# timweiland/DiffEqGMRFs.jl

Hardware: AMD Instinct MI355X
Metric: GMRF posterior solves/sec (mean+samples), 256^2 Darcy (higher is better)
Workload: dtype f64; 1 GPU; darcy256: n=65536, 64 blocks x 1024, nnz=1624084; 256 independent posterior(s) per GPU and step (4 stream(s) x batch 64), each factor + mean + 64 samples; mode=problems, samples_per_problem_per_rank=64, l_blocks_kept=False

## Files before the change

### diffeqgmrfs.jl_amd/api.py

```python
from __future__ import annotations

import ctypes as C
from typing import List, Optional, Sequence, Tuple

import numpy as np
import scipy.sparse as sp

from . import _cabi
from ._cabi import GmrfError, NotPositiveDefinite


def _is_torch(x) -> bool:
    return hasattr(x, "data_ptr") and hasattr(x, "device")


def _colmajor(b, n: int):
    if _is_torch(b):
        import torch
        if b.dtype != torch.float64:
            raise TypeError("float64 required")
        if b.dim() == 1:
            if b.shape[0] != n:
                raise ValueError("dimension mismatch")
            return b.contiguous(), 1, n, True
# ... 453 lines not shown
        return {f: (list(getattr(s, f)) if hasattr(getattr(s, f), "__len__") else getattr(s, f)) for f, _ in s._fields_}

    def select_problem(self, p: int):
        _cabi.check(self._lib.gmrf_bt_select_problem(self._h, int(p)))

    def solve_batch(self, b, mode: int = _cabi.SOLVE_FULL):
        B, k, n = b.shape
        if B != self.batch or n != self.N:
            raise ValueError("expected shape (batch, k, n)")
        if _is_torch(b):
            import torch
            b = b.contiguous()
            out = torch.empty_like(b)
        else:
            b = np.ascontiguousarray(b, dtype=np.float64)
            out = np.empty_like(b)
        _cabi.check(self._lib.gmrf_bt_solve(self._h, _cabi.ptr(b), _cabi.ptr(out), k, n, n, mode))
        return out

    def sample_batch(self, k: int, mean=None, seed: int = 0x5EED, first_id: int = 0, like=None):
        B, n = self.batch, self.N
        ref = like if like is not None else mean
        if _is_torch(ref):
            import torch
            out = torch.empty((B, k, n), dtype=torch.float64, device=ref.device)
            if mean is not None:
                mean = mean.contiguous()
        else:
            out = np.empty((B, k, n), dtype=np.float64)
            if mean is not None:
                mean = np.ascontiguousarray(mean, dtype=np.float64)
        _cabi.check(self._lib.gmrf_bt_sample(self._h, seed, first_id, k, _cabi.ptr(mean), None, _cabi.ptr(out), n))
        return out

    def factor(self, A, N_blocks: int, values=None):
        A = sp.csc_matrix(A)
        if A.shape[0] != A.shape[1]:
            raise ValueError("matrix must be square")
        if not A.has_sorted_indices:
            A = A.copy()
            A.sort_indices()
        n = A.shape[0]
        colptr = A.indptr.astype(np.int64)
        rowval = A.indices.astype(np.int64)
        nz = np.ascontiguousarray(A.data if values is None else values, dtype=np.float64)
        if nz.size != self.batch * A.nnz:
            raise ValueError("values must hold batch * nnz entries")
        info = C.c_int32(0)
        st = self._lib.gmrf_bt_factor_csc(self._h, n, int(N_blocks), _cabi.ptr(colptr), _cabi.ptr(rowval),
                                          _cabi.ptr(nz), 0, C.byref(info))
        _cabi.check(st, info.value)
        self._set_shape(n, int(N_blocks))
        self._pattern = (colptr, rowval)
        return self

    def factor_blocks(self, diag_blocks, off_diag_blocks):
        nb = len(diag_blocks)
        bs = diag_blocks[0].shape[0]
        keep = []

        def mk(blocks):
            arr = (_cabi.SparseBlock * max(len(blocks), 1))()
            for i, b in enumerate(blocks):
                b = sp.csc_matrix(b)
                b.sort_indices()
                p = b.indptr.astype(np.int64); ix = b.indices.astype(np.int64); v = b.data.astype(np.float64)
                keep.extend([p, ix, v])
                arr[i].nnz = b.nnz
                arr[i].ptr = p.ctypes.data; arr[i].idx = ix.ctypes.data; arr[i].val = v.ctypes.data
            return arr

        d = mk(diag_blocks)
        lo = mk(off_diag_blocks)
        info = C.c_int32(0)
        st = self._lib.gmrf_bt_factor_blocks(self._h, nb * bs, nb, C.cast(d, C.c_void_p), C.cast(lo, C.c_void_p),
                                             0, 1, C.byref(info))
        _cabi.check(st, info.value)
        self._set_shape(nb * bs, nb)
        return self

    def refactor(self, nzval):
        info = C.c_int32(0)
        if not _is_torch(nzval):
            nzval = np.ascontiguousarray(nzval, dtype=np.float64)
        st = self._lib.gmrf_bt_refactor_values(self._h, _cabi.ptr(nzval), C.byref(info))
        _cabi.check(st, info.value)
        return self

    def _set_shape(self, n, nb):
        self.N = n
        self.n_blocks = nb
        self.block_size = n // nb
        self.chos = _LazyBlocks(self, _cabi.BLOCK_L, nb)
        self.Cs = _LazyBlocks(self, _cabi.BLOCK_C, nb - 1)
        self.inverses = _LazyBlocks(self, _cabi.BLOCK_LINV, nb)

    def _solve(self, b, mode: int, out=None):
        xa, k, ld, one_d = _colmajor(b, self.N)
        if out is None:
            store, view = _alloc_like(xa, self.N, k, one_d)
        else:
            store, view = out, out
        _cabi.check(self._lib.gmrf_bt_solve(self._h, _cabi.ptr(xa), _cabi.ptr(store), k, ld, self.N, mode))
        return view

    def get_block(self, kind: int, i: int) -> np.ndarray:
        bs = self.block_size
        out = np.empty((bs, bs), dtype=np.float64, order="F")
        _cabi.check(self._lib.gmrf_bt_get_block(self._h, kind, i, _cabi.ptr(out), bs))
        return out

    def logdet(self) -> float:
        v = C.c_double(0.0)
        _cabi.check(self._lib.gmrf_bt_logdet(self._h, C.byref(v)))
        return v.value

    def normals(self, k: int, seed: int = 0x5EED, first_id: int = 0, like=None):
        if self.batch != 1:
            raise ValueError("a batched handle draws (batch, k, n) normals: normals_batch")
        store, view = _alloc_like(like if like is not None else np.empty(0), self.N, k, False)
        _cabi.check(self._lib.gmrf_bt_normals(self._h, seed, first_id, k, _cabi.ptr(store), self.N))
        return view

    def normals_batch(self, k: int, seed: int = 0x5EED, first_id: int = 0):
        out = np.empty((self.batch, k, self.N), dtype=np.float64)
        _cabi.check(self._lib.gmrf_bt_normals(self._h, seed, first_id, k, _cabi.ptr(out), self.N))
        return out

    def sample(self, k: int, mean=None, z=None, seed: int = 0x5EED, first_id: int = 0, like=None):
        ref = like if like is not None else (z if z is not None else (mean if mean is not None else np.empty(0)))
        za = None
        if z is not None:
            za, kz, _, _ = _colmajor(z, self.N)
            k = kz
        if mean is not None and not _is_torch(mean):
            mean = np.ascontiguousarray(mean, dtype=np.float64)
        store, view = _alloc_like(ref if _is_torch(ref) else np.empty(0), self.N, k, False)
        _cabi.check(self._lib.gmrf_bt_sample(self._h, seed, first_id, k, _cabi.ptr(mean), _cabi.ptr(za),
                                             _cabi.ptr(store), self.N))
        return view

    def posterior(self, b, k: int, seed: int = 0x5EED, first_id: int = 0):
        if self.batch != 1:
            raise ValueError("posterior(): one problem per handle (use solve_batch / sample_batch for batches)")
        xa, kb, ld, one_d = _colmajor(b, self.N)
        if kb != 1:
            raise ValueError("posterior(): one right-hand side")
        mstore, mview = _alloc_like(xa, self.N, 1, True)
        sstore, sview = _alloc_like(xa, self.N, k, False)
        _cabi.check(self._lib.gmrf_bt_posterior(self._h, _cabi.ptr(xa), seed, first_id, k, _cabi.ptr(mstore), _cabi.ptr(sstore),
                                                self.N))
        return mview, sview

    def marginal_var(self, method: str = "exact", k: int = 50, seed: int = 0x5EED, Q: Optional[CsrMatrix] = None,
                     q_values=None, out=None):
        m = {"exact": _cabi.VAR_EXACT, "rbmc": _cabi.VAR_RBMC, "mc": _cabi.VAR_MC}[method]
        shape = (self.N,) if self.batch == 1 else (self.batch, self.N)
        if out is None:
            out = np.empty(shape, dtype=np.float64)
        else:
            ok = tuple(out.shape) == shape and (out.is_contiguous() and str(out.dtype) == "torch.float64" if _is_torch(out)
                                                else out.flags.c_contiguous and out.dtype == np.float64)
            if not ok:
                raise ValueError(f"out must be a contiguous float64 array of shape {shape}")
        if self.batch > 1 and m != _cabi.VAR_EXACT:
            qv = None
            if q_values is not None:
                qv = q_values.contiguous() if _is_torch(q_values) else np.ascontiguousarray(q_values, dtype=np.float64)
            _cabi.check(self._lib.gmrf_bt_marginal_var_batch(self._h, m, k, seed, Q._h if Q is not None else None,
                                                             _cabi.ptr(qv) if qv is not None else None, _cabi.ptr(out)))
            return out
        _cabi.check(self._lib.gmrf_bt_marginal_var(self._h, m, k, seed, Q._h if Q is not None else None,
                                                   _cabi.ptr(out)))
        return out

    def var_accumulate(self, acc, method: str, first_id: int, k: int, seed: int = 0x5EED,
                       Q: Optional[CsrMatrix] = None):
        m = {"rbmc": _cabi.VAR_RBMC, "mc": _cabi.VAR_MC}[method]
        _cabi.check(self._lib.gmrf_bt_var_accumulate(self._h, m, first_id, k, seed,
                                                     Q._h if Q is not None else None, _cabi.ptr(acc)))
        return acc

    def stats(self) -> dict:
        s = _cabi.Stats()
        _cabi.check(self._lib.gmrf_bt_stats(self._h, C.byref(s)))
        out = {}
        for f, _ in s._fields_:
            v = getattr(s, f)
            out[f] = list(v) if hasattr(v, "__len__") else v
        return out

    def gemm_shapes(self) -> list:
        n = C.c_int64(0)
        _cabi.check(self._lib.gmrf_test_gemm_shapes(self._h, None, 0, C.byref(n)))
        buf = np.zeros((max(int(n.value), 1), 11))
        _cabi.check(self._lib.gmrf_test_gemm_shapes(self._h, buf.ctypes.data_as(C.POINTER(C.c_double)), buf.shape[0], C.byref(n)))
        names = ("class", "M", "N", "K", "tri", "lower_only", "problems", "k_bounds")
        return [dict({k: int(r[i]) for i, k in enumerate(names)}, launches=int(r[8]), ms=float(r[9]), flops=float(r[10]))
                for r in buf[: int(n.value)]]

    def set_profiling(self, level: int):
        _cabi.check(self._lib.gmrf_bt_set_profiling(self._h, level))

    def set_eager(self, eager: bool):
        _cabi.check(self._lib.gmrf_bt_set_eager(self._h, int(eager)))

    def synchronize(self):
        _cabi.check(self._lib.gmrf_bt_synchronize(self._h))

    def factor_buffer(self, kind: int) -> Tuple[int, int]:
        p = C.c_void_p()
        nbytes = C.c_int64(0)
        _cabi.check(self._lib.gmrf_bt_factor_buffer(self._h, kind, C.byref(p), C.byref(nbytes)))
        return int(p.value or 0), int(nbytes.value)

    def export_factor(self) -> np.ndarray:
        nbytes = C.c_int64(0)
        _cabi.check(self._lib.gmrf_bt_export_size(self._h, C.byref(nbytes)))
        buf = np.empty(nbytes.value, dtype=np.uint8)
        _cabi.check(self._lib.gmrf_bt_export_factor(self._h, _cabi.ptr(buf), nbytes.value))
        return buf

    def import_factor(self, image: np.ndarray):
        image = np.ascontiguousarray(image, dtype=np.uint8)
        _cabi.check(self._lib.gmrf_bt_import_factor(self._h, _cabi.ptr(image), image.size))
        hdr = image[:64].view(np.int64)
        self._set_shape(int(hdr[2]), int(hdr[3]))
        return self

    def adopt_shape(self, n: int, n_blocks: int):
        _cabi.check(self._lib.gmrf_bt_adopt_shape(self._h, n, n_blocks))
        self._set_shape(n, n_blocks)

    def get_layout(self) -> np.ndarray:
        cnt = C.c_int64(0)
        _cabi.check(self._lib.gmrf_bt_get_layout(self._h, None, 0, C.byref(cnt)))
        out = np.zeros(cnt.value, dtype=np.int64)
        _cabi.check(self._lib.gmrf_bt_get_layout(self._h, _cabi.ptr(out), out.size, C.byref(cnt)))
        return out

    def adopt_layout(self, n: int, n_blocks: int, layout=None):
        if layout is None:
            _cabi.check(self._lib.gmrf_bt_adopt_layout(self._h, n, n_blocks, None, 0))
        else:
            lay = np.ascontiguousarray(layout, dtype=np.int64)
            _cabi.check(self._lib.gmrf_bt_adopt_layout(self._h, n, n_blocks, _cabi.ptr(lay), lay.size))
        self._set_shape(n, n_blocks)

    def adopt_commit(self, l_blocks_valid: bool = False):
        _cabi.check(self._lib.gmrf_bt_adopt_commit(self._h, int(l_blocks_valid)))

    def set_keep_l(self, keep: bool):
        _cabi.check(self._lib.gmrf_bt_set_keep_l(self._h, int(keep)))

    def block_range(self, kind: int, i0: int, i1: int):
        a, b, c = C.c_int64(0), C.c_int64(0), C.c_int64(0)
        _cabi.check(self._lib.gmrf_bt_block_range(self._h, kind, i0, i1, C.byref(a), C.byref(b), C.byref(c)))
        return a.value, b.value, c.value

    def packed_size(self, i0: int, i1: int) -> int:
        v = C.c_int64(0)
        _cabi.check(self._lib.gmrf_bt_packed_size(self._h, i0, i1, C.byref(v)))
        return v.value

    def pack_blocks_async(self, i0: int, i1: int, dev_buf):
        _cabi.check(self._lib.gmrf_bt_pack_blocks_async(self._h, i0, i1, _cabi.ptr(dev_buf)))

    def unpack_blocks_async(self, i0: int, i1: int, dev_buf):
        _cabi.check(self._lib.gmrf_bt_unpack_blocks_async(self._h, i0, i1, _cabi.ptr(dev_buf)))

    def factor_begin(self, A, N_blocks: int):
        A = sp.csc_matrix(A)
        n = A.shape[0]
        colptr = A.indptr.astype(np.int64); rowval = A.indices.astype(np.int64)
        nz = np.ascontiguousarray(A.data, dtype=np.float64)
        _cabi.check(self._lib.gmrf_bt_factor_begin_csc(self._h, n, int(N_blocks), _cabi.ptr(colptr),
                                                       _cabi.ptr(rowval), _cabi.ptr(nz), 0))
        self._set_shape(n, int(N_blocks))

    def factor_begin_values(self, nzval):
        if not _is_torch(nzval):
            nzval = np.ascontiguousarray(nzval, dtype=np.float64)
        _cabi.check(self._lib.gmrf_bt_factor_begin_csc(self._h, self.N, self.n_blocks, None, None,
                                                       _cabi.ptr(nzval), 0))

    def factor_step_async(self, i0: int, i1: int):
        _cabi.check(self._lib.gmrf_bt_factor_step_async(self._h, i0, i1))

    def factor_end(self):
        info = C.c_int32(0)
        st = self._lib.gmrf_bt_factor_end(self._h, C.byref(info))
        _cabi.check(st, info.value)



def tridiagonal_cholesky(A, N_blocks: int, device: int = 0, stream: int = 0, order: str = "reference",
                         meet: Optional[int] = None) -> TridiagonalCholeskyFactor:
    n = A.shape[0]
    if N_blocks <= 0 or n % N_blocks != 0:
        raise ValueError("size(A,1) must be a positive multiple of N_blocks")
    return TridiagonalCholeskyFactor(device, stream, order=order, meet=meet).factor(A, N_blocks)


def forward_solve(L: TridiagonalCholeskyFactor, b):
    return L._solve(b, _cabi.SOLVE_FORWARD)

# ... 124 lines not shown
```

### diffeqgmrfs.jl_amd/csrc/gemm_f64_dma.hpp

```cpp
#pragma once
#include "gemm_f64.hpp"

namespace gmrf {

constexpr int DMA_BK = 16;
constexpr int DMA_ROWS_ASCENDING = 1024;
#ifndef GMRF_DMA_READS_FIRST
#define GMRF_DMA_READS_FIRST 0
#endif

template <int BM, int BN>
constexpr size_t gemm_dma_lds_bytes(int stages) { return (size_t)stages * (BM + BN) * DMA_BK * sizeof(double); }

#define GMRF_LDS_PTR(p) ((__attribute__((address_space(3))) void*)(p))
#define GMRF_GLB_PTR(p) ((const __attribute__((address_space(1))) void*)(p))

template <int BM, int BN>
__device__ __forceinline__ void gemm_dma_tile_order(const GemmArgs& g, int& bm, int& bn, int& z) {
    const int nx = g.N / BN, ny = g.M / BM;
    int tpp;
    if (g.lower_only == 1) {
        if (BM >= BN) tpp = (BM / BN) * ny * (ny + 1) / 2;
        else tpp = 0;
    } else tpp = nx * ny;
    const int nz = (int)gridDim.x / tpp;
    const int groups = (nz % 8 == 0) ? 8 : 1;
    const int xg = (int)blockIdx.x % groups, q = (int)blockIdx.x / groups, nzg = nz / groups;
    int zq;
    if (g.lower_only == 1) {
        constexpr int R = BM / BN > 0 ? BM / BN : 1;
        const int tile = q % tpp;
        zq = q / tpp;
        const int tr = (g.tri & DMA_ROWS_ASCENDING) ? tile : tpp - 1 - tile;
        int b = (int)((sqrtf(8.0f * (float)(tr / R) + 1.0f) - 1.0f) * 0.5f);
        while (R * b * (b + 1) / 2 > tr) --b;
        while (R * (b + 1) * (b + 2) / 2 <= tr) ++b;
        bm = b;
        bn = tr - R * b * (b + 1) / 2;
    } else {
        const bool cls_n = (g.tri & (TRI_B_LOWER | TRI_B_UPPER)) || !(g.tri & (TRI_A_LOWER | TRI_A_UPPER));
        const bool desc = cls_n ? ((g.tri & TRI_B_UPPER) != 0 || (g.ke_n && !g.kb_n)) : (g.tri & TRI_A_LOWER) != 0;
        const int ncls = cls_n ? nx : ny, other = cls_n ? ny : nx;
        int c = q / (other * nzg);
        const int rem = q % (other * nzg);
        const int o = rem % other;
        zq = rem / other;
        if (desc) c = ncls - 1 - c;
        bn = cls_n ? c : o;
        bm = cls_n ? o : c;
    }
    z = xg + groups * zq;
}

template <int BM, int BN, bool B_N, int STAGES, bool A_T = false>
__global__ __launch_bounds__(256, (BM + BN > 128) ? 3 : 4) void gemm_f64_dma(GemmArgs g) {
    constexpr int BK = DMA_BK;
    constexpr int MI = BM / 32, NJ = BN / 32;
    constexpr int NA = BM / 32, NB = BN / 32;
    constexpr int A_ST = BM * BK, B_ST = BN * BK, ST = A_ST + B_ST;
    static_assert(NJ % 2 == 0 || !B_N, "the [k][n] image pairs neighbouring column tiles");
    static_assert(MI % 2 == 0 || !A_T, "the [k][m] image pairs neighbouring row tiles");
    int bm, bn, z;
    gemm_dma_tile_order<BM, BN>(g, bm, bn, z);
    const int m0 = bm * BM, n0 = bn * BN;
    if (g.lower_only == 2 && n0 > m0 + BM - 1) return;
    const int zi = z % g.nb1, zp = z / g.nb1;
    const double* __restrict__ A = g.A + (int64_t)zi * g.strideA + (int64_t)zp * g.pA;
    const double* __restrict__ B = g.B + (int64_t)zi * g.strideB + (int64_t)zp * g.pB;
    double* C = g.C + (int64_t)zi * g.strideC + (int64_t)zp * g.pC;
    const double* Dm = g.D ? g.D + (int64_t)zp * g.pD : C;
    const int64_t ldd = g.D ? g.ldd : g.ldc;

    int kb = 0, ke = g.K;
    if (g.tri & TRI_A_LOWER) ke = min(ke, m0 + BM);
    if (g.tri & TRI_A_UPPER) kb = max(kb, m0);
    if (g.tri & TRI_B_LOWER) kb = max(kb, n0);
    if (g.tri & TRI_B_UPPER) ke = min(ke, n0 + BN);
    if (g.kb_m) kb = max(kb, g.kb_m[bm * (BM / 64)]);
    if (g.kb_n) kb = max(kb, g.kb_n[bn * (BN / 64)]);
    if (g.ke_n) ke = min(ke, g.ke_n[bn * (BN / 64) + BN / 64 - 1]);
    const int nkt = (ke > kb) ? (ke - kb) / BK : 0;

    extern __shared__ __attribute__((aligned(16))) double gsm[];
    const int t = threadIdx.x;
    const int lane = t & 63, w = __builtin_amdgcn_readfirstlane(t >> 6);
    const int wm = (w >> 1) * (BM / 2), wn = (w & 1) * (BN / 2);
    const int li = lane & 15, lq = lane >> 4;
    const bool idle = g.lower_only != 0 && ((n0 + wn) / 64 > (m0 + wm + BM / 2 - 1) / 64);

    uint32_t offa[NA], offb[NB];
#pragma unroll
    for (int i = 0; i < NA; ++i) {
        const int q = w + 4 * i;
        if (A_T) {
            constexpr int LPR = BM / 2;
            const int k = q * (64 / LPR) + lane / LPR, col = (lane % LPR) * 2;
            offa[i] = (uint32_t)(((int64_t)k * g.lda + m0 + col) * 8);
        } else {
            const int row = 8 * q + (lane >> 3), ch = (lane & 7) ^ ((row >> 1) & 7);
            offa[i] = (uint32_t)(((int64_t)(m0 + row) * g.lda + 2 * ch) * 8);
        }
    }
#pragma unroll
    for (int i = 0; i < NB; ++i) {
        const int q = w + 4 * i;
        if (B_N) {
            constexpr int LPR = BN / 2;
            const int k = q * (64 / LPR) + lane / LPR, col = (lane % LPR) * 2;
            offb[i] = (uint32_t)(((int64_t)k * g.ldb + n0 + col) * 8);
        } else {
            const int row = 8 * q + (lane >> 3), ch = (lane & 7) ^ ((row >> 1) & 7);
            offb[i] = (uint32_t)(((int64_t)(n0 + row) * g.ldb + 2 * ch) * 8);
        }
    }
    auto issue = [&](int kt, int stage) {
        const int k0 = kb + kt * BK;
        const char* abase = reinterpret_cast<const char*>(A_T ? A + (int64_t)k0 * g.lda : A + k0);
        const char* bbase = reinterpret_cast<const char*>(B_N ? B + (int64_t)k0 * g.ldb : B + k0);
        double* as = gsm + stage * ST;
        double* bs = as + A_ST;
#pragma unroll
        for (int i = 0; i < NA; ++i) {
            asm volatile("" : "+v"(offa[i]));
            __builtin_amdgcn_global_load_lds(GMRF_GLB_PTR(abase + offa[i]), GMRF_LDS_PTR(as + (w + 4 * i) * 128), 16, 0, 0);
        }
#pragma unroll
        for (int i = 0; i < NB; ++i) {
            asm volatile("" : "+v"(offb[i]));
            __builtin_amdgcn_global_load_lds(GMRF_GLB_PTR(bbase + offb[i]), GMRF_LDS_PTR(bs + (w + 4 * i) * 128), 16, 0, 0);
        }
    };

    v4d acc[MI][NJ];
#pragma unroll
    for (int i = 0; i < MI; ++i)
#pragma unroll
        for (int j = 0; j < NJ; ++j) acc[i][j] = (v4d){0.0, 0.0, 0.0, 0.0};

    int fa[MI], fb[NJ];
#pragma unroll
    for (int i = 0; i < MI; ++i) {
        const int row = wm + 16 * i + li;
        fa[i] = A_T ? (2 * lq + (i & 1)) * BM + wm + 32 * (i >> 1) + 2 * li : row * 16 + 2 * (lq ^ ((row >> 1) & 3));
    }
    int sa2[MI], sb2[NJ];
#pragma unroll
    for (int i = 0; i < MI; ++i) { const int row = wm + 16 * i + li; sa2[i] = (!A_T && ((row >> 1) & 4)) ? 8 : 0; }
    if (!B_N) {
#pragma unroll
        for (int j = 0; j < NJ; ++j) {
            const int row = wn + 16 * j + li;
            fb[j] = A_ST + row * 16 + 2 * (lq ^ ((row >> 1) & 3));
            sb2[j] = ((row >> 1) & 4) ? 8 : 0;
        }
    } else {
#pragma unroll
        for (int j = 0; j < NJ; ++j) { fb[j] = A_ST + (2 * lq + (j & 1)) * BN + wn + 32 * (j >> 1) + 2 * li; sb2[j] = 0; }
    }

    constexpr int DEPTH = STAGES - 1;
#pragma unroll
    for (int s = 0; s < DEPTH; ++s)
        if (s < nkt) issue(s, s);
    for (int kt = 0; kt < nkt; ++kt) {
        const int ahead = min(DEPTH - 1, nkt - 1 - kt);
        if (ahead <= 0) asm volatile("s_waitcnt vmcnt(0)" ::: "memory");
        else if (ahead == 1) asm volatile("s_waitcnt vmcnt(%0)" ::"n"(NA + NB) : "memory");
        else asm volatile("s_waitcnt vmcnt(%0)" ::"n"(2 * (NA + NB)) : "memory");
        __builtin_amdgcn_s_barrier();
        __builtin_amdgcn_sched_barrier(0);
        if (!GMRF_DMA_READS_FIRST && kt + DEPTH < nkt) issue(kt + DEPTH, (kt + DEPTH) % STAGES);
        if (!idle) {
            const double* sm = gsm + (kt % STAGES) * ST;
            v2d a[BK / 8][MI], b[BK / 8][NJ];
#pragma unroll
            for (int kg = 0; kg < BK / 8; ++kg) {
#pragma unroll
                for (int i = 0; i < MI; ++i) a[kg][i] = *reinterpret_cast<const v2d*>(sm + fa[i] + (A_T ? kg * 8 * BM : ((kg * 8) ^ sa2[i])));
#pragma unroll
                for (int j = 0; j < NJ; ++j)
                    b[kg][j] = *reinterpret_cast<const v2d*>(sm + fb[j] + (B_N ? kg * 8 * BN : ((kg * 8) ^ sb2[j])));
            }
            __builtin_amdgcn_sched_barrier(0);
            if (GMRF_DMA_READS_FIRST && kt + DEPTH < nkt) issue(kt + DEPTH, (kt + DEPTH) % STAGES);
            __builtin_amdgcn_sched_barrier(0);
#pragma unroll
            for (int kg = 0; kg < BK / 8; ++kg)
#pragma unroll
                for (int p = 0; p < 2; ++p)
#pragma unroll
                    for (int i = 0; i < MI; ++i)
#pragma unroll
                        for (int j = 0; j < NJ; ++j) {
                            double av;
                            if (A_T) av = (i & 1) ? a[kg][2 * (i >> 1) + p].y : a[kg][2 * (i >> 1) + p].x;
                            else av = p ? a[kg][i].y : a[kg][i].x;
                            double bv;
                            if (B_N) bv = (j & 1) ? b[kg][2 * (j >> 1) + p].y : b[kg][2 * (j >> 1) + p].x;
                            else bv = p ? b[kg][j].y : b[kg][j].x;
                            acc[i][j] = __builtin_amdgcn_mfma_f64_16x16x4f64(av, bv, acc[i][j], 0, 0, 0);
                        }
            __builtin_amdgcn_sched_barrier(0);
        } else if (GMRF_DMA_READS_FIRST && kt + DEPTH < nkt) issue(kt + DEPTH, (kt + DEPTH) % STAGES);
    }
    if (idle) return;

    const double alpha = g.alpha, beta = g.beta;
    auto orow = [&](int i, int r) -> int64_t {
        return A_T ? m0 + wm + 32 * (i >> 1) + 2 * (lq + 4 * r) + (i & 1) : m0 + wm + i * 16 + lq + 4 * r;
    };
    if (B_N) {
        v2d d[MI][4][NJ / 2 > 0 ? NJ / 2 : 1];
        if (beta != 0.0) {
#pragma unroll
            for (int i = 0; i < MI; ++i)
#pragma unroll
                for (int r = 0; r < 4; ++r)
#pragma unroll
                    for (int jp = 0; jp < NJ / 2; ++jp)
                        d[i][r][jp] = *reinterpret_cast<const v2d*>(Dm + orow(i, r) * ldd + n0 + wn + jp * 32 + 2 * li);
        }
#pragma unroll
        for (int i = 0; i < MI; ++i)
#pragma unroll
            for (int r = 0; r < 4; ++r)
#pragma unroll
                for (int jp = 0; jp < NJ / 2; ++jp) {
                    v2d v = (v2d){alpha * acc[i][2 * jp][r], alpha * acc[i][2 * jp + 1][r]};
                    if (beta != 0.0) { v.x += beta * d[i][r][jp].x; v.y += beta * d[i][r][jp].y; }
                    *reinterpret_cast<v2d*>(C + orow(i, r) * g.ldc + n0 + wn + jp * 32 + 2 * li) = v;
                }
    } else {
        double d[MI][4][NJ];
        if (beta != 0.0) {
#pragma unroll
            for (int i = 0; i < MI; ++i)
#pragma unroll
                for (int r = 0; r < 4; ++r)
#pragma unroll
                    for (int j = 0; j < NJ; ++j)
                        d[i][r][j] = Dm[orow(i, r) * ldd + n0 + wn + j * 16 + li];
        }
#pragma unroll
        for (int i = 0; i < MI; ++i)
#pragma unroll
            for (int r = 0; r < 4; ++r)
#pragma unroll
                for (int j = 0; j < NJ; ++j) {
                    double v = alpha * acc[i][j][r];
                    if (beta != 0.0) v += beta * d[i][r][j];
                    C[orow(i, r) * g.ldc + n0 + wn + j * 16 + li] = v;
                }
    }
}

inline int& gemm_dma_policy() {
    static int v = [] { const char* e = getenv("GMRF_GEMM_DMA"); return e ? atoi(e) : 2; }();
    return v;
}
inline int& gemm_dma_force() {
    static int v = 0;
    return v;
}
inline int gemm_dma_stages() {
    static const int v = [] { const char* e = getenv("GMRF_GEMM_DMA_STAGES"); const int s = e ? atoi(e) : 2; return s == 3 ? 3 : 2; }();
    return v;
}

inline int gemm_dma_shape(bool a_t, const GemmArgs& g, int batch) {
    const int policy = gemm_dma_force() ? 2 : gemm_dma_policy();
    if (policy == 0 || g.stamps || (g.tri & ~15) || g.K % DMA_BK || g.M % 64 || g.N % 64) return 0;
    if ((g.lda & 1) || (g.ldb & 1) || ((uintptr_t)g.A & 15) || ((uintptr_t)g.B & 15) || ((g.strideA | g.strideB | g.pA | g.pB) & 1)) return 0;
    if (((uintptr_t)g.C & 15) || (g.ldc & 1) || ((g.strideC | g.pC) & 1)) return 0;
    if (g.D && (((uintptr_t)g.D & 15) || (g.ldd & 1) || (g.pD & 1))) return 0;
    if ((int64_t)g.M * g.ldc * 8 >= ((int64_t)1 << 32) || (g.D && (int64_t)g.M * g.ldd * 8 >= ((int64_t)1 << 32))) return 0;
    if ((int64_t)(a_t ? g.K : g.M) * g.lda * 8 >= ((int64_t)1 << 32) || (int64_t)std::max(g.N, g.K) * g.ldb * 8 >= ((int64_t)1 << 32)) return 0;
    if (a_t) return 1;
    const int force = gemm_dma_force();
    if (force == 2 && g.M % 128 == 0) return 2;
    if (force == 3 && g.N % 128 == 0 && !g.lower_only) return 3;
    if (force) return 1;
    if (policy == 1) return 1;
    const bool plain = !g.lower_only && !g.tri && !g.kb_m && !g.kb_n && !g.ke_n;
    const int64_t t64 = (int64_t)(g.M / 64) * (g.N / 64) * batch;
    if (policy >= 3 || (plain && t64 >= 2048)) {
        if (g.M % 128 == 0) return 2;
        if (g.N % 128 == 0 && !g.lower_only) return 3;
    }
    return 1;
}
inline bool gemm_uses_dma(bool a_t, const GemmArgs& g, int batch) { return gemm_dma_shape(a_t, g, batch) != 0; }

inline hipError_t gemm_dma_init() {
    hipError_t e = hipSuccess;
#define GMRF_DMA_ATTR(BM, BN, BNAT, ST)                                                                          \
    if (e == hipSuccess)                                                                                          \
        e = hipFuncSetAttribute((const void*)gemm_f64_dma<BM, BN, BNAT, ST>, hipFuncAttributeMaxDynamicSharedMemorySize, \
                                (int)gemm_dma_lds_bytes<BM, BN>(ST) + 64 * 1024);
    GMRF_DMA_ATTR(64, 64, false, 2) GMRF_DMA_ATTR(64, 64, true, 2) GMRF_DMA_ATTR(64, 64, false, 3) GMRF_DMA_ATTR(64, 64, true, 3)
    GMRF_DMA_ATTR(128, 64, false, 2) GMRF_DMA_ATTR(128, 64, true, 2) GMRF_DMA_ATTR(128, 64, false, 3) GMRF_DMA_ATTR(128, 64, true, 3)
    GMRF_DMA_ATTR(64, 128, false, 2) GMRF_DMA_ATTR(64, 128, true, 2) GMRF_DMA_ATTR(64, 128, false, 3) GMRF_DMA_ATTR(64, 128, true, 3)
#undef GMRF_DMA_ATTR
    return e;
}

inline bool gemm_try_dma(hipStream_t st, bool a_t, bool b_n, const GemmArgs& g, int batch, hipEvent_t ev_start, hipEvent_t ev_stop,
                         hipError_t* err) {
    const int shape = gemm_dma_shape(a_t, g, batch);
    if (shape == 0) return false;
    const bool tri_grid = g.lower_only && g.M == g.N;
    GemmArgs gs = g;
    gs.lower_only = tri_grid ? 1 : (g.lower_only ? 2 : 0);
    static const bool asc_off = [] { const char* e = getenv("GMRF_GEMM_G2_ORDER"); return e && atoi(e) == 0; }();
    if (tri_grid && (g.kb_m || g.kb_n) && !asc_off) gs.tri |= DMA_ROWS_ASCENDING;
    const int stages = gemm_dma_stages();
    const dim3 block(256);
#define GMRF_DMA_GO(BM, BN)                                                                                       \
    do {                                                                                                          \
        const int64_t nx = g.N / BN, ny = g.M / BM;                                                               \
        const int64_t tiles = tri_grid ? (int64_t)(BM / BN > 0 ? BM / BN : 1) * ny * (ny + 1) / 2 : nx * ny;      \
        const dim3 grid((unsigned)(tiles * batch));                                                               \
        static const size_t lds_pad = [] { const char* e = getenv("GMRF_GEMM_DMA_LDS_PAD_KB"); return (size_t)(e ? atoi(e) : 0) * 1024; }();    \
        const size_t lds = gemm_dma_lds_bytes<BM, BN>(stages) + lds_pad;                                          \
        if (a_t && BM == 64 && BN == 64) {                                                                        \
            if (b_n) GMRF_DMA_K((gemm_f64_dma<64, 64, true, 2, true>)); else GMRF_DMA_K((gemm_f64_dma<64, 64, false, 2, true>)); \
        } else if (stages == 3) {                                                                                 \
            if (b_n) GMRF_DMA_K((gemm_f64_dma<BM, BN, true, 3>)); else GMRF_DMA_K((gemm_f64_dma<BM, BN, false, 3>)); \
        } else {                                                                                                  \
            if (b_n) GMRF_DMA_K((gemm_f64_dma<BM, BN, true, 2>)); else GMRF_DMA_K((gemm_f64_dma<BM, BN, false, 2>)); \
        }                                                                                                         \
    } while (0)
#define GMRF_DMA_K(KERNEL)                                                                                        \
    do {                                                                                                          \
        if (ev_start) hipExtLaunchKernelGGL(KERNEL, grid, block, lds, st, ev_start, ev_stop, 0, gs);              \
        else hipLaunchKernelGGL(KERNEL, grid, block, lds, st, gs);                                                \
    } while (0)
    if (shape == 2) GMRF_DMA_GO(128, 64);
    else if (shape == 3) GMRF_DMA_GO(64, 128);
    else GMRF_DMA_GO(64, 64);
#undef GMRF_DMA_K
#undef GMRF_DMA_GO
    *err = hipGetLastError();
    return true;
}

}
```

### diffeqgmrfs.jl_amd/csrc/gmrf_hip.hip

```cpp
#include <hip/hip_runtime.h>
#include <dlfcn.h>
#include <stdint.h>
#include <stdlib.h>
#include <string.h>
#include <time.h>

#include <algorithm>
#include <iterator>
#include <cmath>
#include <map>
#include <memory>
#include <chrono>
#include <functional>
#include <initializer_list>
#include <mutex>
#include <string>
#include <type_traits>
#include <vector>

#include "../../include/gmrf_hip.h"
#include "assemble.hpp"
#include "fem_assemble.hpp"
#include "gemm_f64.hpp"
#include "gemm_f64_dma.hpp"
// ... 4 lines not shown
#include "sweep.hpp"
#include "sweep_persist.hpp"
#include "swe_assemble.hpp"
#include "fem_assemble_p2.hpp"

using namespace gmrf;

static thread_local std::string g_last_error;
static double g_tile_us = 0.0;
static unsigned long long g_tile_stamps[64];
static unsigned long long g_persist_stamps[128];

#define HIPCHK(expr)                                                                        \
    do {                                                                                    \
        hipError_t _e = (expr);                                                             \
        if (_e != hipSuccess) {                                                             \
            g_last_error = std::string(#expr) + ": " + hipGetErrorString(_e);               \
            return GMRF_ERR_HIP;                                                            \
        }                                                                                   \
    } while (0)

#define GCHK(expr)                                                                          \
    do {                                                                                    \
        gmrf_status _s = (expr);                                                            \
        if (_s != GMRF_OK) return _s;                                                       \
    } while (0)

static gmrf_status bad_shape(const char* msg) {
    g_last_error = msg;
    return GMRF_ERR_BAD_SHAPE;
}

static bool is_device_ptr(const void* p) {
    if (!p) return false;
    hipPointerAttribute_t attr;
    hipError_t e = hipPointerGetAttributes(&attr, p);
    if (e != hipSuccess) {
        (void)hipGetLastError();
        return false;
    }
    return attr.type == hipMemoryTypeDevice || attr.type == hipMemoryTypeManaged;
}

static bool ranges_overlap(const void* p, int64_t pb, const void* q, int64_t qb) {
    if (!p || !q || pb <= 0 || qb <= 0) return false;
    const uintptr_t a = reinterpret_cast<uintptr_t>(p), b = reinterpret_cast<uintptr_t>(q);
    return a < b + (uintptr_t)qb && b < a + (uintptr_t)pb;
}

static int64_t cols_bytes(int64_t n, int64_t cols, int64_t ld) {
    return cols <= 0 ? 0 : ((cols - 1) * ld + n) * (int64_t)sizeof(double);
}

static int64_t next_pow2(int64_t v) {
    int64_t p = 1;
    while (p < v) p <<= 1;
    return p;
}

struct gmrf_csr {
    int device = 0;
    hipStream_t stream = nullptr;
    bool own_stream = false;
    int64_t n_rows = 0, n_cols = 0, nnz = 0;
    int64_t* d_rowptr = nullptr;
    int32_t* d_colidx = nullptr;
    double* d_vals = nullptr;
    float* d_vals32 = nullptr;
    double* d_diag = nullptr;
    bool tiles128_ok = false;
    bool tiles_ok = false;
    double* d_stage_x = nullptr;
    double* d_stage_y = nullptr;
    int64_t stage_cap = 0;
    int plan_state = 0;
    int64_t* d_tile_uptr = nullptr;
    int32_t* d_ucols = nullptr;
    uint16_t* d_lidx = nullptr;
    int64_t n_ucols = 0;
    int plan_rows = 0, plan_ucap = 0, plan_ecap = 0, plan_ecap_pad = 0, plan_umax = 0;
};

struct EvPair {
    hipEvent_t a, b;
    int kind;
    double work;
    int shape = -1;
};

struct GemmShapeStat {
    int64_t key[8];
    double launches = 0, ms = 0, work = 0;
};

struct TwistState;

struct gmrf_handle {
    int device = 0;
    hipStream_t stream = nullptr;
    bool own_stream = false;
    int64_t n = 0, N = 0, bs = 0, bsp = 0, n_pad = 0;
    int64_t B = 1;
    int64_t sel = 0;
    int64_t alloc_B = 0, vals_B = 0;
    int64_t nnz_in = 0, n_entries = 0;
    uint64_t* d_keys = nullptr;
    double* d_vals = nullptr;
    int64_t* d_src = nullptr;
    double* d_nz_stage = nullptr;
    std::vector<int64_t> diag_first, diag_count, low_first, low_count;
    bool analyzed = false;
    int64_t cmin = 0, rmax = 0;
    std::vector<int> kst, mend;
    int* d_kst = nullptr;
    int* d_mend = nullptr;
    int* d_kbx = nullptr;
    int kst_cap = 0;
    double c_streamed = 0.0;
    double g2_tile_k = 0.0;
    bool c_dirty = false;
    int* d_lo_rowptr = nullptr;
    int* d_dg_rowptr = nullptr;
    int* d_bxt_uptr = nullptr; int* d_bxt_ucols = nullptr; uint16_t* d_bxt_lidx = nullptr; int* d_bxt_gtiles = nullptr;
    std::vector<int> bxt_ng;
    int bxt_ecap = 0; int bxt_nrt = 0; bool bxt_plan_ok = false;
    int64_t lo_row_max = 0;
    bool sparse_b = false;
    bool dense_g1 = false;
    double *d_L = nullptr, *d_C = nullptr, *d_Linv = nullptr;
    bool external_storage = false;
    bool keep_l = true;
    bool l_valid = false;
    bool logdet_valid = false;
    std::vector<char> got_block;
    int64_t alloc_rm = 0, alloc_wc = 0;
    bool alloc_keep_l = true;
    double *d_S = nullptr, *d_B = nullptr, *d_T = nullptr, *d_W = nullptr;
    double* d_V = nullptr;
    int64_t v_elems = 0;
    int* d_info = nullptr;
    double* d_logdet = nullptr;
    int64_t alloc_N = 0, alloc_bsp = 0;
    bool factored = false;
    double *d_P = nullptr, *d_Y = nullptr, *d_Tp = nullptr;
    int64_t kp_cap = 0;
    double* d_stage = nullptr;
    int64_t stage_cap = 0;
    double* d_mean = nullptr;
    double* d_acc = nullptr;
    int64_t acc_B = 0;
    bool eager = false;
    bool split_step = false;
    bool sweep_no_gemm = false;
    unsigned long long* dbg_stamps = nullptr;
    bool fork_graph = false;
    bool no_staircase = false;
    bool doubling_x = false;
    int xsplit = 0;
    int adopt_xsplit = 0;
    bool no_xsplit = false;
    bool no_lookahead = false;
    bool no_persist = false;
    bool persist_gave_up = false;
    bool persist_launched = false;
    int persist_cus = 0;
    int info_checked = 0;
    int factor_graph_route = 0;
    int persist_aborts = 0;
    int cu_count = 0;
    unsigned* d_pflags = nullptr;
    int64_t pflags_words = 0;
    bool no_sweep_persist = false;
    bool no_scatter_fold = false;
    bool sweep_persist_planned = false;
    bool sweep_persist_launched = false;
    unsigned* d_sweep_flags = nullptr;
    double* d_Tsw = nullptr;
    int64_t t_elems = 0;
    unsigned* h_sweep_abort = nullptr;
    int sweep_nw = 0;
    double *d_P2 = nullptr, *d_Y2 = nullptr, *d_T2 = nullptr;
    int64_t p2_elems = 0;
    bool sweep_persist_hold = false;
    bool no_persist_panels = false;
    hipStream_t aux = nullptr;
    bool aux_distinct = false;
    hipStream_t gemm_stream = nullptr;
    bool capturing = false;
    std::vector<hipEvent_t> fork_events;
    size_t fork_next = 0;
    hipGraphExec_t factor_graph = nullptr;
    int64_t factor_graph_i0 = -1, factor_graph_i1 = -1;
    std::map<int64_t, hipGraphExec_t> sweep_graphs;
    int profiling = 0;
    std::vector<EvPair> events;
    std::vector<hipEvent_t> ev_pool;
    std::vector<GemmShapeStat> gemm_shapes;
    gmrf_stats stats;
    hipEvent_t ev0 = nullptr, ev1 = nullptr;
    int order = GMRF_ORDER_REFERENCE;
    int64_t meet_req = -1;
    int32_t eager_bits = 0;
    TwistState* tw = nullptr;
    int64_t tw_blk = -1;
    const double* tw_hj = nullptr;
    double* tw_w = nullptr;
};

struct TwistState {
    gmrf_handle* top = nullptr;
    gmrf_handle* bot = nullptr;
    int64_t m = -1, N = 0, n = 0, bs = 0, bsp = 0, nnz = 0;
    uint64_t* d_mkeys = nullptr;
    int64_t* d_msrc = nullptr;
    double* d_mvals = nullptr;
    int64_t m_count = 0;
    double *d_Bm = nullptr, *d_HJ = nullptr, *d_W = nullptr, *d_Smm = nullptr;
    int64_t dense_bsp = 0;
    double* d_nz = nullptr;
    const double* d_nz_cur = nullptr;
    double* d_z = nullptr;
    double* d_var = nullptr;
    hipEvent_t ev_fork = nullptr, ev_join = nullptr;
};


static bool tw_on(const gmrf_handle* h) { return h && h->tw && h->tw->bot; }
static gmrf_handle* tw_route(gmrf_handle* h) {
    return (h && h->order == GMRF_ORDER_TWISTED && h->tw && h->tw->top && !h->tw->bot && h->factored) ? h->tw->top : h;
}
static gmrf_status tw_refuse(const gmrf_handle* h, const char* what) {
    if (!h || h->order != GMRF_ORDER_TWISTED) return GMRF_OK;
    g_last_error = std::string(what) + ": not supported on a handle in the twisted elimination order (gmrf_bt_set_order)";
    return GMRF_ERR_BAD_SHAPE;
}

static void destroy_graphs(gmrf_handle* h) {
    if (h->factor_graph) { (void)hipGraphExecDestroy(h->factor_graph); h->factor_graph = nullptr; }
    for (auto& kv : h->sweep_graphs) (void)hipGraphExecDestroy(kv.second);
    h->sweep_graphs.clear();
}

static hipEvent_t ev_get(gmrf_handle* h) {
    if (!h->ev_pool.empty()) {
        hipEvent_t e = h->ev_pool.back();
        h->ev_pool.pop_back();
        return e;
    }
    hipEvent_t e;
    (void)hipEventCreate(&e);
    return e;
}

struct ProfScope {
    gmrf_handle* h;
    EvPair p;
    bool on;
    ProfScope(gmrf_handle* hh, int kind, double work) : h(hh), on(hh->profiling > 0) {
        if (on) {
            p.kind = kind; p.work = work;
            p.a = ev_get(h); p.b = ev_get(h);
            (void)hipEventRecord(p.a, h->stream);
        }
    }
    ~ProfScope() {
        if (on) {
            (void)hipEventRecord(p.b, h->stream);
            h->events.push_back(p);
        }
    }
};

static void prof_collect(gmrf_handle* h) {
    for (auto& p : h->events) {
        float ms = 0.f;
        (void)hipEventElapsedTime(&ms, p.a, p.b);
        h->stats.kernel_ms[p.kind] += ms; h->stats.kernel_work[p.kind] += p.work; h->stats.kernel_launches[p.kind]++;
        if (p.shape >= 0) { auto& g = h->gemm_shapes[(size_t)p.shape]; g.launches += 1; g.ms += ms; g.work += p.work; }
        h->ev_pool.push_back(p.a);
        h->ev_pool.push_back(p.b);
    }
    h->events.clear();
}

static gmrf_status gemm(gmrf_handle* h, bool a_t, bool b_n, int M, int N, int K, int tri, int lower_only,
                        double alpha, const double* A, int64_t lda, const double* B, int64_t ldb,
                        double beta, double* C, int64_t ldc, int64_t pA, int64_t pB, int64_t pC,
                        int batch = 1, int64_t sA = 0, int64_t sB = 0, int64_t sC = 0, const double* D = nullptr,
                        int64_t ldd = 0, int64_t pD = 0, int pclass = 0, double pwork = -1.0,
                        const int* kb_m = nullptr, const int* kb_n = nullptr, const int* ke_n = nullptr) {
    GemmArgs g;
    g.kb_m = kb_m; g.kb_n = kb_n; g.ke_n = ke_n;
    g.D = D; g.ldd = ldd; g.pD = pD;
    g.A = A; g.B = B; g.C = C;
    g.lda = lda; g.ldb = ldb; g.ldc = ldc;
    g.strideA = sA; g.strideB = sB; g.strideC = sC;
    g.pA = pA; g.pB = pB; g.pC = pC; g.nb1 = batch;
    g.M = M; g.N = N; g.K = K; g.tri = tri; g.lower_only = lower_only;
    g.alpha = alpha; g.beta = beta; g.stamps = nullptr;
    double flops = 2.0 * M * N * (double)K * batch * (double)h->B;
    if (lower_only) flops *= 0.5 * (1.0 + 64.0 / std::max(M, 64));
    if (tri) flops *= 0.5 * (1.0 + 64.0 / std::max(K, 64));
    if (gemm_uses_big(a_t, g, batch * (int)h->B)) { pclass = b_n ? 7 : 6; pwork = -1.0; }
    else if (pclass == 0) {
        if (gemm_uses_ll(g, batch * (int)h->B)) pclass = 13;
        else if (gemm_uses_dma(a_t, g, batch * (int)h->B)) pclass = a_t ? 18 : (b_n ? 15 : 14);
        else pclass = a_t ? 12 : (b_n ? 11 : 0);
    }
    if (h->profiling > 0) {
        EvPair p;
        p.kind = pclass; p.work = pwork >= 0.0 ? pwork : flops;
        p.a = ev_get(h); p.b = ev_get(h);
        const int64_t key[8] = {pclass, M, N, K, tri, lower_only, batch * h->B, (kb_m || kb_n || ke_n) ? 1 : 0};
        for (size_t i = 0; i < h->gemm_shapes.size() && p.shape < 0; ++i)
            if (!memcmp(h->gemm_shapes[i].key, key, sizeof(key))) p.shape = (int)i;
        if (p.shape < 0) {
            GemmShapeStat st; memcpy(st.key, key, sizeof(key));
            h->gemm_shapes.push_back(st); p.shape = (int)h->gemm_shapes.size() - 1;
        }
        HIPCHK(launch_gemm(h->gemm_stream ? h->gemm_stream : h->stream, a_t, b_n, g, batch * (int)h->B, p.a, p.b));
        h->events.push_back(p);
        return GMRF_OK;
    }
    HIPCHK(launch_gemm(h->gemm_stream ? h->gemm_stream : h->stream, a_t, b_n, g, batch * (int)h->B));
    return GMRF_OK;
}

static void free_dev(void* p) {
    if (p) (void)hipFree(p);
}

static inline int64_t blk_elems(const gmrf_handle* h) { return h->bsp * h->bsp; }
static inline int64_t c_ld(const gmrf_handle* h) { return h->bsp - h->cmin; }
static inline int64_t c_blk(const gmrf_handle* h) { return h->rmax * (h->bsp - h->cmin); }
static inline int64_t stride_pL(const gmrf_handle* h) { return blk_elems(h) * (h->keep_l ? h->N : 1); }
static inline int64_t stride_pX(const gmrf_handle* h) { return blk_elems(h) * h->N; }
static inline int64_t stride_pC(const gmrf_handle* h) { return c_blk(h) * std::max<int64_t>(h->N - 1, 1); }
static inline double* l_block(const gmrf_handle* h, int64_t i) { return h->d_L + (h->keep_l ? i * blk_elems(h) : 0); }

static gmrf_status set_layout(gmrf_handle* h, int64_t cmin, int64_t rmax, const std::vector<int64_t>& kst_abs) {
    const int64_t bsp = h->bsp;
    if (cmin < 0 || cmin >= bsp || cmin % 64 || rmax <= 0 || rmax > bsp || rmax % 64) return bad_shape("bad coupling-block layout");
    const int nrt = (int)(rmax / 64), nct = (int)((bsp - cmin) / 64), ntile = (int)(bsp / 64);
    if ((int)kst_abs.size() != nrt) return bad_shape("bad coupling-block layout (row tiles)");
    (void)hipStreamSynchronize(h->stream);
    destroy_graphs(h);
    h->cmin = cmin; h->rmax = rmax;
    h->kst.assign((size_t)ntile, 0);
    int64_t run = bsp - 64;
    for (int t = nrt - 1; t >= 0; --t) {
        int64_t v = std::min(std::max(kst_abs[t], cmin), bsp - 64);
        run = std::min(run, (v / 64) * 64);
        h->kst[t] = (int)(run - cmin);
    }
    if (nrt > 0) h->kst[0] = 0;
    for (int t = nrt; t < ntile; ++t) h->kst[t] = (int)(bsp - cmin);
    h->mend.assign((size_t)ntile, (int)rmax);
    for (int u = 0; u < nct; ++u) {
        int m = 0;
        for (int t = 0; t < nrt; ++t) if (h->kst[t] <= 64 * u) m = 64 * (t + 1);
        h->mend[u] = m;
    }
    h->c_streamed = 0.0; h->g2_tile_k = 0.0;
    for (int t = 0; t < nrt; ++t) {
        h->c_streamed += 64.0 * (double)(bsp - cmin - h->kst[t]);
        h->g2_tile_k += (double)(t + 1) * (double)(bsp - cmin - h->kst[t]);
    }
    if (!h->d_kst || !h->d_mend || h->kst_cap < ntile) {
        free_dev(h->d_kst); free_dev(h->d_mend); free_dev(h->d_kbx); h->d_kst = h->d_mend = h->d_kbx = nullptr; h->kst_cap = 0;
        HIPCHK(hipMalloc(&h->d_kst, sizeof(int) * ntile));
        HIPCHK(hipMalloc(&h->d_mend, sizeof(int) * ntile));
        HIPCHK(hipMalloc(&h->d_kbx, sizeof(int) * ntile));
        h->kst_cap = ntile;
    }
    {
        std::vector<int> kbx((size_t)ntile);
        for (int u = 0; u < ntile; ++u) kbx[(size_t)u] = (int)std::max<int64_t>(0, 64 * (int64_t)u - cmin);
        HIPCHK(hipMemcpyAsync(h->d_kbx, kbx.data(), sizeof(int) * ntile, hipMemcpyHostToDevice, h->stream));
        HIPCHK(hipStreamSynchronize(h->stream));
    }
    HIPCHK(hipMemcpyAsync(h->d_kst, h->kst.data(), sizeof(int) * ntile, hipMemcpyHostToDevice, h->stream));
    HIPCHK(hipMemcpyAsync(h->d_mend, h->mend.data(), sizeof(int) * ntile, hipMemcpyHostToDevice, h->stream));
    HIPCHK(hipStreamSynchronize(h->stream));
    h->c_dirty = true;
    return GMRF_OK;
}

static gmrf_status set_layout_dense(gmrf_handle* h) {
    return set_layout(h, 0, h->bsp, std::vector<int64_t>((size_t)(h->bsp / 64), 0));
}

static gmrf_status alloc_work(gmrf_handle* h);
static gmrf_status alloc_factor(gmrf_handle* h) {
    if (h->alloc_N == h->N && h->alloc_bsp == h->bsp && h->alloc_B == h->B && h->alloc_rm == h->rmax &&
        h->alloc_wc == c_ld(h) && h->alloc_keep_l == h->keep_l && h->d_Linv)
        return GMRF_OK;
    destroy_graphs(h);
    h->logdet_valid = false;
    if (h->external_storage) {
        if (h->alloc_N != h->N || h->alloc_bsp != h->bsp || h->alloc_B != h->B || h->alloc_keep_l != h->keep_l) {
            g_last_error = "external factor storage does not match the shape / batch";
            return GMRF_ERR_BAD_SHAPE;
        }
        h->alloc_rm = h->rmax; h->alloc_wc = c_ld(h);
        h->l_valid = false;
        return GMRF_OK;
    }
    free_dev(h->d_L); free_dev(h->d_C); free_dev(h->d_Linv);
    free_dev(h->d_S); free_dev(h->d_B); free_dev(h->d_T); free_dev(h->d_W);
    free_dev(h->d_logdet);
    h->d_L = h->d_C = h->d_Linv = h->d_S = h->d_B = h->d_T = h->d_W = h->d_logdet = nullptr;
    h->l_valid = false;
    const size_t blk = (size_t)blk_elems(h) * sizeof(double) * (size_t)h->B;
    HIPCHK(hipMalloc(&h->d_L, blk * (h->keep_l ? h->N : 1)));
    HIPCHK(hipMalloc(&h->d_Linv, blk * h->N));
    HIPCHK(hipMalloc(&h->d_C, (size_t)stride_pC(h) * sizeof(double) * (size_t)h->B));
    HIPCHK(hipMemsetAsync(h->d_L, 0, blk * (h->keep_l ? h->N : 1), h->stream));
    HIPCHK(hipMemsetAsync(h->d_Linv, 0, blk * h->N, h->stream));
    HIPCHK(hipMemsetAsync(h->d_C, 0, (size_t)stride_pC(h) * sizeof(double) * (size_t)h->B, h->stream));
    h->c_dirty = false;
    GCHK(alloc_work(h));
    h->alloc_rm = h->rmax; h->alloc_wc = c_ld(h); h->alloc_keep_l = h->keep_l;
    return GMRF_OK;
}

static gmrf_status alloc_work(gmrf_handle* h) {
    const size_t blk = (size_t)blk_elems(h) * sizeof(double) * (size_t)h->B;
    HIPCHK(hipMalloc(&h->d_S, blk));
    HIPCHK(hipMalloc(&h->d_B, blk));
    HIPCHK(hipMalloc(&h->d_T, blk));
    HIPCHK(hipMalloc(&h->d_W, blk));
    HIPCHK(hipMalloc(&h->d_logdet, sizeof(double) * h->N * h->B));
    {
        const int64_t words = (int64_t)persist_flag_words((int)(h->bsp / 64)) * h->B;
        if (!h->d_pflags || h->pflags_words < words) {
            free_dev(h->d_pflags); h->d_pflags = nullptr; h->pflags_words = 0;
            HIPCHK(hipMalloc(&h->d_pflags, sizeof(unsigned) * (size_t)words));
            HIPCHK(hipMemsetAsync(h->d_pflags, 0, sizeof(unsigned) * (size_t)words, h->stream));
            HIPCHK(hipStreamSynchronize(h->stream));
            h->pflags_words = words;
        }
    }
    h->alloc_N = h->N; h->alloc_bsp = h->bsp; h->alloc_B = h->B;
    h->stats.factor_bytes = (int64_t)(blk * ((h->keep_l ? 2 : 1) * h->N) + (size_t)stride_pC(h) * sizeof(double) * (size_t)h->B);
    return GMRF_OK;
}

static void release_shape_buffers(gmrf_handle* h) {
    for (auto& kv : h->sweep_graphs) (void)hipGraphExecDestroy(kv.second);
    h->sweep_graphs.clear();
    free_dev(h->d_P); free_dev(h->d_Y); free_dev(h->d_Tp);
    h->d_P = h->d_Y = h->d_Tp = nullptr; h->kp_cap = 0;
    free_dev(h->d_mean); h->d_mean = nullptr;
    free_dev(h->d_acc); h->d_acc = nullptr; h->acc_B = 0;
    free_dev(h->d_stage); h->d_stage = nullptr; h->stage_cap = 0;
// ... 909 lines not shown
    return std::chrono::duration<double, std::milli>(std::chrono::steady_clock::now() - t0).count();
}

gmrf_status gmrf_streams_create(int32_t device, int32_t n, void** streams, int32_t* n_distinct) {
    if (n <= 0 || n > 32 || !streams) return bad_shape("gmrf_streams_create: 1 <= n <= 32 streams");
    HIPCHK(hipSetDevice(device));
    const int ncand = std::min(3 * n + 4, 48);
    std::vector<hipStream_t> cand((size_t)ncand, nullptr);
    for (int i = 0; i < ncand; ++i) {
        if (hipStreamCreateWithFlags(&cand[(size_t)i], hipStreamNonBlocking) != hipSuccess) {
            for (int j = 0; j < i; ++j) (void)hipStreamDestroy(cand[(size_t)j]);
            g_last_error = "hipStreamCreateWithFlags failed"; return GMRF_ERR_HIP;
        }
        hipLaunchKernelGGL(gmrf_spin_kernel, dim3(1), dim3(64), 0, cand[(size_t)i], 1ull);
    }
    HIPCHK(hipDeviceSynchronize());
    const unsigned long long ticks = 100000ull;
    double one = 1e30;
    for (int r = 0; r < 3; ++r) one = std::min(one, spin_pair_ms(cand[0], nullptr, ticks));
    std::vector<int> chosen;
    for (int i = 0; i < ncand && (int)chosen.size() < n; ++i) {
        bool ok = true;
        for (int c : chosen) {
            const double t = std::min(spin_pair_ms(cand[(size_t)c], cand[(size_t)i], ticks), spin_pair_ms(cand[(size_t)c], cand[(size_t)i], ticks));
            if (t > 1.5 * one) { ok = false; break; }
        }
        if (ok) chosen.push_back(i);
    }
    const int nd = (int)chosen.size();
    std::vector<char> used((size_t)ncand, 0);
    for (int c : chosen) used[(size_t)c] = 1;
    for (int i = 0; i < ncand && (int)chosen.size() < n; ++i)
        if (!used[(size_t)i]) { chosen.push_back(i); used[(size_t)i] = 1; }
    for (int k = 0; k < n; ++k) streams[k] = (void*)cand[(size_t)chosen[(size_t)k]];
    for (int i = 0; i < ncand; ++i)
        if (!used[(size_t)i]) (void)hipStreamDestroy(cand[(size_t)i]);
    if (n_distinct) *n_distinct = nd;
    return GMRF_OK;
}

gmrf_status gmrf_streams_destroy(int32_t device, int32_t n, void** streams) {
    if (n < 0 || (n > 0 && !streams)) return bad_shape("gmrf_streams_destroy");
    HIPCHK(hipSetDevice(device));
    for (int k = 0; k < n; ++k)
        if (streams[k]) { (void)hipStreamSynchronize((hipStream_t)streams[k]); (void)hipStreamDestroy((hipStream_t)streams[k]); streams[k] = nullptr; }
    return GMRF_OK;
}

static double sweep_bytes(const gmrf_handle* h, int64_t k) {
    const double bs = (double)h->bs, N = (double)h->N;
    return 8.0 * (N * bs * (bs + 1) / 2.0 + (N - 1) * bs * bs) + 16.0 * (double)h->n * (double)k;
}

static bool sweep_persist_ok(const gmrf_handle* h, int kp) {
    if (!h->sweep_persist_planned || h->sweep_persist_hold || h->no_sweep_persist || h->no_persist || h->persist_gave_up || h->B != 1 || h->xsplit != 0) return false;
    if (h->persist_cus < h->cu_count || sweep_persist_demand(h) <= 0) return false;
    if (kp != 1 && (kp % 16 != 0 || (int64_t)kp * h->n_pad * 8 >= ((int64_t)1 << 31))) return false;
    if (h->n_pad * 8 >= ((int64_t)1 << 31)) return false;
    const bool via_gemm = (kp % 64 == 0) && !h->sweep_no_gemm && (int64_t)(h->bsp / 64) * (kp / 64) >= 128;
    return !via_gemm;
}

static gmrf_status sweep_persist_prepare(gmrf_handle* h, int kp) {
    if (!h->d_sweep_flags) {
        HIPCHK(hipMalloc(&h->d_sweep_flags, sizeof(unsigned) * 16));
        HIPCHK(hipMemsetAsync(h->d_sweep_flags, 0, sizeof(unsigned) * 16, h->stream));
    }
    h->sweep_nw = std::min(256, h->cu_count);
    if (!h->h_sweep_abort) {
        HIPCHK(hipHostMalloc(reinterpret_cast<void**>(&h->h_sweep_abort), 64, hipHostMallocMapped));
        *h->h_sweep_abort = 0u;
    }
    const int64_t need = (int64_t)kp * h->n_pad;
    if (!h->d_Tsw || h->t_elems < need) {
        HIPCHK(hipStreamSynchronize(h->stream));
        free_dev(h->d_Tsw); h->d_Tsw = nullptr; h->t_elems = 0;
        destroy_graphs(h);
        HIPCHK(hipMalloc(&h->d_Tsw, sizeof(double) * (size_t)need));
        h->t_elems = need;
    }
    return GMRF_OK;
}

static gmrf_status launch_sweep_persist(gmrf_handle* h, bool backward, int kp, double* Pin, double* Yout, hipStream_t st_over = nullptr,
                                        double* T_over = nullptr) {
    const int nw = h->sweep_nw;
    const int64_t elems = (int64_t)kp * h->n_pad;
    hipStream_t st = st_over ? st_over : h->stream;
    double* Tp = T_over ? T_over : h->d_Tsw;
    if (!h->d_sweep_flags || !h->h_sweep_abort || nw <= 0 || !Tp || (!T_over && h->t_elems < elems))
        return bad_shape("internal: words / panel of the persistent sweeps not allocated");
    if (elems % 2 != 0) return bad_shape("internal: the persistent sweeps' panels need an even element count (sweep_fill_sentinel)");
    SweepPersistArgs a;
    a.C = h->d_C; a.Linv = h->d_Linv; a.Pin = Pin; a.T = Tp; a.Yout = Yout;
    a.N = (int)h->N; a.bsp = (int)h->bsp; a.cm = (int)h->cmin; a.rm = (int)h->rmax; a.kp = kp; a.backward = backward ? 1 : 0; a.nw = nw;
    a.npad = h->n_pad; a.ldc = c_ld(h); a.cstride = c_blk(h); a.bstride = (int64_t)h->bsp * h->bsp;
    a.kst = h->d_kst; a.mend = h->d_mend;
    a.abort_w = h->d_sweep_flags;
    void* dev_abort = nullptr;
    HIPCHK(hipHostGetDevicePointer(&dev_abort, h->h_sweep_abort, 0));
    a.host_abort = reinterpret_cast<unsigned*>(dev_abort);
    static const int limit_ms = [] {
        const char* e = getenv("GMRF_SWEEP_SPIN_MS");
        if (!e) e = getenv("GMRF_PERSIST_SPIN_MS");
        return e ? atoi(e) : -1;
    }();
    a.spin_limit = (unsigned)(limit_ms >= 0 ? limit_ms : 2000) * 100000u;
    static const int dbg = [] { const char* e = getenv("GMRF_SWEEP_DBG"); return e ? atoi(e) : 0; }();
    a.dbg = dbg;
    static const int pause_env = [] { const char* e = getenv("GMRF_SWEEP_PAUSE"); return e ? atoi(e) : -1; }();
    a.pause = (kp == 1) ? 8 : (pause_env >= 0 ? pause_env : 64);
    const double N = (double)h->N, bsp = (double)h->bsp;
    const double work = (kp == 1) ? 8.0 * ((N - 1) * h->c_streamed + N * 0.5 * bsp * (bsp + 1))
                                  : kp * (2.0 * (N - 1) * h->c_streamed + N * bsp * (bsp + 1));
    {
        ProfScope ps(h, 5, 16.0 * (double)elems);
        hipLaunchKernelGGL(sweep_fill_sentinel, dim3((unsigned)((elems / 2 + 255) / 256)), dim3(256), 0, st, Tp, Yout, elems);
        HIPCHK(hipGetLastError());
    }
    ProfScope ps(h, kp == 1 ? 19 : 20, work);
    if (kp == 1) hipLaunchKernelGGL(sweep_persist<true>, dim3((unsigned)nw), dim3(256), 0, st, a);
    else hipLaunchKernelGGL(sweep_persist<false>, dim3((unsigned)nw), dim3(256), 0, st, a);
    HIPCHK(hipGetLastError());
    return GMRF_OK;
}

static gmrf_status sweep_persist_check(gmrf_handle* h, bool* repeat) {
    *repeat = false;
    if (!h->sweep_persist_launched) return GMRF_OK;
    h->sweep_persist_launched = false;
    if (!h->h_sweep_abort || *reinterpret_cast<volatile unsigned*>(h->h_sweep_abort) == 0u) return GMRF_OK;
    *h->h_sweep_abort = 0u;
    persist_give_up(h);
    HIPCHK(hipMemsetAsync(h->d_sweep_flags, 0, sizeof(unsigned) * 16, h->stream));
    h->stats.sweep_persist = 0;
    *repeat = true;
    return GMRF_OK;
}

struct SweepIo { const void* in; int64_t in_bytes; const void* out; int64_t out_bytes; };

static gmrf_status sweep_guarded(gmrf_handle* h, std::initializer_list<SweepIo> io, const std::function<gmrf_status()>& body,
                                 const std::function<gmrf_status()>& restore = nullptr) {
    h->stats.sweep_persist = 0;
    h->sweep_persist_hold = std::any_of(io.begin(), io.end(), [](const SweepIo& r) { return ranges_overlap(r.in, r.in_bytes, r.out, r.out_bytes); });
    GCHK(body());
    bool repeat = false;
    GCHK(sweep_persist_check(h, &repeat));
    if (!repeat) return GMRF_OK;
    if (restore) GCHK(restore());
    return body();
}

static gmrf_status sweep_launches(gmrf_handle* h, bool backward, int kp, double* Pin, double* Yout) {
    if (sweep_persist_ok(h, kp)) return launch_sweep_persist(h, backward, kp, Pin, Yout);
    const int bsp = (int)h->bsp;
    const int64_t ld = bsp, bstride = (int64_t)bsp * bsp, npad = h->n_pad;
    const int64_t N = h->N;
    SweepArgs s;
    s.ld = ld;
    const int nprob = (int)h->B;
    s.narrow = (nprob < 8 && bsp >= 512 && bsp <= SWEEP_PERSIST_XMAX) ? 1 : 0;
    const int64_t pPanel = (int64_t)kp * npad;
    const int64_t pX = stride_pX(h), pCm = stride_pC(h);
    const int64_t ldc = c_ld(h), cstride = c_blk(h);
    const int cm = (int)h->cmin, rm = (int)h->rmax, wc = bsp - cm;
    const int pclass = (kp == 1) ? 3 : 2;
    const double blk_work_c = ((kp == 1) ? 8.0 * h->c_streamed : 2.0 * h->c_streamed * kp) * nprob;
    const double blk_work_t = ((kp == 1) ? 4.0 * bsp * (double)(bsp + 1) : 1.0 * bsp * (double)(bsp + 1) * kp) * nprob;
    const bool via_gemm = (kp % 64 == 0) && !h->sweep_no_gemm && (int64_t)nprob * (bsp / 64) * (kp / 64) >= 128;
    for (int64_t step = 0; step < N; ++step) {
        const int64_t i = backward ? (N - 1 - step) : step;
        double* rhs = Pin + i * bsp;
        if (step > 0) {
            const int64_t ci = backward ? i : (i - 1);
            const int64_t prev = backward ? (i + 1) : (i - 1);
            const double* Cs = h->d_C + ci * cstride;
            const double* xin = Yout + prev * bsp + (backward ? 0 : cm);
            double* out = rhs + (backward ? cm : 0);
            const int rows = backward ? wc : rm, kdim = backward ? rm : wc;
            if (via_gemm) {
                GCHK(gemm(h, false, backward, kp, rows, kdim, 0, 0, -1.0, xin, npad, Cs, ldc, 1.0, out, npad, pPanel, pCm,
                          pPanel, 1, 0, 0, 0, nullptr, 0, 0, 0, 2.0 * h->c_streamed * kp * nprob,
                          nullptr, backward ? nullptr : h->d_kst, backward ? h->d_mend : nullptr));
            } else {
                s.Mat = Cs; s.ld = ldc; s.Xin = xin; s.ldx = npad; s.Bin = out; s.ldb = npad; s.Out = out; s.ldo = npad;
                s.rows = rows; s.kdim = kdim; s.sub = 1;
                s.pMat = pCm; s.pXin = pPanel; s.pBin = pPanel; s.pOut = pPanel;
                s.kst = h->d_kst; s.mend = h->d_mend;
                ProfScope ps(h, pclass, blk_work_c);
                HIPCHK(launch_sweep(h->stream, backward, false, kp, s, nprob));
            }
        }
        const double* X = h->d_Linv + i * bstride;
        double* yout = Yout + i * bsp;
        if (h->xsplit > 0) {
            const int p = h->xsplit, q = bsp - p;
            const double* Xbb = X + (int64_t)p * ld + p;
            const double* Lba = X + (int64_t)p * ld;
            for (int part = 0; part < 3; ++part) {
                const int which = backward ? 2 - part : part;
                if (via_gemm) {
                    if (which == 0)
                        GCHK(gemm(h, false, backward, kp, p, p, backward ? TRI_B_LOWER : TRI_B_UPPER, 0, 1.0, rhs, npad, X, ld, 0.0, yout, npad,
                                  pPanel, pX, pPanel));
                    else if (which == 2)
                        GCHK(gemm(h, false, backward, kp, q, q, backward ? TRI_B_LOWER : TRI_B_UPPER, 0, 1.0, rhs + p, npad, Xbb, ld, 0.0,
                                  yout + p, npad, pPanel, pX, pPanel));
                    else if (!backward)
                        GCHK(gemm(h, false, false, kp, q, p, 0, 0, -1.0, yout, npad, Lba, ld, 1.0, rhs + p, npad, pPanel, pX, pPanel));
                    else
                        GCHK(gemm(h, false, true, kp, p, q, 0, 0, -1.0, yout + p, npad, Lba, ld, 1.0, rhs, npad, pPanel, pX, pPanel));
                } else {
                    s.ld = ld; s.ldx = npad; s.ldo = npad; s.pMat = pX; s.pXin = pPanel; s.pOut = pPanel; s.kst = nullptr; s.mend = nullptr;
                    if (which == 0) { s.Mat = X; s.Xin = rhs; s.Bin = nullptr; s.ldb = 0; s.Out = yout; s.rows = p; s.kdim = p; s.sub = 0; s.pBin = 0; }
                    else if (which == 2) { s.Mat = Xbb; s.Xin = rhs + p; s.Bin = nullptr; s.ldb = 0; s.Out = yout + p; s.rows = q; s.kdim = q; s.sub = 0; s.pBin = 0; }
                    else if (!backward) { s.Mat = Lba; s.Xin = yout; s.Bin = rhs + p; s.ldb = npad; s.Out = rhs + p; s.rows = q; s.kdim = p; s.sub = 1; s.pBin = pPanel; }
                    else { s.Mat = Lba; s.Xin = yout + p; s.Bin = rhs; s.ldb = npad; s.Out = rhs; s.rows = p; s.kdim = q; s.sub = 1; s.pBin = pPanel; }
                    const double frac = which == 0 ? (double)p * (p + 1) : (which == 2 ? (double)q * (q + 1) : 2.0 * p * q);
                    ProfScope ps(h, pclass, blk_work_t * frac / ((double)bsp * (bsp + 1)));
                    HIPCHK(launch_sweep(h->stream, backward, which != 1, kp, s, nprob));
                }
            }
        } else if (via_gemm) {
            GCHK(gemm(h, false, backward, kp, bsp, bsp, backward ? TRI_B_LOWER : TRI_B_UPPER, 0, 1.0, rhs, npad, X, ld, 0.0,
                      yout, npad, pPanel, pX, pPanel, 1, 0, 0, 0, nullptr, 0, 0, 0, -1.0));
        } else {
            s.Mat = X; s.ld = ld; s.Xin = rhs; s.ldx = npad; s.Bin = nullptr; s.ldb = 0; s.Out = yout; s.ldo = npad;
            s.rows = bsp; s.kdim = bsp; s.sub = 0;
            s.pMat = pX; s.pXin = pPanel; s.pBin = 0; s.pOut = pPanel;
            s.kst = nullptr; s.mend = nullptr;
            ProfScope ps(h, pclass, blk_work_t);
            HIPCHK(launch_sweep(h->stream, backward, true, kp, s, nprob));
        }
    }
    return GMRF_OK;
}

constexpr int SWEEP_BACKWARD_YP = 3;
static gmrf_status run_sweeps(gmrf_handle* h, int mode, int kp) {
    auto body = [&]() -> gmrf_status {
        if (mode == GMRF_SOLVE_FORWARD) return sweep_launches(h, false, kp, h->d_P, h->d_Y);
        if (mode == SWEEP_BACKWARD_YP) return sweep_launches(h, true, kp, h->d_Y, h->d_P);
        if (mode == GMRF_SOLVE_BACKWARD) return sweep_launches(h, true, kp, h->d_P, h->d_Y);
        GCHK(sweep_launches(h, false, kp, h->d_P, h->d_Y));
        return sweep_launches(h, true, kp, h->d_Y, h->d_P);
    };
    const bool persistent = sweep_persist_ok(h, kp);
    if (persistent) {
        GCHK(sweep_persist_prepare(h, kp));
        h->sweep_persist_launched = true;
        h->stats.sweep_persist = 1;
        h->stats.sweep_persist_launches += (mode == GMRF_SOLVE_FULL) ? 2 : 1;
    }
    if (h->eager || h->profiling) return body();
    const int64_t key = ((int64_t)h->xsplit << 32) | ((int64_t)mode * 4096 + kp) |
                        (persistent ? ((int64_t)1 << 60) : 0);
    auto it = h->sweep_graphs.find(key);
    if (it == h->sweep_graphs.end()) {
        std::lock_guard<std::mutex> capture_lock(g_capture_mu);
        hipGraph_t graph = nullptr;
        hipGraphExec_t exec = nullptr;
        HIPCHK(hipStreamBeginCapture(h->stream, hipStreamCaptureModeThreadLocal));
        gmrf_status s = body();
        hipError_t e = hipStreamEndCapture(h->stream, &graph);
        if (s != GMRF_OK) { if (graph) (void)hipGraphDestroy(graph); return s; }
        HIPCHK(e);
        HIPCHK(hipGraphInstantiate(&exec, graph, nullptr, nullptr, 0));
        (void)hipGraphDestroy(graph);
        it = h->sweep_graphs.emplace(key, exec).first;
    }
    HIPCHK(hipGraphLaunch(it->second, h->stream));
    return GMRF_OK;
}

static int pad_k(int64_t k) { return k == 1 ? 1 : (int)((k + 15) / 16 * 16); }

static gmrf_status launch_pack(gmrf_handle* h, const double* d_src, int64_t ld, int k, int kp) {
    const int64_t total = (int64_t)kp * h->n_pad;
    hipLaunchKernelGGL(pack_panel, dim3((unsigned)((total + 255) / 256), (unsigned)h->B), dim3(256), 0, h->stream, d_src, ld,
                       h->d_P, h->n_pad, (int)h->bs, (int)h->bsp, (int)h->N, k, kp);
    HIPCHK(hipGetLastError());
    return GMRF_OK;
}

static gmrf_status launch_unpack(gmrf_handle* h, const double* panel, double* d_dst, int64_t ld, int k,
                                 const double* d_mean) {
    const int64_t total = h->n * (int64_t)k;
    hipLaunchKernelGGL(unpack_panel, dim3((unsigned)((total + 255) / 256), (unsigned)h->B), dim3(256), 0, h->stream, panel,
                       h->n_pad, d_dst, ld, (int)h->bs, (int)h->bsp, h->n, k, pad_k(k), d_mean);
    HIPCHK(hipGetLastError());
    return GMRF_OK;
}

static gmrf_status cols_in(gmrf_handle* h, const double* src, int64_t ld, bool src_dev, int k, const double** d_src, int64_t* d_ld) {
    *d_src = src; *d_ld = ld;
    if (src_dev) return GMRF_OK;
    GCHK(ensure_stage(h, (int64_t)k * h->n * h->B));
    HIPCHK(hipMemcpy2DAsync(h->d_stage, h->n * sizeof(double), src, ld * sizeof(double),
                            h->n * sizeof(double), k * h->B, hipMemcpyHostToDevice, h->stream));
    *d_src = h->d_stage; *d_ld = h->n;
    return GMRF_OK;
}

static gmrf_status cols_out(gmrf_handle* h, const double* panel, int k, const double* d_mean, double* dst, int64_t ld, bool dst_dev) {
    if (dst_dev) return launch_unpack(h, panel, dst, ld, k, d_mean);
    GCHK(ensure_stage(h, (int64_t)k * h->n * h->B));
    GCHK(launch_unpack(h, panel, h->d_stage, h->n, k, d_mean));
    HIPCHK(hipMemcpy2DAsync(dst, ld * sizeof(double), h->d_stage, h->n * sizeof(double),
                            h->n * sizeof(double), k * h->B, hipMemcpyDeviceToHost, h->stream));
    return GMRF_OK;
}

constexpr int64_t KP_CHUNK = 128;

static void tw_free(gmrf_handle* h);
static gmrf_status tw_analyze(gmrf_handle* h, int64_t n, int64_t N, const int64_t* colptr, const int64_t* rowval, int32_t base);
static gmrf_status tw_numeric(gmrf_handle* h, const double* nzval, int32_t* info);
static gmrf_status tw_solve(gmrf_handle* h, const double* b, double* y, int64_t k, int64_t ldb, int64_t ldy, int mode);
static gmrf_status tw_sample(gmrf_handle* h, uint64_t seed, int64_t first_id, int64_t k, const double* mean, const double* z,
                             double* out, int64_t ld);
static gmrf_status tw_logdet(gmrf_handle* h, double* out);
static gmrf_status tw_get_block(gmrf_handle* h, int32_t kind, int64_t i, double* out, int64_t ld);
static gmrf_status tw_var_exact(gmrf_handle* h, double* d_out);
static gmrf_status tw_var_accumulate_dev(gmrf_handle* h, int method, int64_t first_id, int64_t k, uint64_t seed, const gmrf_csr* Q,
                                         double* d_acc);

extern "C" {

int32_t gmrf_version(void) { return 100; }
const char* gmrf_last_error(void) { return g_last_error.c_str(); }

gmrf_status gmrf_bt_create(int32_t device, void* stream, gmrf_handle** out) {
    if (!out) return bad_shape("null out pointer");
    int count = 0;
    if (hipGetDeviceCount(&count) != hipSuccess || count <= 0 || device < 0 || device >= count) {
        (void)hipGetLastError();
        g_last_error = "no HIP device visible (libgmrf_hip needs an MI355X / gfx950 GPU)";
        return GMRF_ERR_NO_DEVICE;
    }
    HIPCHK(hipSetDevice(device));
    gmrf_handle* h = new gmrf_handle();
    memset(&h->stats, 0, sizeof(h->stats));
    h->device = device;
    if (stream) { h->stream = (hipStream_t)stream; h->own_stream = false; }
    else { HIPCHK(hipStreamCreateWithFlags(&h->stream, hipStreamNonBlocking)); h->own_stream = true; }
    HIPCHK(hipMalloc(&h->d_info, 4 * sizeof(int)));
    HIPCHK(hipMemsetAsync(h->d_info, 0, 4 * sizeof(int), h->stream));
    HIPCHK(hipStreamSynchronize(h->stream));
    HIPCHK(hipEventCreate(&h->ev0));
    HIPCHK(hipEventCreate(&h->ev1));
    HIPCHK(hipFuncSetAttribute((const void*)potrf_step<false>, hipFuncAttributeMaxDynamicSharedMemorySize, (int)POTRF_STEP_LDS));
    HIPCHK(hipFuncSetAttribute((const void*)potrf_diag128, hipFuncAttributeMaxDynamicSharedMemorySize, 160 * 1024));
    HIPCHK(hipFuncSetAttribute((const void*)potrf_persist<false>, hipFuncAttributeMaxDynamicSharedMemorySize, (int)POTRF_PERSIST_LDS));
    HIPCHK(hipDeviceGetAttribute(&h->cu_count, hipDeviceAttributeMultiprocessorCount, device));
    { const char* e = getenv("GMRF_PERSIST"); if (e && atoi(e) == 0) h->no_persist = true; }
    { const char* e = getenv("GMRF_SWEEP_PERSIST"); if (e && atoi(e) == 0) h->no_sweep_persist = true; }
    HIPCHK(hipFuncSetAttribute((const void*)potrf_diag128_slim, hipFuncAttributeMaxDynamicSharedMemorySize, 160 * 1024));
    HIPCHK(gemm_init());
    HIPCHK(gemm_dma_init());
    *out = h;
    return GMRF_OK;
}

gmrf_status gmrf_bt_destroy(gmrf_handle* h) {
    if (!h) return GMRF_OK;
    (void)hipSetDevice(h->device);
    tw_free(h);
    (void)hipStreamSynchronize(h->stream);
    persist_release(h);
    destroy_graphs(h);
    free_dev(h->d_keys); free_dev(h->d_vals); free_dev(h->d_src); free_dev(h->d_nz_stage);
    free_dev(h->d_lo_rowptr); free_dev(h->d_dg_rowptr); free_dev(h->d_kst); free_dev(h->d_mend);
    free_dev(h->d_bxt_uptr); free_dev(h->d_bxt_ucols); free_dev(h->d_bxt_lidx); free_dev(h->d_bxt_gtiles);
    if (!h->external_storage) { free_dev(h->d_L); free_dev(h->d_C); free_dev(h->d_Linv); }
    else if (!h->keep_l) free_dev(h->d_L);
    free_dev(h->d_S); free_dev(h->d_B); free_dev(h->d_T); free_dev(h->d_W);
    free_dev(h->d_sweep_flags); free_dev(h->d_Tsw); free_dev(h->d_P2); free_dev(h->d_Y2); free_dev(h->d_T2);
    if (h->h_sweep_abort) { (void)hipHostFree(h->h_sweep_abort); h->h_sweep_abort = nullptr; }
    free_dev(h->d_info); free_dev(h->d_logdet); free_dev(h->d_pflags); free_dev(h->d_kbx); free_dev(h->d_V);
    free_dev(h->d_P); free_dev(h->d_Y); free_dev(h->d_Tp);
    free_dev(h->d_stage); free_dev(h->d_mean); free_dev(h->d_acc);
    for (auto e : h->ev_pool) (void)hipEventDestroy(e);
    if (h->ev0) (void)hipEventDestroy(h->ev0);
    if (h->ev1) (void)hipEventDestroy(h->ev1);
    for (auto e : h->fork_events) (void)hipEventDestroy(e);
    if (h->aux) (void)hipStreamDestroy(h->aux);
    if (h->own_stream) (void)hipStreamDestroy(h->stream);
    delete h;
    return GMRF_OK;
}

gmrf_status gmrf_bt_set_batch(gmrf_handle* h, int64_t batch) {
    if (!h || batch < 1 || batch > 4096) return bad_shape("batch must be in [1, 4096]");
    if (batch != 1) GCHK(tw_refuse(h, "gmrf_bt_set_batch (batch > 1)"));
    if (batch != h->B) {
        HIPCHK(hipSetDevice(h->device));
        HIPCHK(hipStreamSynchronize(h->stream));
        destroy_graphs(h);
        h->B = batch;
        h->sel = 0;
        h->factored = false;
        release_shape_buffers(h);
        if (h->n > 0) (void)set_shape(h, h->n, h->N);
    }
    return GMRF_OK;
}

gmrf_status gmrf_bt_select_problem(gmrf_handle* h, int64_t p) {
    if (!h || p < 0 || p >= h->B) return bad_shape("problem index out of range");
    h->sel = p;
    return GMRF_OK;
}

gmrf_status gmrf_bt_set_profiling(gmrf_handle* h, int32_t level) {
    if (!h) return bad_shape("null handle");
    h->profiling = level;
    if (h->tw)
        for (gmrf_handle* s : {h->tw->top, h->tw->bot}) if (s) GCHK(gmrf_bt_set_profiling(s, level));
    if (level > 0 && h->events.empty()) h->gemm_shapes.clear();
    for (int i = 0; i < GMRF_KERNEL_CLASSES; ++i) { h->stats.kernel_ms[i] = h->stats.kernel_work[i] = 0; h->stats.kernel_launches[i] = 0; }
    return GMRF_OK;
}

gmrf_status gmrf_bt_set_eager(gmrf_handle* h, int32_t eager) {
    if (!h) return bad_shape("null handle");
    if (((eager & 2) != 0) != h->split_step) { destroy_graphs(h); h->split_step = (eager & 2) != 0; }
    if (((eager & 4) != 0) != h->sweep_no_gemm) { destroy_graphs(h); h->sweep_no_gemm = (eager & 4) != 0; }
    if (((eager & 8) != 0) != h->dense_g1) { destroy_graphs(h); h->dense_g1 = (eager & 8) != 0; }
    if (((eager & 16) != 0) != h->fork_graph) { destroy_graphs(h); h->fork_graph = (eager & 16) != 0; }
    h->no_staircase = (eager & 32) != 0;
    if (((eager & 128) != 0) != h->doubling_x) { destroy_graphs(h); h->doubling_x = (eager & 128) != 0; }
    if (((eager & 256) != 0) != h->no_lookahead) { destroy_graphs(h); h->no_lookahead = (eager & 256) != 0; }
    if (((eager & 4096) != 0) != h->no_xsplit) { destroy_graphs(h); h->no_xsplit = (eager & 4096) != 0; }
    if (((eager & 8192) != 0) != h->no_persist) { destroy_graphs(h); h->no_persist = (eager & 8192) != 0; }
    if (((eager & 32768) != 0) != h->no_persist_panels) { destroy_graphs(h); h->no_persist_panels = (eager & 32768) != 0; }
    if (((eager & 65536) != 0) != h->no_sweep_persist) { destroy_graphs(h); h->no_sweep_persist = (eager & 65536) != 0; }
    if (((eager & 131072) != 0) != h->no_scatter_fold) { destroy_graphs(h); h->no_scatter_fold = (eager & 131072) != 0; }
    h->eager = (eager & 1) != 0;
    h->eager_bits = eager;
    if (h->tw)
        for (gmrf_handle* s : {h->tw->top, h->tw->bot})
            if (s) {
                GCHK(gmrf_bt_set_eager(s, eager));
                if (h->tw->bot) s->no_sweep_persist = true;
            }
    return GMRF_OK;
}

gmrf_status gmrf_bt_synchronize(gmrf_handle* h) {
    if (!h) return bad_shape("null handle");
    HIPCHK(hipStreamSynchronize(h->stream));
    if (tw_on(h)) HIPCHK(hipStreamSynchronize(h->tw->bot->stream));
    return GMRF_OK;
}

gmrf_status gmrf_bt_stats(gmrf_handle* h, gmrf_stats* out) {
    if (!h || !out) return bad_shape("null pointer");
    if (tw_on(h)) {
        const gmrf_stats &a = h->tw->top->stats, &b = h->tw->bot->stats;
        *out = h->stats;
        out->persist_route = a.persist_route;
        out->persist_aborts = a.persist_aborts + b.persist_aborts;
        out->persist_cus = a.persist_cus + b.persist_cus;
        out->persist_refused = a.persist_refused | b.persist_refused;
        out->factor_bytes = a.factor_bytes + b.factor_bytes;
        return GMRF_OK;
    }
    h = tw_route(h);
    *out = h->stats;
    return GMRF_OK;
}

gmrf_status gmrf_bt_factor_csc(gmrf_handle* h, int64_t n, int64_t n_blocks, const int64_t* colptr,
                               const int64_t* rowval, const double* nzval, int32_t index_base,
                               int32_t* info) {
    if (!h) return bad_shape("null handle");
    HIPCHK(hipSetDevice(h->device));
    if (info) *info = 0;
    if (h->order == GMRF_ORDER_TWISTED) {
        GCHK(tw_analyze(h, n, n_blocks, colptr, rowval, index_base));
        return tw_numeric(h, nzval, info);
    }
    GCHK(analyze_csc(h, n, n_blocks, colptr, rowval, index_base));
    return numeric_factor(h, nzval, info);
}

gmrf_status gmrf_bt_factor_begin_csc(gmrf_handle* h, int64_t n, int64_t n_blocks, const int64_t* colptr,
                                     const int64_t* rowval, const double* nzval, int32_t index_base) {
    GCHK(tw_refuse(h, "gmrf_bt_factor_begin_csc"));
    if (!h) return bad_shape("null handle");
    HIPCHK(hipSetDevice(h->device));
    if (colptr) GCHK(analyze_csc(h, n, n_blocks, colptr, rowval, index_base));
    if (!h->analyzed) { g_last_error = "no sparsity pattern analysed"; return GMRF_ERR_NO_FACTOR; }
    GCHK(alloc_factor(h));
    if (h->c_dirty) {
        HIPCHK(hipMemsetAsync(h->d_C, 0, sizeof(double) * stride_pC(h) * h->B, h->stream));
        h->c_dirty = false;
    }
    persist_plan(h);
    GCHK(load_values(h, nzval));
    HIPCHK(hipMemsetAsync(h->d_info, 0, 4 * sizeof(int), h->stream));
    h->info_checked = 0; h->persist_launched = false; h->stats.persist_route = 0;
    h->factored = false;
    return GMRF_OK;
}

gmrf_status gmrf_bt_factor_step_async(gmrf_handle* h, int64_t i0, int64_t i1) {
    GCHK(tw_refuse(h, "gmrf_bt_factor_step_async"));
    if (!h) return bad_shape("null handle");
    if (i0 < 0 || i1 > h->N || i0 > i1) return bad_shape("bad block range");
    HIPCHK(hipSetDevice(h->device));
    GCHK(factor_blocks_range(h, i0, i1));
    if (h->persist_launched) GCHK(persist_check_range(h, i0, i1, nullptr));
    return GMRF_OK;
}

gmrf_status gmrf_bt_factor_end(gmrf_handle* h, int32_t* info) {
    GCHK(tw_refuse(h, "gmrf_bt_factor_end"));
    if (!h) return bad_shape("null handle");
    HIPCHK(hipSetDevice(h->device));
    gmrf_status s = factor_finish(h, info);
    if (h->profiling) prof_collect(h);
    return s;
}

gmrf_status gmrf_bt_refactor_values(gmrf_handle* h, const double* nzval, int32_t* info) {
    if (!h) return bad_shape("null handle");
    HIPCHK(hipSetDevice(h->device));
    if (info) *info = 0;
    if (h->order == GMRF_ORDER_TWISTED) return tw_numeric(h, nzval, info);
    return numeric_factor(h, nzval, info);
}

gmrf_status gmrf_bt_factor_blocks(gmrf_handle* h, int64_t n, int64_t n_blocks, const gmrf_sparse_block* diag,
                                  const gmrf_sparse_block* lower, int32_t index_base,
                                  int32_t compressed_by_column, int32_t* info) {
    GCHK(tw_refuse(h, "gmrf_bt_factor_blocks"));
    if (!h || !diag || (n_blocks > 1 && !lower)) return bad_shape("null pointer");
    HIPCHK(hipSetDevice(h->device));
    if (info) *info = 0;
    GCHK(set_shape(h, n, n_blocks));
    const int64_t bs = h->bs;
    std::vector<std::vector<HostEntry>> dg(n_blocks), lo(n_blocks);
    std::vector<double> vals;
    auto add_block = [&](const gmrf_sparse_block& b, std::vector<HostEntry>& dst, bool lower_tri_only) -> bool {
        for (int64_t o = 0; o < bs; ++o) {
            for (int64_t p = b.ptr[o] - index_base; p < b.ptr[o + 1] - index_base; ++p) {
                const int64_t in = b.idx[p] - index_base;
                if (in < 0 || in >= bs) return false;
                const int64_t r = compressed_by_column ? in : o, c = compressed_by_column ? o : in;
                if (lower_tri_only && r < c) continue;
                dst.push_back({((uint64_t)r << 32) | (uint64_t)c, (int64_t)vals.size()});
                vals.push_back(b.val[p]);
            }
        }
        return true;
    };
    for (int64_t i = 0; i < n_blocks; ++i) {
        if (!add_block(diag[i], dg[i], true)) return bad_shape("block index out of range");
        if (i > 0 && !add_block(lower[i - 1], lo[i], false)) return bad_shape("block index out of range");
    }
    GCHK(upload_entries(h, dg, lo, (int64_t)vals.size()));
    return numeric_factor(h, vals.data(), info);
}


gmrf_status gmrf_bt_storage_bytes(int64_t n, int64_t n_blocks, int64_t batch, int64_t* bytes_L, int64_t* bytes_C,
                                  int64_t* bytes_Linv) {
    if (n <= 0 || n_blocks <= 0 || n % n_blocks != 0 || batch < 1 || !bytes_L || !bytes_C || !bytes_Linv)
        return bad_shape("n must be a positive multiple of N_blocks, batch >= 1");
    const int64_t bs = n / n_blocks, bsp = 64 * next_pow2((bs + 63) / 64);
    const int64_t blk = bsp * bsp * (int64_t)sizeof(double) * batch;
    *bytes_L = blk * n_blocks; *bytes_Linv = blk * n_blocks; *bytes_C = blk * std::max<int64_t>(n_blocks - 1, 1);
    return GMRF_OK;
}

gmrf_status gmrf_bt_set_storage(gmrf_handle* h, int64_t n, int64_t n_blocks, int64_t batch, void* dev_L, void* dev_C,
                                void* dev_Linv) {
    GCHK(tw_refuse(h, "gmrf_bt_set_storage"));
    if (!h || !dev_C || !dev_Linv) return bad_shape("null pointer");
    if (batch != h->B) return bad_shape("storage batch differs from the handle's batch (gmrf_bt_set_batch first)");
    if (!dev_L && h->keep_l) return bad_shape("dev_L may be NULL only after gmrf_bt_set_keep_l(h, 0)");
    HIPCHK(hipSetDevice(h->device));
    GCHK(set_shape(h, n, n_blocks));
    HIPCHK(hipStreamSynchronize(h->stream));
    destroy_graphs(h);
    if (!h->external_storage) { free_dev(h->d_L); free_dev(h->d_C); free_dev(h->d_Linv); }
    else if (!h->keep_l) free_dev(h->d_L);
    free_dev(h->d_S); free_dev(h->d_B); free_dev(h->d_T); free_dev(h->d_W); free_dev(h->d_logdet);
    h->d_S = h->d_B = h->d_T = h->d_W = h->d_logdet = nullptr;
// ... 474 lines not shown
    } else {
        HIPCHK(hipStreamSynchronize(c->stream));
    }
    return GMRF_OK;
}

gmrf_status gmrf_bt_bcast_blocks_async(gmrf_handle* h, gmrf_comm* c, int32_t root, int64_t i0, int64_t i1, int32_t with_l) {
    GCHK(tw_refuse(h, "gmrf_bt_bcast_blocks_async"));
    if (!h || !c) return bad_shape("null pointer");
    if (!h->d_Linv || h->N <= 0) { g_last_error = "no factor storage"; return GMRF_ERR_NO_FACTOR; }
    if (i0 < 0 || i1 > h->N || i0 >= i1 || root < 0 || root >= c->world) return bad_shape("bad block range / root");
    if (with_l && !h->keep_l) return bad_shape("the L blocks are not kept on this handle");
    if (c->device != h->device) return bad_shape("communicator and handle live on different devices");
    HIPCHK(hipSetDevice(h->device));
    int64_t seg = 0;
    GCHK(gmrf_bt_packed_size(h, i0, i1, &seg));
    const size_t need = (size_t)seg * (size_t)h->B * sizeof(double);
    if (need > c->pack_cap) {
        HIPCHK(hipStreamSynchronize(c->stream));
        free_dev(c->d_pack); c->d_pack = nullptr; c->pack_cap = 0;
        HIPCHK(hipMalloc(&c->d_pack, need));
        c->pack_cap = need;
    }
    HIPCHK(hipEventRecord(c->ev_in, h->stream));
    HIPCHK(hipStreamWaitEvent(c->stream, c->ev_in, 0));
    if (c->rank == root) GCHK(pack_blocks_on(h, c->stream, i0, i1, c->d_pack, true));
    NCCLCHK(g_rccl.Broadcast(c->d_pack, c->d_pack, (size_t)seg * (size_t)h->B,  8, root, c->comm, c->stream));
    c->bytes_moved += (double)need;
    if (c->rank != root) GCHK(pack_blocks_on(h, c->stream, i0, i1, c->d_pack, false));
    if (with_l) {
        int64_t first = 0, cnt = 0, pstride = 0;
        GCHK(gmrf_bt_block_range(h, GMRF_BLOCK_L, i0, i1, &first, &cnt, &pstride));
        NCCLCHK(g_rccl.GroupStart());
        int rc = 0;
        for (int64_t p = 0; p < h->B && rc == 0; ++p) {
            double* ptr = h->d_L + p * pstride + first;
            rc = g_rccl.Broadcast(ptr, ptr, (size_t)cnt,  8, root, c->comm, c->stream);
        }
        const int rg = g_rccl.GroupEnd();
        if (rc != 0 || rg != 0) { g_last_error = std::string("ncclBroadcast: ") + g_rccl.GetErrorString(rc ? rc : rg); return GMRF_ERR_RCCL; }
        c->bytes_moved += (double)cnt * (double)h->B * sizeof(double);
    }
    return GMRF_OK;
}

gmrf_status gmrf_bt_allgather_blocks_async(gmrf_handle* src, gmrf_handle* dst, gmrf_comm* c, int64_t i0, int64_t i1) {
    GCHK(tw_refuse(src, "gmrf_bt_allgather_blocks_async"));
    GCHK(tw_refuse(dst, "gmrf_bt_allgather_blocks_async"));
    if (!src || !dst || !c) return bad_shape("null pointer");
    if (!src->d_Linv || !dst->d_Linv || src->N <= 0) { g_last_error = "no factor storage"; return GMRF_ERR_NO_FACTOR; }
    if (src->n != dst->n || src->N != dst->N || src->bsp != dst->bsp || src->cmin != dst->cmin || src->rmax != dst->rmax || src->kst != dst->kst)
        return bad_shape("the two handles differ in shape or coupling-block layout (gmrf_bt_adopt_layout the gathering handle with the factoring handle's record)");
    if (dst->B != src->B * (int64_t)c->world) return bad_shape("the gathering handle's batch must be world x the factoring handle's");
    if (i0 < 0 || i1 > src->N || i0 >= i1) return bad_shape("bad block range");
    if (c->device != src->device || c->device != dst->device) return bad_shape("communicator and handles live on different devices");
    HIPCHK(hipSetDevice(src->device));
    int64_t seg = 0;
    GCHK(gmrf_bt_packed_size(src, i0, i1, &seg));
    const size_t own = (size_t)seg * (size_t)src->B, all = own * (size_t)c->world;
    const size_t need = (own + all) * sizeof(double);
    if (need > c->pack_cap) {
        HIPCHK(hipStreamSynchronize(c->stream));
        free_dev(c->d_pack); c->d_pack = nullptr; c->pack_cap = 0;
        HIPCHK(hipMalloc(&c->d_pack, need));
        c->pack_cap = need;
    }
    HIPCHK(hipEventRecord(c->ev_in, src->stream));
    HIPCHK(hipStreamWaitEvent(c->stream, c->ev_in, 0));
    HIPCHK(hipEventRecord(c->ev_in, dst->stream));
    HIPCHK(hipStreamWaitEvent(c->stream, c->ev_in, 0));
    GCHK(pack_blocks_on(src, c->stream, i0, i1, c->d_pack, true));
    NCCLCHK(g_rccl.AllGather(c->d_pack, c->d_pack + own, own,  8, c->comm, c->stream));
    c->bytes_moved += (double)(all - own) * sizeof(double);
    GCHK(pack_blocks_on(dst, c->stream, i0, i1, c->d_pack + own, false));
    return GMRF_OK;
}

gmrf_status gmrf_comm_bytes(gmrf_comm* c, int32_t reset, double* bytes) {
    if (!c || !bytes) return bad_shape("null pointer");
    *bytes = c->bytes_moved;
    if (reset) c->bytes_moved = 0.0;
    return GMRF_OK;
}

gmrf_status gmrf_comm_wait(gmrf_handle* h, gmrf_comm* c) {
    if (!h || !c) return bad_shape("null pointer");
    HIPCHK(hipSetDevice(h->device));
    HIPCHK(hipEventRecord(c->ev_out, c->stream));
    HIPCHK(hipStreamWaitEvent(h->stream, c->ev_out, 0));
    return GMRF_OK;
}

gmrf_status gmrf_bt_solve(gmrf_handle* h, const double* b, double* y, int64_t k, int64_t ldb, int64_t ldy, int32_t mode) {
    h = tw_route(h);
    if (!h || !b || !y) return bad_shape("null pointer");
    if (!h->factored) { g_last_error = "solve before factor"; return GMRF_ERR_NO_FACTOR; }
    if (k <= 0 || ldb < h->n || ldy < h->n || mode < 0 || mode > 2) return bad_shape("bad k / ldb / ldy / mode");
    if (b == y && ldb != ldy) return bad_shape("in place (y == b) needs ldb == ldy");
    HIPCHK(hipSetDevice(h->device));
    if (tw_on(h)) return tw_solve(h, b, y, k, ldb, ldy, mode);
    if (h->B > 1 && k > KP_CHUNK) return bad_shape("with a batch of problems k is limited to 128 per call");
    const bool b_dev = is_device_ptr(b), y_dev = is_device_ptr(y);
    const int64_t nb = h->B;
    return sweep_guarded(h, {{b, cols_bytes(h->n, k * nb, ldb), y, cols_bytes(h->n, k * nb, ldy)}}, [&]() -> gmrf_status {
        h->stats.solve_ms = 0.0;
        for (int64_t c0 = 0; c0 < k; c0 += KP_CHUNK) {
            const int kc = (int)std::min<int64_t>(KP_CHUNK, k - c0);
            const int kp = pad_k(kc);
            GCHK(ensure_panels(h, kp));
            const double* d_b = nullptr;
            int64_t ld_b = 0;
            GCHK(cols_in(h, b + c0 * ldb, ldb, b_dev, kc, &d_b, &ld_b));
            GCHK(launch_pack(h, d_b, ld_b, kc, kp));
            HIPCHK(hipEventRecord(h->ev0, h->stream));
            GCHK(run_sweeps(h, mode, kp));
            HIPCHK(hipEventRecord(h->ev1, h->stream));
            GCHK(cols_out(h, (mode == GMRF_SOLVE_FULL) ? h->d_P : h->d_Y, kc, nullptr, y + c0 * ldy, ldy, y_dev));
            HIPCHK(hipStreamSynchronize(h->stream));
            float ms = 0.f;
            (void)hipEventElapsedTime(&ms, h->ev0, h->ev1);
            h->stats.solve_ms += ms;
            const int nsweeps = (mode == GMRF_SOLVE_FULL) ? 2 : 1;
            h->stats.sweep_ms = ms / nsweeps;
            h->stats.sweep_bytes = sweep_bytes(h, kc) * (double)nb;
            h->stats.sweep_bytes_streamed = (8.0 * ((double)h->N * 0.5 * (double)h->bsp * (double)(h->bsp + 1) +
                                                    (double)(h->N - 1) * h->c_streamed) + 16.0 * (double)h->n_pad * kc) * (double)nb;
            if (h->profiling) prof_collect(h);
        }
        return GMRF_OK;
    });
}

static gmrf_status stage_vector(gmrf_handle* h, const double* v, double** d_buf, const double** d_out) {
    if (!v) { *d_out = nullptr; return GMRF_OK; }
    if (is_device_ptr(v)) { *d_out = v; return GMRF_OK; }
    if (!*d_buf) HIPCHK(hipMalloc(d_buf, sizeof(double) * h->n * h->B));
    HIPCHK(hipMemcpyAsync(*d_buf, v, sizeof(double) * h->n * h->B, hipMemcpyHostToDevice, h->stream));
    *d_out = *d_buf;
    return GMRF_OK;
}

static gmrf_status sample_chunk(gmrf_handle* h, uint64_t seed, int64_t first_id, int kc, const double* z,
                                int64_t ldz, int64_t id_stride) {
    const int kp = pad_k(kc);
    GCHK(ensure_panels(h, kp));
    if (z) {
        const double* d_z = nullptr;
        int64_t ldd = 0;
        GCHK(cols_in(h, z, ldz, is_device_ptr(z), kc, &d_z, &ldd));
        GCHK(launch_pack(h, d_z, ldd, kc, kp));
    } else {
        const int64_t total = (int64_t)kp * h->n_pad;
        hipLaunchKernelGGL(fill_normals_panel, dim3((unsigned)((total + 255) / 256), (unsigned)h->B), dim3(256), 0,
                           h->stream, h->d_P, h->n_pad, (int)h->bs, (int)h->bsp, kc, kp, seed, first_id, id_stride);
        HIPCHK(hipGetLastError());
    }
    return run_sweeps(h, GMRF_SOLVE_BACKWARD, kp);
}

gmrf_status gmrf_bt_sample(gmrf_handle* h, uint64_t seed, int64_t first_id, int64_t k, const double* mean,
                           const double* z, double* out, int64_t ld) {
    h = tw_route(h);
    if (!h || !out) return bad_shape("null pointer");
    if (!h->factored) { g_last_error = "sample before factor"; return GMRF_ERR_NO_FACTOR; }
    if (k <= 0 || ld < h->n) return bad_shape("bad k / ld");
    if (h->B > 1 && k > KP_CHUNK) return bad_shape("with a batch of problems k is limited to 128 per call");
    HIPCHK(hipSetDevice(h->device));
    if (tw_on(h)) return tw_sample(h, seed, first_id, k, mean, z, out, ld);
    const double* d_mean = nullptr;
    GCHK(stage_vector(h, mean, &h->d_mean, &d_mean));
    const bool out_dev = is_device_ptr(out);
    const int64_t smp_bytes = cols_bytes(h->n, k * h->B, ld);
    GCHK(sweep_guarded(h, {{z, smp_bytes, out, smp_bytes}, {mean, h->n * h->B * (int64_t)sizeof(double), out, smp_bytes}},
                       [&]() -> gmrf_status {
        HIPCHK(hipEventRecord(h->ev0, h->stream));
        for (int64_t c0 = 0; c0 < k; c0 += KP_CHUNK) {
            const int kc = (int)std::min<int64_t>(KP_CHUNK, k - c0);
            GCHK(sample_chunk(h, seed, first_id + c0, kc, z ? z + c0 * ld : nullptr, ld, k));
            GCHK(cols_out(h, h->d_Y, kc, d_mean, out + c0 * ld, ld, out_dev));
            if (!out_dev) HIPCHK(hipStreamSynchronize(h->stream));
        }
        HIPCHK(hipEventRecord(h->ev1, h->stream));
        HIPCHK(hipStreamSynchronize(h->stream));
        return GMRF_OK;
    }));
    float ms = 0.f;
    (void)hipEventElapsedTime(&ms, h->ev0, h->ev1);
    h->stats.sample_ms = ms;
    if (h->profiling) prof_collect(h);
    return GMRF_OK;
}

static gmrf_status ensure_aux(gmrf_handle* h) {
    if (h->aux_distinct) return GMRF_OK;
    HIPCHK(hipStreamSynchronize(h->stream));
    if (h->aux) { (void)hipStreamSynchronize(h->aux); (void)hipStreamDestroy(h->aux); h->aux = nullptr; }
    const unsigned long long ticks = 100000ull;
    double one = 1e30;
    for (int r = 0; r < 2; ++r) one = std::min(one, spin_pair_ms(h->stream, nullptr, ticks));
    std::vector<hipStream_t> cand;
    for (int c = 0; c < 12 && !h->aux; ++c) {
        hipStream_t st = nullptr;
        HIPCHK(hipStreamCreateWithFlags(&st, hipStreamNonBlocking));
        hipLaunchKernelGGL(gmrf_spin_kernel, dim3(1), dim3(64), 0, st, 1ull);
        (void)hipStreamSynchronize(st);
        const double t = std::min(spin_pair_ms(h->stream, st, ticks), spin_pair_ms(h->stream, st, ticks));
        if (t < 1.5 * one) h->aux = st; else cand.push_back(st);
    }
    if (!h->aux && !cand.empty()) { h->aux = cand.back(); cand.pop_back(); }
    for (hipStream_t st : cand) (void)hipStreamDestroy(st);
    if (!h->aux) return bad_shape("internal: no second stream");
    h->aux_distinct = true;
    return GMRF_OK;
}

static gmrf_status posterior_beside(gmrf_handle* h, const double* b, uint64_t seed, int64_t first_id, int64_t k, double* mean,
                                    double* samples, int64_t ld) {
    const int kp = pad_k(k);
    GCHK(ensure_panels(h, 1));
    GCHK(sweep_persist_prepare(h, 1));
    const int64_t elems = (int64_t)kp * h->n_pad;
    if (!h->d_P2 || h->p2_elems < elems) {
        HIPCHK(hipStreamSynchronize(h->stream));
        free_dev(h->d_P2); free_dev(h->d_Y2); free_dev(h->d_T2);
        h->d_P2 = h->d_Y2 = h->d_T2 = nullptr; h->p2_elems = 0;
        HIPCHK(hipMalloc(&h->d_P2, sizeof(double) * (size_t)elems));
        HIPCHK(hipMalloc(&h->d_Y2, sizeof(double) * (size_t)elems));
        HIPCHK(hipMalloc(&h->d_T2, sizeof(double) * (size_t)elems));
        h->p2_elems = elems;
    }
    GCHK(ensure_aux(h));
    h->fork_next = 0;
    hipEvent_t ev_fork = nullptr, ev_join = nullptr;
    GCHK(fork_event(h, &ev_fork)); GCHK(fork_event(h, &ev_join));
    h->sweep_persist_launched = true;
    h->stats.sweep_persist = 1;
    h->stats.sweep_persist_launches += 3;
    HIPCHK(hipEventRecord(h->ev0, h->stream));
    HIPCHK(hipEventRecord(ev_fork, h->stream));
    HIPCHK(hipStreamWaitEvent(h->aux, ev_fork, 0));
    {
        const int64_t total = (int64_t)kp * h->n_pad;
        hipLaunchKernelGGL(fill_normals_panel, dim3((unsigned)((total + 255) / 256), 1), dim3(256), 0, h->aux, h->d_P2, h->n_pad,
                           (int)h->bs, (int)h->bsp, (int)k, kp, seed, first_id, k);
        HIPCHK(hipGetLastError());
        GCHK(launch_sweep_persist(h, true, kp, h->d_P2, h->d_Y2, h->aux, h->d_T2));
        HIPCHK(hipEventRecord(ev_join, h->aux));
    }
    GCHK(launch_pack(h, b, h->n, 1, 1));
    GCHK(launch_sweep_persist(h, false, 1, h->d_P, h->d_Y));
    GCHK(launch_sweep_persist(h, true, 1, h->d_Y, h->d_P));
    GCHK(launch_unpack(h, h->d_P, mean, h->n, 1, nullptr));
    HIPCHK(hipStreamWaitEvent(h->stream, ev_join, 0));
    GCHK(launch_unpack(h, h->d_Y2, samples, ld, (int)k, mean));
    HIPCHK(hipEventRecord(h->ev1, h->stream));
    HIPCHK(hipStreamSynchronize(h->stream));
    return GMRF_OK;
}

gmrf_status gmrf_bt_posterior(gmrf_handle* h, const double* b, uint64_t seed, int64_t first_id, int64_t k, double* mean,
                              double* samples, int64_t ld) {
    h = tw_route(h);
    if (!h || !b || !mean || !samples) return bad_shape("null pointer");
    if (!h->factored) { g_last_error = "posterior before factor"; return GMRF_ERR_NO_FACTOR; }
    if (k <= 0 || ld < h->n) return bad_shape("bad k / ld");
    HIPCHK(hipSetDevice(h->device));
    const bool dev_all = is_device_ptr(b) && is_device_ptr(mean) && is_device_ptr(samples);
    const int64_t vec_bytes = h->n * h->B * (int64_t)sizeof(double), smp_bytes = cols_bytes(h->n, k * h->B, ld);
    bool beside = false;
    GCHK(sweep_guarded(h, {{b, vec_bytes, mean, vec_bytes}, {b, vec_bytes, samples, smp_bytes}, {mean, vec_bytes, samples, smp_bytes}},
                       [&]() -> gmrf_status {
        beside = !tw_on(h) && h->B == 1 && k <= KP_CHUNK && k >= 2 && dev_all && !h->profiling && sweep_persist_ok(h, 1) &&
                 sweep_persist_ok(h, pad_k(k));
        return beside ? posterior_beside(h, b, seed, first_id, k, mean, samples, ld) : GMRF_OK;
    }, [&]() -> gmrf_status {
        HIPCHK(hipStreamSynchronize(h->aux));
        return GMRF_OK;
    }));
    if (!beside) {
        GCHK(gmrf_bt_solve(h, b, mean, 1, h->n, h->n, GMRF_SOLVE_FULL));
        return gmrf_bt_sample(h, seed, first_id, k, mean, nullptr, samples, ld);
    }
    float ms = 0.f;
    (void)hipEventElapsedTime(&ms, h->ev0, h->ev1);
    h->stats.solve_ms = ms;
    h->stats.sample_ms = 0.0;
    return GMRF_OK;
}

gmrf_status gmrf_bt_normals(gmrf_handle* h, uint64_t seed, int64_t first_id, int64_t k, double* z, int64_t ld) {
    if (!h || !z) return bad_shape("null pointer");
    if (h->n <= 0) return bad_shape("no shape set");
    if (k <= 0 || ld < h->n) return bad_shape("bad k / ld");
    if (h->B > 1 && k > KP_CHUNK) return bad_shape("with a batch of problems k is limited to 128 per call");
    HIPCHK(hipSetDevice(h->device));
    const bool z_dev = is_device_ptr(z);
    for (int64_t c0 = 0; c0 < k; c0 += KP_CHUNK) {
        const int kc = (int)std::min<int64_t>(KP_CHUNK, k - c0);
        const int kp = pad_k(kc);
        GCHK(ensure_panels(h, kp));
        const int64_t total = (int64_t)kp * h->n_pad;
        hipLaunchKernelGGL(fill_normals_panel, dim3((unsigned)((total + 255) / 256), (unsigned)h->B), dim3(256), 0,
                           h->stream, h->d_P, h->n_pad, (int)h->bs, (int)h->bsp, kc, kp, seed, first_id + c0, k);
        HIPCHK(hipGetLastError());
        GCHK(cols_out(h, h->d_P, kc, nullptr, z + c0 * ld, ld, z_dev));
        HIPCHK(hipStreamSynchronize(h->stream));
    }
    return GMRF_OK;
}

gmrf_status gmrf_bt_logdet(gmrf_handle* h, double* out) {
    h = tw_route(h);
    if (!h || !out) return bad_shape("null pointer");
    if (!h->factored) { g_last_error = "logdet before factor"; return GMRF_ERR_NO_FACTOR; }
    HIPCHK(hipSetDevice(h->device));
    if (tw_on(h)) return tw_logdet(h, out);
    if (h->keep_l && h->l_valid) {
        hipLaunchKernelGGL(logdet_blocks, dim3((unsigned)h->N, 1), dim3(256), 0, h->stream,
                           h->d_L + h->sel * stride_pL(h), blk_elems(h), h->bsp, (int)h->bs, h->d_logdet + h->sel * h->N,
                           (int64_t)0, (int64_t)0);
        HIPCHK(hipGetLastError());
    } else if (!h->logdet_valid) {
        g_last_error = "neither the L blocks nor the log-determinant parts of this factor are resident (adopted as raw buffers without L)";
        return GMRF_ERR_NO_FACTOR;
    }
    std::vector<double> part((size_t)h->N);
    HIPCHK(hipMemcpyAsync(part.data(), h->d_logdet + h->sel * h->N, sizeof(double) * h->N, hipMemcpyDeviceToHost, h->stream));
    HIPCHK(hipStreamSynchronize(h->stream));
    double s = 0.0;
    for (double v : part) s += v;
    *out = 2.0 * s;
    return GMRF_OK;
}

gmrf_status gmrf_csr_create(int32_t device, void* stream, int64_t n_rows, int64_t n_cols, const int64_t* rowptr,
                            const int64_t* colidx, const double* vals, int32_t index_base, int32_t values_f32,
                            gmrf_csr** out) {
    if (!out || !rowptr || !colidx || !vals || n_rows <= 0 || n_cols <= 0) return bad_shape("bad CSR arguments");
    int count = 0;
    if (hipGetDeviceCount(&count) != hipSuccess || count <= 0 || device < 0 || device >= count) {
        (void)hipGetLastError();
        g_last_error = "no HIP device visible";
        return GMRF_ERR_NO_DEVICE;
    }
    HIPCHK(hipSetDevice(device));
    const int64_t nnz = rowptr[n_rows] - index_base;
    if (nnz < 0 || rowptr[0] != index_base) return bad_shape("bad CSR row pointers");
    std::vector<int64_t> rp((size_t)n_rows + 1);
    for (int64_t i = 0; i <= n_rows; ++i) {
        rp[i] = rowptr[i] - index_base;
        if (i > 0 && rp[i] < rp[i - 1]) return bad_shape("CSR row pointers must be non-decreasing");
    }
    std::vector<int32_t> ci((size_t)nnz);
    for (int64_t p = 0; p < nnz; ++p) {
        const int64_t c = colidx[p] - index_base;
        if (c < 0 || c >= n_cols) return bad_shape("column index out of range");
        ci[p] = (int32_t)c;
    }
    gmrf_csr* m = new gmrf_csr();
    m->device = device;
    m->tiles_ok = true;
    for (int64_t r = 0; r < n_rows; r += SPMV_ROWS)
        if (rp[std::min(n_rows, r + SPMV_ROWS)] - rp[r] > SPMV_CAP) { m->tiles_ok = false; break; }
    m->tiles128_ok = true;
    for (int64_t r = 0; r < n_rows; r += 128)
        if (rp[std::min<int64_t>(n_rows, r + 128)] - rp[r] > 2 * SPMV_CAP) { m->tiles128_ok = false; break; }
#define CSRCHK(expr)                                                                          \
    do {                                                                                      \
        hipError_t _e = (expr);                                                               \
        if (_e != hipSuccess) {                                                               \
            g_last_error = std::string(#expr) + ": " + hipGetErrorString(_e);                 \
            (void)gmrf_csr_destroy(m);                                                        \
            return GMRF_ERR_HIP;                                                              \
        }                                                                                     \
    } while (0)
    if (stream) { m->stream = (hipStream_t)stream; } else { CSRCHK(hipStreamCreateWithFlags(&m->stream, hipStreamNonBlocking)); m->own_stream = true; }
    m->n_rows = n_rows; m->n_cols = n_cols; m->nnz = nnz;
    CSRCHK(hipMalloc(&m->d_rowptr, sizeof(int64_t) * (n_rows + 1)));
    CSRCHK(hipMalloc(&m->d_colidx, sizeof(int32_t) * std::max<int64_t>(nnz, 1)));
    CSRCHK(hipMemcpyAsync(m->d_rowptr, rp.data(), sizeof(int64_t) * (n_rows + 1), hipMemcpyHostToDevice, m->stream));
    CSRCHK(hipMemcpyAsync(m->d_colidx, ci.data(), sizeof(int32_t) * nnz, hipMemcpyHostToDevice, m->stream));
    CSRCHK(hipStreamSynchronize(m->stream));
    if (values_f32) {
        std::vector<float> vf((size_t)nnz);
        for (int64_t p = 0; p < nnz; ++p) vf[p] = (float)vals[p];
        CSRCHK(hipMalloc(&m->d_vals32, sizeof(float) * std::max<int64_t>(nnz, 1)));
        CSRCHK(hipMemcpyAsync(m->d_vals32, vf.data(), sizeof(float) * nnz, hipMemcpyHostToDevice, m->stream));
        CSRCHK(hipStreamSynchronize(m->stream));
    } else {
        CSRCHK(hipMalloc(&m->d_vals, sizeof(double) * std::max<int64_t>(nnz, 1)));
        CSRCHK(hipMemcpyAsync(m->d_vals, vals, sizeof(double) * nnz, hipMemcpyHostToDevice, m->stream));
        CSRCHK(hipStreamSynchronize(m->stream));
    }
    if (n_rows == n_cols) {
        CSRCHK(hipMalloc(&m->d_diag, sizeof(double) * n_rows));
        hipLaunchKernelGGL(csr_extract_diag, dim3((unsigned)((n_rows + 255) / 256)), dim3(256), 0, m->stream,
                           m->d_rowptr, m->d_colidx, m->d_vals, m->d_vals32, n_rows, m->d_diag);
        CSRCHK(hipGetLastError());
        CSRCHK(hipStreamSynchronize(m->stream));
    }
#undef CSRCHK
    *out = m;
    return GMRF_OK;
}

gmrf_status gmrf_csr_destroy(gmrf_csr* m) {
    if (!m) return GMRF_OK;
    (void)hipSetDevice(m->device);
    (void)hipStreamSynchronize(m->stream);
    free_dev(m->d_rowptr); free_dev(m->d_colidx); free_dev(m->d_vals); free_dev(m->d_vals32);
    free_dev(m->d_diag); free_dev(m->d_stage_x); free_dev(m->d_stage_y);
    free_dev(m->d_tile_uptr); free_dev(m->d_ucols); free_dev(m->d_lidx);
    if (m->own_stream) (void)hipStreamDestroy(m->stream);
    delete m;
    return GMRF_OK;
}

static gmrf_status spmm_device(const gmrf_csr* S, hipStream_t st, const double* d_X, int64_t ldx, double* d_Y,
                               int64_t ldy, int k, const double* vals_override = nullptr) {
    const double avg = (double)S->nnz / (double)S->n_rows;
    const int bl = 256;
    if (k == 1 && S->tiles_ok) {
        static const int rows_env = [] { const char* e = getenv("GMRF_SPMV_ROWS"); return e ? atoi(e) : SPMV_ROWS; }();
        const bool tall = rows_env == 128 && S->tiles128_ok;
        const int rows = tall ? 128 : SPMV_ROWS;
        static const int wg_cap = [] { const char* e = getenv("GMRF_SPMV_WGS"); return e ? atoi(e) : 256 * 8; }();
        const dim3 grid((unsigned)std::min<int64_t>((S->n_rows + rows - 1) / rows, wg_cap > 0 ? wg_cap : (1 << 30)));
#define GMRF_SPMV(VT, VP)                                                                                                   \
        do {                                                                                                                \
            if (tall) hipLaunchKernelGGL((csr_spmv_tiles<VT, 128>), grid, dim3(bl), 0, st, S->d_rowptr, S->d_colidx, VP, S->n_rows, d_X + r * ldx, d_Y + r * ldy); \
            else hipLaunchKernelGGL((csr_spmv_tiles<VT, SPMV_ROWS>), grid, dim3(bl), 0, st, S->d_rowptr, S->d_colidx, VP, S->n_rows, d_X + r * ldx, d_Y + r * ldy); \
        } while (0)
        for (int r = 0; r < k; ++r) {
            if (vals_override) GMRF_SPMV(double, vals_override);
            else if (S->d_vals32) GMRF_SPMV(float, S->d_vals32);
            else GMRF_SPMV(double, S->d_vals);
        }
#undef GMRF_SPMV
        HIPCHK(hipGetLastError());
        return GMRF_OK;
    }
    auto grid_for = [&](int G) { return dim3((unsigned)((S->n_rows * G + bl - 1) / bl)); };
#define SPMM_LAUNCH(VT, G, VP)                                                                               \
    hipLaunchKernelGGL((csr_spmm<VT, G>), grid_for(G), dim3(bl), 0, st, S->d_rowptr, S->d_colidx, VP,        \
                       S->n_rows, d_X, ldx, d_Y, ldy, k)
    if (vals_override) {
        if (avg > 40) SPMM_LAUNCH(double, 64, vals_override);
        else if (avg > 20) SPMM_LAUNCH(double, 32, vals_override);
        else if (avg > 10) SPMM_LAUNCH(double, 16, vals_override);
        else SPMM_LAUNCH(double, 8, vals_override);
    } else if (S->d_vals32) {
        if (avg > 40) SPMM_LAUNCH(float, 64, S->d_vals32);
        else if (avg > 20) SPMM_LAUNCH(float, 32, S->d_vals32);
        else if (avg > 10) SPMM_LAUNCH(float, 16, S->d_vals32);
        else SPMM_LAUNCH(float, 8, S->d_vals32);
    } else {
// ... 1432 lines not shown
        GCHK(tw_cols_out(h, mode == GMRF_SOLVE_FULL, kc, nullptr, y + c0 * ldy, ldy, y_dev));
        HIPCHK(hipStreamSynchronize(h->stream));
        float ms = 0.f;
        (void)hipEventElapsedTime(&ms, h->ev0, h->ev1);
        h->stats.solve_ms += ms;
        h->stats.sweep_ms = ms / ((mode == GMRF_SOLVE_FULL) ? 2 : 1);
        h->stats.sweep_bytes = sweep_bytes(h, kc);
    }
    return GMRF_OK;
}

static gmrf_status tw_sample_chunk(gmrf_handle* h, uint64_t seed, int64_t first_id, int kc, const double* z, int64_t ldz) {
    const int kp = pad_k(kc);
    GCHK(tw_panels(h, kp));
    const double* d_z = nullptr;
    int64_t ldd = 0;
    if (z) GCHK(cols_in(h, z, ldz, is_device_ptr(z), kc, &d_z, &ldd));
    GCHK(tw_fill(h, d_z, ldd, kc, kp, seed, first_id));
    return tw_sweeps(h, GMRF_SOLVE_BACKWARD, kp);
}

static gmrf_status tw_sample(gmrf_handle* h, uint64_t seed, int64_t first_id, int64_t k, const double* mean, const double* z,
                             double* out, int64_t ld) {
    const double* d_mean = nullptr;
    GCHK(stage_vector(h, mean, &h->d_mean, &d_mean));
    const bool out_dev = is_device_ptr(out);
    HIPCHK(hipEventRecord(h->ev0, h->stream));
    for (int64_t c0 = 0; c0 < k; c0 += KP_CHUNK) {
        const int kc = (int)std::min<int64_t>(KP_CHUNK, k - c0);
        GCHK(tw_sample_chunk(h, seed, first_id + c0, kc, z ? z + c0 * ld : nullptr, ld));
        GCHK(tw_cols_out(h, false, kc, d_mean, out + c0 * ld, ld, out_dev));
        if (!out_dev) HIPCHK(hipStreamSynchronize(h->stream));
    }
    HIPCHK(hipEventRecord(h->ev1, h->stream));
    HIPCHK(hipStreamSynchronize(h->stream));
    float ms = 0.f;
    (void)hipEventElapsedTime(&ms, h->ev0, h->ev1);
    h->stats.sample_ms = ms;
    return GMRF_OK;
}

static gmrf_status tw_var_exact(gmrf_handle* h, double* d_out) {
    TwistState* t = h->tw;
    gmrf_handle *top = t->top, *bot = t->bot;
    const int bsp = (int)t->bsp;
    const int64_t bstride = (int64_t)bsp * bsp;
    GCHK(ensure_full_inverse(top)); GCHK(ensure_full_inverse(bot));
    GCHK(tw_fork(h));
    {
        const double* Xm = top->d_Linv + t->m * bstride;
        const double* Xl = bot->d_Linv + (bot->N - 1) * bstride;
        GCHK(gemm(bot, true, true, bsp, bsp, bsp, 0, 0, 1.0, Xm, bsp, Xm, bsp, 0.0, t->d_Smm, bsp, 0, 0, 0));
        GCHK(gemm(bot, false, true, bsp, bsp, bsp, 0, 0, 1.0, t->d_Smm, bsp, t->d_HJ, bsp, 0.0, bot->d_W, bsp, 0, 0, 0));
        GCHK(gemm(bot, true, true, bsp, bsp, bsp, 0, 0, 1.0, t->d_HJ, bsp, bot->d_W, bsp, 0.0, bot->d_B, bsp, 0, 0, 0));
        hipLaunchKernelGGL(add_identity, dim3((unsigned)((bsp + 255) / 256)), dim3(256), 0, bot->stream, bot->d_B, (int64_t)bsp, bsp);
        HIPCHK(hipGetLastError());
        GCHK(gemm(bot, false, true, bsp, bsp, bsp, 0, 0, 1.0, bot->d_B, bsp, Xl, bsp, 0.0, bot->d_T, bsp, 0, 0, 0));
        GCHK(gemm(bot, true, true, bsp, bsp, bsp, 0, 0, 1.0, Xl, bsp, bot->d_T, bsp, 0.0, bot->d_S, bsp, 0, 0, 0));
        GCHK(var_exact(bot, t->d_var, true));
        const int64_t cnt = bot->N * t->bs;
        hipLaunchKernelGGL(tw_reverse, dim3((unsigned)((cnt + 255) / 256)), dim3(256), 0, bot->stream, t->d_var, d_out + (t->m + 1) * t->bs, cnt);
        HIPCHK(hipGetLastError());
    }
    GCHK(var_exact(top, d_out));
    return tw_join(h);
}

static gmrf_status tw_var_accumulate_dev(gmrf_handle* h, int method, int64_t first_id, int64_t k, uint64_t seed, const gmrf_csr* Q,
                                         double* d_acc) {
    TwistState* t = h->tw;
    if (!t->d_z) HIPCHK(hipMalloc(&t->d_z, sizeof(double) * (size_t)(64 * t->n)));
    for (int64_t c0 = 0; c0 < k; c0 += 64) {
        const int kc = (int)std::min<int64_t>(64, k - c0);
        GCHK(tw_sample_chunk(h, seed, first_id + c0, kc, nullptr, 0));
        GCHK(tw_cols_out(h, false, kc, nullptr, t->d_z, t->n, true));
        GCHK(var_chunk(h, method, 0, kc, Q, nullptr, Q ? Q->d_diag : nullptr, d_acc, t->d_z, t->n, t->n, t->n));
    }
    return GMRF_OK;
}

static gmrf_status tw_logdet(gmrf_handle* h, double* out) {
    double a = 0.0, b = 0.0;
    GCHK(gmrf_bt_logdet(h->tw->top, &a));
    GCHK(gmrf_bt_logdet(h->tw->bot, &b));
    *out = a + b;
    return GMRF_OK;
}

static gmrf_status tw_get_block(gmrf_handle* h, int32_t kind, int64_t i, double* out, int64_t ld) {
    TwistState* t = h->tw;
    const int64_t N = t->N, m = t->m, bs = t->bs, bsp = t->bsp;
    if (ld < bs) return bad_shape("ld < block_size");
    std::vector<double> tmp((size_t)(bs * bs)), res((size_t)(bs * bs));
    bool flip = false;
    if (kind == GMRF_BLOCK_L || kind == GMRF_BLOCK_LINV) {
        if (i < 0 || i >= N) return bad_shape("block index");
        if (i <= m) GCHK(gmrf_bt_get_block(t->top, kind, i, tmp.data(), bs));
        else { GCHK(gmrf_bt_get_block(t->bot, kind, N - 1 - i, tmp.data(), bs)); flip = true; }
    } else if (kind == GMRF_BLOCK_C) {
        if (i < 0 || i >= N - 1) return bad_shape("block index");
        if (i < m) GCHK(gmrf_bt_get_block(t->top, kind, i, tmp.data(), bs));
        else if (i > m) { GCHK(gmrf_bt_get_block(t->bot, kind, N - 2 - i, tmp.data(), bs)); flip = true; }
        else {
            std::vector<double> hj((size_t)(bsp * bsp));
            HIPCHK(hipMemcpyAsync(hj.data(), t->d_HJ, hj.size() * sizeof(double), hipMemcpyDeviceToHost, h->stream));
            HIPCHK(hipStreamSynchronize(h->stream));
            for (int64_t c = 0; c < bs; ++c)
                for (int64_t r = 0; r < bs; ++r) tmp[(size_t)(c * bs + r)] = hj[(size_t)(r * bsp + (bs - 1 - c))];
        }
    } else return bad_shape("bad block kind");
    for (int64_t c = 0; c < bs; ++c)
        for (int64_t r = 0; r < bs; ++r)
            res[(size_t)(c * bs + r)] = flip ? tmp[(size_t)((bs - 1 - c) * bs + (bs - 1 - r))] : tmp[(size_t)(c * bs + r)];
    HIPCHK(hipMemcpy2DAsync(out, ld * sizeof(double), res.data(), bs * sizeof(double), bs * sizeof(double), bs, hipMemcpyDefault, h->stream));
    HIPCHK(hipStreamSynchronize(h->stream));
    return GMRF_OK;
}

gmrf_status gmrf_bt_set_order(gmrf_handle* h, int32_t order, int64_t meet) {
    if (!h) return bad_shape("null handle");
    if (order != GMRF_ORDER_REFERENCE && order != GMRF_ORDER_TWISTED) return bad_shape("unknown elimination order");
    if (meet < -1) return bad_shape("twisted order: meet must be -1 (automatic) or a block index");
    if (order == GMRF_ORDER_TWISTED && h->B != 1) return bad_shape("the twisted order needs batch 1");
    HIPCHK(hipSetDevice(h->device));
    HIPCHK(hipStreamSynchronize(h->stream));
    tw_free(h);
    tw_drop_own_factor(h);
    h->order = order;
    h->meet_req = meet;
    return GMRF_OK;
}

gmrf_status gmrf_bt_get_order(gmrf_handle* h, int32_t* order, int64_t* meet) {
    if (!h || !order || !meet) return bad_shape("null pointer");
    *order = h->order;
    if (h->order == GMRF_ORDER_TWISTED) *meet = (h->tw && h->tw->m >= 0) ? h->tw->m : h->meet_req;
    else *meet = h->N > 0 ? h->N - 1 : -1;
    return GMRF_OK;
}

gmrf_status gmrf_bt_half_stats(gmrf_handle* h, int32_t half, gmrf_stats* out) {
    if (!h || !out) return bad_shape("null pointer");
    if (h->order != GMRF_ORDER_TWISTED || !h->tw || !h->tw->top) return bad_shape("gmrf_bt_half_stats: not a factored twisted handle");
    if (half != 0 && half != 1) return bad_shape("half must be 0 (top) or 1 (bottom)");
    if (half == 1 && !h->tw->bot) { memset(out, 0, sizeof(*out)); return GMRF_OK; }
    *out = (half == 0 ? h->tw->top : h->tw->bot)->stats;
    return GMRF_OK;
}

gmrf_status gmrf_test_gemm(int32_t device, int64_t M, int64_t N, int64_t K, int32_t transA, int32_t transB,
                           int32_t tri_flags, int32_t lower_only, double alpha, const double* A, int64_t lda,
                           const double* B, int64_t ldb, double beta, double* C, int64_t ldc) {
    if (M % 64 || N % 64 || K % 16 || (lda & 1) || (ldb & 1)) return bad_shape("gemm test sizes");
    HIPCHK(hipSetDevice(device));
    const int64_t a_rows = transA ? K : M, b_rows = transB ? N : K;
    double *dA, *dB, *dC;
    HIPCHK(hipMalloc(&dA, sizeof(double) * a_rows * lda));
    HIPCHK(hipMalloc(&dB, sizeof(double) * b_rows * ldb));
    HIPCHK(hipMalloc(&dC, sizeof(double) * M * ldc));
    HIPCHK(hipMemcpy(dA, A, sizeof(double) * a_rows * lda, hipMemcpyHostToDevice));
    HIPCHK(hipMemcpy(dB, B, sizeof(double) * b_rows * ldb, hipMemcpyHostToDevice));
    HIPCHK(hipMemcpy(dC, C, sizeof(double) * M * ldc, hipMemcpyHostToDevice));
    GemmArgs g;
    g.A = dA; g.B = dB; g.C = dC; g.lda = lda; g.ldb = ldb; g.ldc = ldc;
    g.strideA = g.strideB = g.strideC = 0;
    g.pA = g.pB = g.pC = 0; g.nb1 = 1;
    g.D = nullptr; g.ldd = 0; g.pD = 0;
    const bool force_big = (tri_flags & 2048) != 0, use_ll = (tri_flags & 4096) != 0;
    const int dma_shape = (tri_flags & 8192) ? 1 : ((tri_flags & 16384) ? 2 : ((tri_flags & 32768) ? 3 : 0));
    g.M = (int)M; g.N = (int)N; g.K = (int)K; g.tri = tri_flags & ~(2048 | 4096 | 8192 | 16384 | 32768); g.lower_only = lower_only;
    g.alpha = alpha; g.beta = beta;
    unsigned long long* dst = nullptr;
    HIPCHK(hipMalloc(&dst, 16));
    HIPCHK(hipMemset(dst, 0, 16));
    g.stamps = (force_big || use_ll || dma_shape) ? nullptr : dst;
    HIPCHK(gemm_init());
    HIPCHK(gemm_dma_init());
    const int saved = gemm_big_policy(), saved_ll = gemm_ll_policy(), saved_dma = gemm_dma_policy(), saved_force = gemm_dma_force();
    gemm_big_policy() = force_big ? 1 : 2;
    gemm_ll_policy() = use_ll ? 0 : 2;
    gemm_dma_policy() = dma_shape ? 2 : 0;
    gemm_dma_force() = dma_shape;
    hipError_t le = launch_gemm(nullptr, transA != 0, transB == 0, g, 1);
    gemm_big_policy() = saved; gemm_ll_policy() = saved_ll; gemm_dma_policy() = saved_dma; gemm_dma_force() = saved_force;
    HIPCHK(le);
    HIPCHK(hipDeviceSynchronize());
    HIPCHK(hipMemcpy(C, dC, sizeof(double) * M * ldc, hipMemcpyDeviceToHost));
    HIPCHK(hipMemcpy(g_tile_stamps, dst, 16, hipMemcpyDeviceToHost));
    hipFree(dst);
    hipFree(dA); hipFree(dB); hipFree(dC);
    return GMRF_OK;
}

gmrf_status gmrf_test_gemm_shapes(gmrf_handle* h, double* rows, int64_t cap_rows, int64_t* n_rows) {
    if (!h || !n_rows) return bad_shape("null argument");
    HIPCHK(hipStreamSynchronize(h->stream));
    prof_collect(h);
    *n_rows = (int64_t)h->gemm_shapes.size();
    for (int64_t i = 0; rows && i < std::min<int64_t>(cap_rows, *n_rows); ++i) {
        const auto& g = h->gemm_shapes[(size_t)i];
        for (int c = 0; c < 8; ++c) rows[i * 11 + c] = (double)g.key[c];
        rows[i * 11 + 8] = g.launches; rows[i * 11 + 9] = g.ms; rows[i * 11 + 10] = g.work;
    }
    return GMRF_OK;
}

struct ClockProbe { int device; hipStream_t st; unsigned long long* d; int n; };
gmrf_status gmrf_test_clock_probe_start(int32_t device, int32_t n, int32_t sleeps, void** probe) {
    if (!probe || n < 2 || n > 100000 || sleeps < 1 || sleeps > 64) return bad_shape("clock probe: 2 <= n <= 100000, 1 <= sleeps <= 64");
    HIPCHK(hipSetDevice(device));
    ClockProbe* p = new ClockProbe{device, nullptr, nullptr, n};
    auto drop = [&](hipError_t e) {
        if (p->d) (void)hipFree(p->d);
        if (p->st) (void)hipStreamDestroy(p->st);
        delete p;
        g_last_error = std::string("clock probe: ") + hipGetErrorString(e);
        return GMRF_ERR_HIP;
    };
    hipError_t e = hipStreamCreateWithFlags(&p->st, hipStreamNonBlocking);
    if (e == hipSuccess) e = hipMalloc(&p->d, sizeof(unsigned long long) * 2 * 8 * (size_t)n);
    if (e == hipSuccess) e = hipMemsetAsync(p->d, 0, sizeof(unsigned long long) * 2 * 8 * (size_t)n, p->st);
    if (e != hipSuccess) return drop(e);
    hipLaunchKernelGGL(clock_probe_kernel, dim3(8), dim3(64), 0, p->st, p->d, n, sleeps);
    if ((e = hipGetLastError()) != hipSuccess) return drop(e);
    *probe = p;
    return GMRF_OK;
}
gmrf_status gmrf_test_clock_probe_finish(void* probe, double* ghz, double* t_ms) {
    ClockProbe* p = static_cast<ClockProbe*>(probe);
    if (!p || !ghz) return bad_shape("null pointer");
    std::vector<unsigned long long> h((size_t)2 * 8 * p->n);
    hipError_t e = hipSetDevice(p->device);
    if (e == hipSuccess) e = hipStreamSynchronize(p->st);
    if (e == hipSuccess) e = hipMemcpy(h.data(), p->d, h.size() * sizeof(unsigned long long), hipMemcpyDeviceToHost);
    if (e != hipSuccess) {
        (void)hipFree(p->d); (void)hipStreamDestroy(p->st);
        delete p;
        g_last_error = std::string("clock probe: ") + hipGetErrorString(e);
        return GMRF_ERR_HIP;
    }
    for (int i = 0; i + 1 < p->n; ++i) {
        double v[8];
        for (int b = 0; b < 8; ++b) {
            const unsigned long long* a = &h[((size_t)b * p->n + i) * 2];
            const double dc = (double)(a[2] - a[0]), dr = (double)(a[3] - a[1]);
            v[b] = dr > 0 ? dc / dr * 0.1 : 0.0;
        }
        std::sort(v, v + 8);
        ghz[i] = 0.5 * (v[3] + v[4]);
        if (t_ms) t_ms[i] = (double)(h[(size_t)i * 2 + 1] - h[1]) * 1e-5;
    }
    (void)hipFree(p->d); (void)hipStreamDestroy(p->st);
    delete p;
    return GMRF_OK;
}

gmrf_status gmrf_test_gemm_rate(int32_t device, int64_t M, int64_t N, int64_t K, int32_t transB, int32_t tri_flags,
                                int32_t lower_only, int32_t batch, int32_t big, int32_t reps, double* ms_per_launch) {
    if (M % 64 || N % 64 || K % 16 || batch < 1 || reps < 1) return bad_shape("gemm rate sizes");
    HIPCHK(hipSetDevice(device));
    const int64_t ld = std::max(std::max(M, N), K);
    const int64_t pm = ld * ld;
    double *dA, *dB, *dC;
    HIPCHK(hipMalloc(&dA, sizeof(double) * pm * batch));
    HIPCHK(hipMalloc(&dB, sizeof(double) * pm * batch));
    HIPCHK(hipMalloc(&dC, sizeof(double) * pm * batch));
    const int64_t tot = pm * batch;
    hipLaunchKernelGGL(fill_normals_panel, dim3((unsigned)((tot + 255) / 256)), dim3(256), 0, nullptr, dA, tot, 1 << 30,
                       1 << 30, 1, 1, 1ull, 0, 0);
    hipLaunchKernelGGL(fill_normals_panel, dim3((unsigned)((tot + 255) / 256)), dim3(256), 0, nullptr, dB, tot, 1 << 30,
                       1 << 30, 1, 1, 2ull, 0, 0);
    HIPCHK(hipMemset(dC, 0, sizeof(double) * pm * batch));
    GemmArgs g;
    g.A = dA; g.B = dB; g.C = dC; g.lda = g.ldb = g.ldc = ld;
    g.strideA = g.strideB = g.strideC = 0;
    g.pA = g.pB = g.pC = pm; g.nb1 = 1;
    g.D = nullptr; g.ldd = 0; g.pD = 0;
    g.M = (int)M; g.N = (int)N; g.K = (int)K; g.tri = tri_flags; g.lower_only = lower_only;
    g.alpha = 1.0; g.beta = 0.0; g.stamps = nullptr;
    HIPCHK(gemm_init());
    HIPCHK(gemm_dma_init());
    const int saved = gemm_big_policy(), saved_dma = gemm_dma_policy(), saved_force = gemm_dma_force();
    gemm_big_policy() = big == 1 ? 1 : (big == 2 ? 0 : 2);
    gemm_dma_policy() = big >= 3 ? 2 : 0;
    gemm_dma_force() = (big >= 3 && big <= 5) ? big - 2 : 0;
    if (big == 6) gemm_big_policy() = 0;
    hipEvent_t e0, e1;
    HIPCHK(hipEventCreate(&e0)); HIPCHK(hipEventCreate(&e1));
    hipError_t le = hipSuccess;
    for (int r = 0; r < 3 && le == hipSuccess; ++r) le = launch_gemm(nullptr, false, transB == 0, g, batch);
    HIPCHK(hipEventRecord(e0, nullptr));
    for (int r = 0; r < reps && le == hipSuccess; ++r) le = launch_gemm(nullptr, false, transB == 0, g, batch);
    HIPCHK(hipEventRecord(e1, nullptr));
    gemm_big_policy() = saved; gemm_dma_policy() = saved_dma; gemm_dma_force() = saved_force;
    HIPCHK(le);
    HIPCHK(hipEventSynchronize(e1));
    float ms = 0.f;
    HIPCHK(hipEventElapsedTime(&ms, e0, e1));
    *ms_per_launch = ms / reps;
    hipEventDestroy(e0); hipEventDestroy(e1);
    hipFree(dA); hipFree(dB); hipFree(dC);
    return GMRF_OK;
}

gmrf_status gmrf_test_potrf_tile(int32_t device, double* tile64, double* inv64, int32_t* info) {
    HIPCHK(hipSetDevice(device));
    double *dS, *dL, *dX;
    int* dinfo;
    HIPCHK(hipMalloc(&dS, sizeof(double) * 4096));
    HIPCHK(hipMalloc(&dL, sizeof(double) * 4096));
    HIPCHK(hipMalloc(&dX, sizeof(double) * 4096));
    HIPCHK(hipMalloc(&dinfo, sizeof(int)));
    HIPCHK(hipMemset(dinfo, 0, sizeof(int)));
    HIPCHK(hipMemcpy(dS, tile64, sizeof(double) * 4096, hipMemcpyHostToDevice));
    auto kern = potrf_tile_kernel;
    const dim3 tpb(256);
    (void)hipFuncSetAttribute((const void*)kern, hipFuncAttributeMaxDynamicSharedMemorySize, (int)POTRF_TILE_LDS);
    unsigned long long* dstamps;
    HIPCHK(hipMalloc(&dstamps, 64 * sizeof(unsigned long long)));
    HIPCHK(hipMemset(dstamps, 0, 64 * sizeof(unsigned long long)));
    hipLaunchKernelGGL(kern, dim3(1), tpb, POTRF_TILE_LDS, nullptr, dS, dL, dX, dinfo, (unsigned long long*)nullptr);
    HIPCHK(hipDeviceSynchronize());
    {
        hipEvent_t e0, e1; HIPCHK(hipEventCreate(&e0)); HIPCHK(hipEventCreate(&e1));
        HIPCHK(hipEventRecord(e0, nullptr));
        for (int i = 0; i < 200; ++i)
            hipLaunchKernelGGL(kern, dim3(1), tpb, POTRF_TILE_LDS, nullptr, dS, dL, dX, dinfo, (unsigned long long*)nullptr);
        HIPCHK(hipEventRecord(e1, nullptr)); HIPCHK(hipEventSynchronize(e1));
        float ms = 0.f; HIPCHK(hipEventElapsedTime(&ms, e0, e1));
        g_tile_us = ms * 1e3 / 200.0;
        hipEventDestroy(e0); hipEventDestroy(e1);
    }
    hipLaunchKernelGGL(kern, dim3(1), tpb, POTRF_TILE_LDS, nullptr, dS, dL, dX, dinfo, dstamps);
    HIPCHK(hipDeviceSynchronize());
    HIPCHK(hipMemcpy(g_tile_stamps, dstamps, 64 * sizeof(unsigned long long), hipMemcpyDeviceToHost));
    hipFree(dstamps);
    HIPCHK(hipGetLastError());
    HIPCHK(hipDeviceSynchronize());
    HIPCHK(hipMemcpy(tile64, dL, sizeof(double) * 4096, hipMemcpyDeviceToHost));
    HIPCHK(hipMemcpy(inv64, dX, sizeof(double) * 4096, hipMemcpyDeviceToHost));
    int hi = 0;
    HIPCHK(hipMemcpy(&hi, dinfo, sizeof(int), hipMemcpyDeviceToHost));
    if (info) *info = hi;
    hipFree(dS); hipFree(dL); hipFree(dX); hipFree(dinfo);
    return GMRF_OK;
}

gmrf_status gmrf_test_tile_timing(double* out, int32_t n) {
    if (!out || n < 18) return bad_shape("need 18 outputs");
    out[0] = g_tile_us;
    for (int i = 0; i < 17; ++i) out[1 + i] = (double)(g_tile_stamps[i] - g_tile_stamps[15]);
    if (n >= 24) for (int i = 0; i < 3; ++i) out[18 + i] = (double)(g_tile_stamps[20 + i] - g_tile_stamps[15]);
    if (n >= 30) for (int i = 0; i < 6; ++i) out[24 + i] = (double)(g_tile_stamps[24 + i] - g_tile_stamps[24]);
    if (n >= 62) for (int i = 0; i < 8; ++i) out[54 + i] = g_tile_stamps[56 + i] ? (double)(g_tile_stamps[56 + i] - g_tile_stamps[15]) : -1.0;
    if (n >= 54) for (int i = 0; i < 24; ++i) out[30 + i] = g_tile_stamps[32 + i] ? (double)(g_tile_stamps[32 + i] - g_tile_stamps[15]) : -1.0;
    return GMRF_OK;
}

gmrf_status gmrf_test_persist_stamps(double* out, int32_t n) {
    if (!out || n < 1 || n > 128) return bad_shape("1 .. 128 outputs");
    for (int i = 0; i < n; ++i)
        out[i] = g_persist_stamps[i] ? (g_persist_stamps[i] < 64 ? (double)g_persist_stamps[i] : (double)(g_persist_stamps[i] - g_persist_stamps[0])) : -1.0;
    return GMRF_OK;
}

gmrf_status gmrf_test_persist_aborts(gmrf_handle* h, int32_t* n) {
    if (!h || !n) return bad_shape("null argument");
    *n = h->persist_aborts;
    return GMRF_OK;
}

gmrf_status gmrf_test_persist_budget(int32_t cus, int32_t n, const int32_t* demands, int32_t* granted) {
    if (n < 0 || (n > 0 && (!demands || !granted))) return bad_shape("null argument");
    std::map<const void*, int> claims;
    for (int i = 0; i < n; ++i) granted[i] = persist_budget_claim(claims, (const void*)(demands + i), demands[i], cus, 0) ? 1 : 0;
    return GMRF_OK;
}

gmrf_status gmrf_test_potrf_block(int32_t device, int64_t bs, double* S, double* Linv, int32_t* info) {
    if (bs % 64 || next_pow2(bs / 64) != bs / 64) return bad_shape("bs must be 64 * 2^p");
    gmrf_handle* h = nullptr;
    GCHK(gmrf_bt_create(device, nullptr, &h));
    h->N = 1; h->n = bs; h->bs = bs; h->bsp = bs; h->n_pad = bs; h->B = 1;
    gmrf_status s = set_layout_dense(h);
    if (s == GMRF_OK) s = alloc_factor(h);
    unsigned long long* dst = nullptr;
    if (s == GMRF_OK && hipMalloc(&dst, 128 * sizeof(unsigned long long)) == hipSuccess) {
        (void)hipMemset(dst, 0, 128 * sizeof(unsigned long long));
        h->dbg_stamps = dst;
    }
    if (s == GMRF_OK) {
        hipError_t e = hipMemcpyAsync(h->d_S, S, sizeof(double) * bs * bs, hipMemcpyHostToDevice, h->stream);
        persist_plan(h);
        if (e == hipSuccess) s = potrf_block(h, h->d_S, h->d_L, h->d_Linv, h->d_T, 1);
        if (s == GMRF_OK) {
            int hi = 0;
            (void)hipMemcpyAsync(&hi, h->d_info, sizeof(int), hipMemcpyDeviceToHost, h->stream);
            (void)hipMemcpyAsync(S, h->d_L, sizeof(double) * bs * bs, hipMemcpyDeviceToHost, h->stream);
            (void)hipMemcpyAsync(Linv, h->d_Linv, sizeof(double) * bs * bs, hipMemcpyDeviceToHost, h->stream);
            if (hipStreamSynchronize(h->stream) != hipSuccess) s = GMRF_ERR_HIP;
            if (info) *info = hi;
            if (dst) (void)hipMemcpy(g_tile_stamps + 24, dst, 6 * sizeof(unsigned long long), hipMemcpyDeviceToHost);
            if (dst) (void)hipMemcpy(g_persist_stamps, dst, 128 * sizeof(unsigned long long), hipMemcpyDeviceToHost);
        }
    }
    if (dst) (void)hipFree(dst);
    gmrf_bt_destroy(h);
    return s;
}

gmrf_status gmrf_test_mfma_f64_rate(int32_t device, double* tflops) {
    HIPCHK(hipSetDevice(device));
    double* d;
    HIPCHK(hipMalloc(&d, 64));
    hipEvent_t a, b;
    HIPCHK(hipEventCreate(&a)); HIPCHK(hipEventCreate(&b));
    const int iters = 20000, blocks = 256 * 2;
    hipLaunchKernelGGL(mfma_f64_rate_kernel, dim3(blocks), dim3(256), 0, nullptr, d, 100);
    HIPCHK(hipDeviceSynchronize());
    HIPCHK(hipEventRecord(a, nullptr));
    hipLaunchKernelGGL(mfma_f64_rate_kernel, dim3(blocks), dim3(256), 0, nullptr, d, iters);
    HIPCHK(hipEventRecord(b, nullptr));
    HIPCHK(hipEventSynchronize(b));
    float ms = 0.f;
// ... 123 lines not shown
```

### diffeqgmrfs.jl_amd/csrc/misc_kernels.hpp

```cpp
#pragma once
#include <hip/hip_runtime.h>
#include <stdint.h>

namespace gmrf {

__global__ void scatter_block(const uint64_t* __restrict__ keys, const double* __restrict__ vals,
                              int64_t first, int64_t count, double* __restrict__ dst, int64_t ld,
                              int64_t pvals, int64_t pdst, int add) {
    const int64_t i = (int64_t)blockIdx.x * blockDim.x + threadIdx.x;
    if (i >= count) return;
    const uint64_t key = keys[first + i];
    const int64_t r = (int64_t)(key >> 32), c = (int64_t)(key & 0xffffffffu);
    double* d = dst + (int64_t)blockIdx.y * pdst + r * ld + c;
    const double v = vals[(int64_t)blockIdx.y * pvals + first + i];
    *d = add ? *d + v : v;
}

__global__ void zero_rows(double* __restrict__ dst, int64_t count, int64_t pdst) {
    const int64_t i = ((int64_t)blockIdx.x * blockDim.x + threadIdx.x) * 2;
    if (i < count) *reinterpret_cast<v2d*>(dst + (int64_t)blockIdx.y * pdst + i) = (v2d){0.0, 0.0};
}

__global__ void pad_identity(double* __restrict__ dst, int64_t ld, int bs, int bsp, int64_t pdst) {
    const int i = bs + blockIdx.x * blockDim.x + threadIdx.x;
    if (i < bsp) dst[(int64_t)blockIdx.y * pdst + (int64_t)i * ld + i] = 1.0;
}

template <bool PACK>
__global__ __launch_bounds__(256) void linv_tiles_copy(double* __restrict__ X, int64_t ld, int64_t blk_stride,
                                                       int64_t pX, double* __restrict__ buf, int64_t pbuf, int ntri) {
    const int b = (int)blockIdx.x / ntri, tile = (int)blockIdx.x % ntri;
    int r = (int)((sqrtf(8.0f * (float)tile + 1.0f) - 1.0f) * 0.5f);
    while (r * (r + 1) / 2 > tile) --r;
    while ((r + 1) * (r + 2) / 2 <= tile) ++r;
    const int c = tile - r * (r + 1) / 2;
    double* x = X + (int64_t)blockIdx.y * pX + (int64_t)b * blk_stride + (int64_t)r * 64 * ld + (int64_t)c * 64;
    double* q = buf + (int64_t)blockIdx.y * pbuf + ((int64_t)b * ntri + tile) * 4096;
    const int t = threadIdx.x;
#pragma unroll
    for (int i = 0; i < 8; ++i) {
        const int e = (i * 256 + t) * 2, row = e >> 6, col = e & 63;
        if (PACK) *reinterpret_cast<v2d*>(q + e) = *reinterpret_cast<const v2d*>(x + (int64_t)row * ld + col);
        else *reinterpret_cast<v2d*>(x + (int64_t)row * ld + col) = *reinterpret_cast<const v2d*>(q + e);
    }
}

constexpr double PACK_TAG_MAGIC = 1196249670.0;
__global__ void pack_tag_write(double* __restrict__ buf, int64_t pbuf, double xsplit) {
    double* q = buf + (int64_t)threadIdx.x * pbuf;
    q[0] = xsplit; q[1] = PACK_TAG_MAGIC;
}
__global__ void pack_tag_read(const double* __restrict__ buf, int64_t pbuf, int nprob, int* __restrict__ seen) {
    int code = *seen;
    for (int p = 0; p < nprob; ++p) {
        const double* q = buf + (int64_t)p * pbuf;
        const double v = q[0];
        const int c = (q[1] == PACK_TAG_MAGIC && v >= 0.0 && v < 1.0e6 && v == (double)(int)v) ? (int)v + 1 : -1;
        code = (code == 0 || code == c) ? c : -1;
    }
    *seen = code;
}

__global__ void pack_panel(const double* __restrict__ src, int64_t ld, double* __restrict__ P,
                           int64_t n_pad, int bs, int bsp, int nblk, int k, int kp) {
    const int64_t idx = (int64_t)blockIdx.x * blockDim.x + threadIdx.x;
    const int64_t total = (int64_t)kp * n_pad;
    if (idx >= total) return;
    const int64_t r = idx / n_pad, j = idx % n_pad;
    const int64_t blk = j / bsp, off = j % bsp;
    double v = 0.0;
    if (r < k && off < bs) v = src[((int64_t)blockIdx.y * k + r) * ld + blk * bs + off];
    P[(int64_t)blockIdx.y * total + idx] = v;
}

__global__ void unpack_panel(const double* __restrict__ P, int64_t n_pad, double* __restrict__ dst,
                             int64_t ld, int bs, int bsp, int64_t n, int k, int kp,
                             const double* __restrict__ mean) {
    const int64_t idx = (int64_t)blockIdx.x * blockDim.x + threadIdx.x;
    if (idx >= n * (int64_t)k) return;
    const int64_t r = idx / n, j = idx % n;
    const int64_t blk = j / bs, off = j % bs;
    double v = P[(int64_t)blockIdx.y * kp * n_pad + r * n_pad + blk * bsp + off];
    if (mean) v += mean[(int64_t)blockIdx.y * n + j];
    dst[((int64_t)blockIdx.y * k + r) * ld + j] = v;
}

__device__ __host__ inline void philox4x32_10(uint32_t c[4], uint32_t k0, uint32_t k1) {
    for (int i = 0; i < 10; ++i) {
        const uint64_t p0 = (uint64_t)0xD2511F53u * c[0];
        const uint64_t p1 = (uint64_t)0xCD9E8D57u * c[2];
        const uint32_t n0 = (uint32_t)(p1 >> 32) ^ c[1] ^ k0;
        const uint32_t n1 = (uint32_t)p1;
        const uint32_t n2 = (uint32_t)(p0 >> 32) ^ c[3] ^ k1;
        const uint32_t n3 = (uint32_t)p0;
        c[0] = n0; c[1] = n1; c[2] = n2; c[3] = n3;
        k0 += 0x9E3779B9u; k1 += 0xBB67AE85u;
    }
}

__device__ __host__ inline double philox_normal(uint64_t seed, uint64_t dof, uint64_t sample) {
    uint32_t c[4] = {(uint32_t)dof, (uint32_t)(dof >> 32), (uint32_t)sample, (uint32_t)(sample >> 32)};
    philox4x32_10(c, (uint32_t)seed, (uint32_t)(seed >> 32));
    const uint64_t a = ((uint64_t)c[1] << 32) | c[0];
    const uint64_t b = ((uint64_t)c[3] << 32) | c[2];
    const double u1 = ((double)(a >> 11) + 0.5) * (1.0 / 9007199254740992.0);
    const double u2 = ((double)(b >> 11) + 0.5) * (1.0 / 9007199254740992.0);
    return sqrt(-2.0 * log(u1)) * cos(6.283185307179586476925 * u2);
}

__global__ void fill_normals_panel(double* __restrict__ P, int64_t n_pad, int bs, int bsp,
                                   int k, int kp, uint64_t seed, int64_t first_id, int64_t id_stride) {
    const int64_t idx = (int64_t)blockIdx.x * blockDim.x + threadIdx.x;
    if (idx >= (int64_t)kp * n_pad) return;
    const int64_t r = idx / n_pad, j = idx % n_pad;
    const int64_t blk = j / bsp, off = j % bsp;
    double v = 0.0;
    if (r < k && off < bs)
        v = philox_normal(seed, (uint64_t)(blk * bs + off), (uint64_t)(first_id + (int64_t)blockIdx.y * id_stride + r));
    P[(int64_t)blockIdx.y * kp * n_pad + idx] = v;
}

struct BxtArgs {
    const int* rowptr;
    const uint64_t* keys;
    const double* vals;
    int64_t n_entries;
    const double* X;
    double* C;
    int64_t ld, ldc, pX, pC;
    const int* kst;
    int cm, rm, bsp;
    int cw;
};

template <int KM>
__global__ __launch_bounds__(256) void spmm_bxt(BxtArgs a) {
    const int ncc = (a.bsp - a.cm) / a.cw, nrc = (a.rm + 255) / 256;
    const int nprob = (int)gridDim.x / (ncc * nrc);
    int cc, rc, prob;
    {
        const int groups = (nprob % 8 == 0) ? 8 : 1;
        const int xg = (int)blockIdx.x % groups, q = (int)blockIdx.x / groups;
        rc = q % nrc;
        cc = (q / nrc) % ncc;
        prob = xg + groups * (q / (nrc * ncc));
    }
    const int r = rc * 256 + (int)threadIdx.x;
    const int c0 = a.cm + cc * a.cw;
    const double* __restrict__ X = a.X + (int64_t)prob * a.pX;
    double* __restrict__ C = a.C + (int64_t)prob * a.pC;
    const double* __restrict__ vals = a.vals + (int64_t)prob * a.n_entries;
    int k0 = 0, len = 0;
    if (r < a.rm) { k0 = a.rowptr[r]; len = a.rowptr[r + 1] - k0; }
    int jt[KM];
    double vt[KM];
#pragma unroll
    for (int t = 0; t < KM; ++t) {
        const bool ok = t < len;
        jt[t] = ok ? (int)(a.keys[k0 + t] & 0xffffffffu) : 0;
        vt[t] = ok ? vals[k0 + t] : 0.0;
    }
    int lm = len;
#pragma unroll
    for (int off = 32; off > 0; off >>= 1) lm = max(lm, __shfl_xor(lm, off));
    lm = __builtin_amdgcn_readfirstlane(lm);
    __shared__ double ls[256 * 17];
    const int tid = (int)threadIdx.x;
    const int wr = tid >> 4, wc = tid & 15;
    const int rbase = rc * 256;
    const int cfirst = a.cm + (a.kst ? a.kst[rbase >> 6] : 0);
    for (int c = c0; c < c0 + a.cw; c += 16) {
        if (c + 16 <= cfirst) continue;
        const double* xr = X + (int64_t)c * a.ld;
        double acc[16];
#pragma unroll
        for (int u = 0; u < 16; ++u) acc[u] = 0.0;
#pragma unroll
        for (int t = 0; t < KM; ++t)
            if (t < lm) {
#pragma unroll
                for (int u = 0; u < 16; ++u) acc[u] = fma(vt[t], xr[(int64_t)u * a.ld + jt[t]], acc[u]);
            }
#pragma unroll
        for (int u = 0; u < 16; ++u) ls[tid * 17 + u] = acc[u];
        __syncthreads();
#pragma unroll 4
        for (int p = 0; p < 16; ++p) {
            const int rr = p * 16 + wr;
            if (rbase + rr < a.rm) C[(int64_t)(rbase + rr) * a.ldc + (c - a.cm) + wc] = ls[rr * 17 + wc];
        }
        __syncthreads();
    }
}

struct BxtTileArgs {
    const int* rowptr;
    const uint16_t* lidx;
    const double* vals;
    int64_t n_entries;
    const int* gtiles;
    int ng;
    const int* uptr;
    const int* ucols;
    const double* X;
    double* C;
    int64_t ld, ldc, pX, pC;
    const int* kst;
    int cm, rm, bsp;
    int nch;
    int ecap;
    int skip_dead;
    int nprob;
    double* zdst; int64_t zcount, zpdst; int zwgs;
    const int* srowptr;
    const uint64_t* skeys;
    const double* svals;
};

constexpr int BXT_UCAP = 256;
constexpr int BXT_GT = 3;

inline size_t bxt_tile_lds_bytes(int ecap) {
    return (size_t)BXT_UCAP * 16 * 8 + (size_t)ecap * 10 + BXT_GT * 128 * 8 + (size_t)BXT_UCAP * 4 + (size_t)BXT_GT * (2 * 64 + 2) * 4 + 16;
}

__global__ __launch_bounds__(256, 3) void spmm_bxt_tiles(BxtTileArgs a) {
    extern __shared__ __attribute__((aligned(16))) double smem[];
    double* xs = smem;
    double* vs = xs + BXT_UCAP * 16;
    uint16_t* ls = reinterpret_cast<uint16_t*>(vs + a.ecap + BXT_GT * 128);
    int* uc = reinterpret_cast<int*>(ls + a.ecap);
    int* rp = uc + BXT_UCAP;
    int* pp = rp + BXT_GT * 65;
    const int t = threadIdx.x;
    const int W = a.bsp - a.cm;
    const int ncg = (W / 16 + a.nch - 1) / a.nch;
    const int nprob = a.nprob;
    if ((int)blockIdx.x >= ncg * a.ng * nprob) {
        const int zi = (int)blockIdx.x - ncg * a.ng * nprob;
        const int p = zi / a.zwgs, z = zi % a.zwgs;
        double* d = a.zdst + (int64_t)p * a.zpdst;
        if (a.srowptr) {
            const int rpw = (a.bsp + a.zwgs - 1) / a.zwgs;
            const int ra = min(a.bsp, z * rpw), rb = min(a.bsp, ra + rpw);
            for (int r = ra; r < rb; ++r) {
                const int cend = min(a.bsp, ((r >> 6) + 1) * 64);
                for (int c = 2 * t; c < cend; c += 512) *reinterpret_cast<v2d*>(d + (int64_t)r * a.ld + c) = (v2d){0.0, 0.0};
            }
            asm volatile("s_waitcnt vmcnt(0)" ::: "memory");
            __syncthreads();
            const int e0 = a.srowptr[ra], e1 = a.srowptr[rb];
            for (int e = e0 + t; e < e1; e += 256) {
                const uint64_t key = a.skeys[e];
                d[(int64_t)(key >> 32) * a.ld + (int64_t)(key & 0xffffffffu)] = a.svals[e];
            }
            return;
        }
        const int64_t per = ((a.zcount / 2 + a.zwgs - 1) / a.zwgs) * 2;
        const int64_t lo = (int64_t)z * per, hi = min(a.zcount, lo + per);
        for (int64_t i = lo + 2 * t; i < hi; i += 512) *reinterpret_cast<v2d*>(d + i) = (v2d){0.0, 0.0};
        return;
    }
    int cg, g, prob;
    {
        const int groups = (nprob % 8 == 0) ? 8 : 1;
        const int xg = (int)blockIdx.x % groups, q = (int)blockIdx.x / groups;
        g = q % a.ng;
        cg = (q / a.ng) % ncg;
        prob = xg + groups * (q / (a.ng * ncg));
    }
    int tile[BXT_GT], cst[BXT_GT], e0s[BXT_GT];
    int nT = 0, cmin_g = 1 << 30;
// ... 787 lines not shown
```

### diffeqgmrfs.jl_amd/posterior.py

```python
from __future__ import annotations

from typing import List, Optional, Tuple

import numpy as np


def shard_range(total: int, world: int, rank: int) -> Tuple[int, int]:
    base, rem = divmod(total, world)
    first = rank * base + min(rank, rem)
    return first, base + (1 if rank < rem else 0)


def block_groups(n_blocks: int, group: int) -> List[Tuple[int, int]]:
    return [(i, min(n_blocks, i + group)) for i in range(0, n_blocks, group)]


class HipEngine:

    def __init__(self, pkg, workload, device_index: int = 0, batch: int = 1, values=None, rhs=None,
                 keep_l: bool = True, transport: str = "torch", comm=None):
        import torch
        self.torch = torch
        self.pkg = pkg
        self.w = workload
        self.batch = batch
        self.dev = torch.device("cuda", device_index)
        torch.cuda.set_device(self.dev)
        self.stream = torch.cuda.current_stream(self.dev)
        if self.stream.cuda_stream == 0:
            self.stream = torch.cuda.Stream(self.dev)
            torch.cuda.set_stream(self.stream)
        self.F = pkg.TridiagonalCholeskyFactor(device=device_index, stream=self.stream.cuda_stream, batch=batch)
        if not keep_l:
            self.F.set_keep_l(False)
        self.keep_l = keep_l
        self.transport, self.comm = transport, comm
        if transport == "cabi" and comm is None:
            raise ValueError('transport "cabi" needs an api.Comm')
        if values is None:
            values = np.tile(np.ascontiguousarray(workload.Q.data), (batch, 1))
        if rhs is None:
            rhs = np.tile(np.ascontiguousarray(workload.rhs), (batch, 1))
        self.values_host = np.ascontiguousarray(values, dtype=np.float64).reshape(batch, -1)
        self.nz = torch.from_numpy(self.values_host).to(self.dev)
        self.rhs = torch.from_numpy(np.ascontiguousarray(rhs, dtype=np.float64).reshape(batch, 1, -1)).to(self.dev)
        self._stage = {}
        self.bytes_moved = 0
        self._pending = []

    def prepare(self, is_root: bool, shared_storage: bool, dist=None):
        if not shared_storage:
            self.F.factor(self.w.Q, self.w.n_blocks, values=self.values_host)
            return
        if is_root:
            self.F.factor(self.w.Q, self.w.n_blocks, values=self.values_host)
            layout = self.F.get_layout()
        else:
            layout = None
        if self.transport == "cabi":
            cnt = np.array([0 if layout is None else layout.size], dtype=np.int64)
            self.comm.bcast_host(cnt, 0)
            if layout is None:
                layout = np.zeros(int(cnt[0]), dtype=np.int64)
            self.comm.bcast_host(layout, 0)
        else:
            box = [layout]
            dist.broadcast_object_list(box, src=0)
            layout = np.asarray(box[0], dtype=np.int64)
        if not is_root:
            self.F.adopt_layout(self.w.n, self.w.n_blocks, layout)

    def factor(self):
        self.F.refactor(self.nz)

    def factor_range_async(self, i0: int, i1: int, first: bool):
        if first:
            self.F.factor_begin_values(self.nz)
        self.F.factor_step_async(i0, i1)

    def factor_end(self):
        self.F.factor_end()

    def adopt_commit(self):
        self.F.adopt_commit(False)

    def _staging(self, i0: int, i1: int):
        key = (i0, i1)
        if key not in self._stage:
            t = self.torch
            self._stage[key] = t.empty((self.batch, self.F.packed_size(i0, i1)), dtype=t.float64, device=self.dev)
        return self._stage[key]

    def share_range(self, dist, i0: int, i1: int, is_root: bool = True):
        if self.transport == "cabi":
            self.comm.bcast_blocks_async(self.F, i0, i1, root=0, with_l=False)
            return
        buf = self._staging(i0, i1)
        if is_root:
            self.F.pack_blocks_async(i0, i1, buf)
        self._pending.append((dist.broadcast(buf, src=0, async_op=True), i0, i1, buf))
        self.bytes_moved += buf.numel() * 8

    def share_finish(self, is_root: bool = True):
        if self.transport == "cabi":
            self.comm.wait(self.F)
            return
        for hnd, i0, i1, buf in self._pending:
            hnd.wait()
            if not is_root:
                self.F.unpack_blocks_async(i0, i1, buf)
        self._pending = []

    def transport_bytes(self, reset: bool = False) -> float:
        if self.transport == "cabi":
            return self.comm.bytes_moved(reset)
        v = self.bytes_moved
        if reset:
            self.bytes_moved = 0
        return float(v)

    def mean(self):
        return self.F.solve_batch(self.rhs)[:, 0, :]

    def sample(self, k: int, mean, seed: int, first_id: int, keep: bool = True):
        if self.batch == 1 or k <= 128:
            return self.F.sample_batch(k, mean=mean, seed=seed, first_id=first_id, like=self.rhs)
        outs = []
        for c0 in range(0, k, 128):
            kc = min(128, k - c0)
            x = self.F.sample_batch(kc, mean=mean, seed=seed, first_id=first_id + c0 * self.batch, like=self.rhs)
            outs = outs + [x] if keep else [x]
        return self.torch.cat(outs, dim=1) if keep else outs[0]

    def synchronize(self):
        self.torch.cuda.synchronize(self.dev)


class HipGatherEngine(HipEngine):

    def __init__(self, pkg, workload, device_index: int, batch_total: int, world: int, rank: int, values_all, rhs_all,
                 keep_l: bool = False, transport: str = "torch", comm=None):
        if batch_total % world:
            raise ValueError("the shared batch must be a multiple of the number of ranks")
        b = batch_total // world
        values_all = np.ascontiguousarray(values_all, dtype=np.float64).reshape(batch_total, -1)
        rhs_all = np.ascontiguousarray(rhs_all, dtype=np.float64).reshape(batch_total, -1)
        super().__init__(pkg, workload, device_index=device_index, batch=b, values=values_all[rank * b:(rank + 1) * b],
                         rhs=rhs_all[rank * b:(rank + 1) * b], keep_l=keep_l, transport=transport, comm=comm)
        t = self.torch
        self.share_batch, self.batch, self.world, self.rank = b, batch_total, world, rank
        self.F_all = pkg.TridiagonalCholeskyFactor(device=device_index, stream=self.stream.cuda_stream, batch=batch_total)
        self.F_all.set_keep_l(False)
        self.rhs = t.from_numpy(rhs_all.reshape(batch_total, 1, -1)).to(self.dev)
        self._own, self._all = {}, {}

    def prepare(self, is_root: bool, shared_storage: bool, dist=None):
        self.F.factor(self.w.Q, self.w.n_blocks, values=self.values_host)
        self.F_all.adopt_layout(self.w.n, self.w.n_blocks, self.F.get_layout())

    def adopt_commit(self):
        self.F_all.adopt_commit(False)

    def share_range(self, dist, i0: int, i1: int, is_root: bool = True):
        if self.transport == "cabi":
            self.comm.allgather_blocks_async(self.F, self.F_all, i0, i1)
            return
        t = self.torch
        key = (i0, i1)
        if key not in self._own:
            seg = self.F.packed_size(i0, i1)
            self._own[key] = t.empty((self.share_batch, seg), dtype=t.float64, device=self.dev)
            self._all[key] = t.empty((self.batch, seg), dtype=t.float64, device=self.dev)
        own, allb = self._own[key], self._all[key]
        self.F.pack_blocks_async(i0, i1, own)
        if dist.get_backend() == "nccl":
            self._pending.append((dist.all_gather_into_tensor(allb, own, async_op=True), i0, i1, allb))
        else:
            b = self.share_batch
            allb[self.rank * b:(self.rank + 1) * b].copy_(own)
            hs = [dist.broadcast(allb[r * b:(r + 1) * b], src=r, async_op=True) for r in range(self.world)]
            for h in hs[:-1]:
                self._pending.append((h, None, None, None))
            self._pending.append((hs[-1], i0, i1, allb))
        self.bytes_moved += (allb.numel() - own.numel()) * 8

    def share_finish(self, is_root: bool = True):
        if self.transport == "cabi":
            self.comm.wait(self.F_all)
            return
        for hnd, i0, i1, allb in self._pending:
            hnd.wait()
            if allb is not None:
                self.F_all.unpack_blocks_async(i0, i1, allb)
        self._pending = []

    def mean(self):
        return self.F_all.solve_batch(self.rhs)[:, 0, :]

    def sample(self, k: int, mean, seed: int, first_id: int, keep: bool = True):
        if k <= 128:
            return self.F_all.sample_batch(k, mean=mean, seed=seed, first_id=first_id, like=self.rhs)
        outs = []
        for c0 in range(0, k, 128):
            kc = min(128, k - c0)
            x = self.F_all.sample_batch(kc, mean=mean, seed=seed, first_id=first_id + c0 * self.batch, like=self.rhs)
            outs = outs + [x] if keep else [x]
        return self.torch.cat(outs, dim=1) if keep else outs[0]


class ShardedPosterior:

    def __init__(self, engine, dist=None, rank: int = 0, world: int = 1, k_samples: int = 64,
                 seed: int = 0x5EED, group: int = 8, replicate_factor: bool = False, force_shared: bool = False,
                 keep_samples: bool = True, timing: bool = False, share: str = "broadcast"):
        self.e, self.dist, self.rank, self.world = engine, dist, rank, world
        self.k, self.seed, self.group = k_samples, seed, group
        self.replicate = replicate_factor or (world == 1 and not force_shared)
        self.groups = block_groups(engine.w.n_blocks, group)
        self.keep_samples = keep_samples
        self.share = share
        if share not in ("broadcast", "allgather"):
            raise ValueError(share)
        if share == "allgather":
            self.replicate = False
        self.timing = timing and hasattr(engine, "torch")
        self._ev = None

    def prepare(self):
        self.e.prepare(is_root=(self.rank == 0), shared_storage=not self.replicate, dist=self.dist)
        if self.dist is not None and self.world > 1:
            self.dist.barrier()

    def _mark(self, i: int):
        if self.timing:
            self._ev[i].record(self.e.torch.cuda.current_stream(self.e.dev))

    def _factor_and_share(self):
        if self.timing and self._ev is None:
            self._ev = [self.e.torch.cuda.Event(enable_timing=True) for _ in range(4)]
        self._mark(0)
        if self.replicate:
            self.e.factor()
            self._mark(1); self._mark(2)
            return
        if self.share == "allgather":
            for gi, (i0, i1) in enumerate(self.groups):
                self.e.factor_range_async(i0, i1, first=(gi == 0))
                self.e.share_range(self.dist, i0, i1, True)
            self._mark(1)
            self.e.factor_end()
            self.e.share_finish(True)
            self._mark(2)
            self.e.adopt_commit()
            return
        root = self.rank == 0
        for gi, (i0, i1) in enumerate(self.groups):
            if root:
                self.e.factor_range_async(i0, i1, first=(gi == 0))
            self.e.share_range(self.dist, i0, i1, root)
        self._mark(1)
        self.e.share_finish(root)
        self._mark(2)
        if root:
            self.e.factor_end()
        else:
            self.e.adopt_commit()

    def step(self, step_index: int = 0):
        self._factor_and_share()
        mu = self.e.mean()
        nb = getattr(self.e, "batch", 1)
        first = (step_index * self.world + self.rank) * self.k * nb
        X = self.e.sample(self.k, mu, self.seed, first) if self.keep_samples else self.e.sample(self.k, mu, self.seed, first, keep=False)
        self._mark(3)
        return mu, X

    def phase_ms(self):
        if not self.timing or self._ev is None:
            return None
        e = self._ev
        return {"factor_ms": e[0].elapsed_time(e[1]), "transfer_wait_ms": e[1].elapsed_time(e[2]),
                "mean_and_samples_ms": e[2].elapsed_time(e[3])}

    def solves_per_step(self) -> int:
        nb = getattr(self.e, "batch", 1)
        if self.replicate:
            return self.world * nb * (1 + self.k)
        return nb * (1 + self.k * self.world)
```

Measured before the change: 48930 solves/s.

## Fuse posterior mean solve into sample backward sweep via tail-row GEMM

```diff
diff --git a/diffeqgmrfs.jl_amd/api.py b/diffeqgmrfs.jl_amd/api.py
--- a/diffeqgmrfs.jl_amd/api.py
+++ b/diffeqgmrfs.jl_amd/api.py
@@ -629,6 +629,15 @@
                                                 self.N))
         return mview, sview
 
+    def posterior_batch(self, b, k: int, seed: int = 0x5EED, first_id: int = 0):
+        import torch
+        B, n = self.batch, self.N
+        b = b.reshape(B, n).contiguous()
+        mean = torch.empty((B, n), dtype=torch.float64, device=b.device)
+        out = torch.empty((B, k, n), dtype=torch.float64, device=b.device)
+        _cabi.check(self._lib.gmrf_bt_posterior(self._h, _cabi.ptr(b), seed, first_id, k, _cabi.ptr(mean), _cabi.ptr(out), n))
+        return mean, out
+
     def marginal_var(self, method: str = "exact", k: int = 50, seed: int = 0x5EED, Q: Optional[CsrMatrix] = None,
                      q_values=None, out=None):
         m = {"exact": _cabi.VAR_EXACT, "rbmc": _cabi.VAR_RBMC, "mc": _cabi.VAR_MC}[method]
diff --git a/diffeqgmrfs.jl_amd/csrc/gemm_f64_dma.hpp b/diffeqgmrfs.jl_amd/csrc/gemm_f64_dma.hpp
--- a/diffeqgmrfs.jl_amd/csrc/gemm_f64_dma.hpp
+++ b/diffeqgmrfs.jl_amd/csrc/gemm_f64_dma.hpp
@@ -52,16 +52,18 @@
     z = xg + groups * zq;
 }
 
-template <int BM, int BN, bool B_N, int STAGES, bool A_T = false>
+template <int BM, int BN, bool B_N, int STAGES, bool A_T = false, bool TAIL = false>
 __global__ __launch_bounds__(256, (BM + BN > 128) ? 3 : 4) void gemm_f64_dma(GemmArgs g) {
     constexpr int BK = DMA_BK;
     constexpr int MI = BM / 32, NJ = BN / 32;
     constexpr int NA = BM / 32, NB = BN / 32;
-    constexpr int A_ST = BM * BK, B_ST = BN * BK, ST = A_ST + B_ST;
+    constexpr int A_ST = BM * BK, B_ST = BN * BK, T_ST = TAIL ? BK : 0, ST = A_ST + B_ST + T_ST;
     static_assert(NJ % 2 == 0 || !B_N, "the [k][n] image pairs neighbouring column tiles");
     static_assert(MI % 2 == 0 || !A_T, "the [k][m] image pairs neighbouring row tiles");
+    static_assert(!TAIL || (BM == 64 && BN == 64 && B_N && !A_T), "the tail row: 64 x 64 tiles, B stored [k][n]");
     int bm, bn, z;
     gemm_dma_tile_order<BM, BN>(g, bm, bn, z);
+    const bool tail = TAIL && bm == g.M / BM - 1;
     const int m0 = bm * BM, n0 = bn * BN;
     if (g.lower_only == 2 && n0 > m0 + BM - 1) return;
     const int zi = z % g.nb1, zp = z / g.nb1;
@@ -113,12 +115,16 @@
             offb[i] = (uint32_t)(((int64_t)(n0 + row) * g.ldb + 2 * ch) * 8);
         }
     }
+    const double* arow = A + (int64_t)g.M * g.lda;
     auto issue = [&](int kt, int stage) {
         const int k0 = kb + kt * BK;
         const char* abase = reinterpret_cast<const char*>(A_T ? A + (int64_t)k0 * g.lda : A + k0);
         const char* bbase = reinterpret_cast<const char*>(B_N ? B + (int64_t)k0 * g.ldb : B + k0);
         double* as = gsm + stage * ST;
         double* bs = as + A_ST;
+        if constexpr (TAIL)
+            if (tail && w == 0 && lane < 8)
+                __builtin_amdgcn_global_load_lds(GMRF_GLB_PTR(arow + k0 + 2 * lane), GMRF_LDS_PTR(bs + B_ST), 16, 0, 0);
 #pragma unroll
         for (int i = 0; i < NA; ++i) {
             asm volatile("" : "+v"(offa[i]));
@@ -136,6 +142,8 @@
     for (int i = 0; i < MI; ++i)
 #pragma unroll
         for (int j = 0; j < NJ; ++j) acc[i][j] = (v4d){0.0, 0.0, 0.0, 0.0};
+    v2d tacc = (v2d){0.0, 0.0};
+    const int tkg = w >> 1;
 
     int fa[MI], fb[NJ];
 #pragma unroll
@@ -181,6 +189,9 @@
                 for (int j = 0; j < NJ; ++j)
                     b[kg][j] = *reinterpret_cast<const v2d*>(sm + fb[j] + (B_N ? kg * 8 * BN : ((kg * 8) ^ sb2[j])));
             }
+            v2d ta = (v2d){0.0, 0.0};
+            if constexpr (TAIL)
+                if (tail) ta = *reinterpret_cast<const v2d*>(sm + A_ST + B_ST + tkg * 8 + 2 * lq);
             __builtin_amdgcn_sched_barrier(0);
             if (GMRF_DMA_READS_FIRST && kt + DEPTH < nkt) issue(kt + DEPTH, (kt + DEPTH) % STAGES);
             __builtin_amdgcn_sched_barrier(0);
@@ -200,6 +211,13 @@
                             else bv = p ? b[kg][j].y : b[kg][j].x;
                             acc[i][j] = __builtin_amdgcn_mfma_f64_16x16x4f64(av, bv, acc[i][j], 0, 0, 0);
                         }
+            if constexpr (TAIL) {
+                if (tail) {
+                    const v2d b0 = tkg ? b[1][0] : b[0][0], b1 = tkg ? b[1][1] : b[0][1];
+                    tacc.x = fma(ta.x, b0.x, tacc.x); tacc.x = fma(ta.y, b1.x, tacc.x);
+                    tacc.y = fma(ta.x, b0.y, tacc.y); tacc.y = fma(ta.y, b1.y, tacc.y);
+                }
+            }
             __builtin_amdgcn_sched_barrier(0);
         } else if (GMRF_DMA_READS_FIRST && kt + DEPTH < nkt) issue(kt + DEPTH, (kt + DEPTH) % STAGES);
     }
@@ -251,6 +269,21 @@
                     if (beta != 0.0) v += beta * d[i][r][j];
                     C[orow(i, r) * g.ldc + n0 + wn + j * 16 + li] = v;
                 }
+    }
+    if constexpr (TAIL) {
+        if (tail) {
+            __syncthreads();
+            *reinterpret_cast<v2d*>(gsm + (tkg * 4 + lq) * BN + wn + 2 * li) = tacc;
+            __syncthreads();
+            if (w == 0) {
+                double s = 0.0;
+#pragma unroll
+                for (int q = 0; q < 8; ++q) s += gsm[q * BN + lane];
+                double v = alpha * s;
+                if (beta != 0.0) v += beta * Dm[(int64_t)g.M * ldd + n0 + lane];
+                C[(int64_t)g.M * g.ldc + n0 + lane] = v;
+            }
+        }
     }
 }
 
@@ -302,6 +335,28 @@
     GMRF_DMA_ATTR(64, 128, false, 2) GMRF_DMA_ATTR(64, 128, true, 2) GMRF_DMA_ATTR(64, 128, false, 3) GMRF_DMA_ATTR(64, 128, true, 3)
 #undef GMRF_DMA_ATTR
     return e;
+}
+
+inline bool gemm_tail_ok(bool a_t, bool b_n, const GemmArgs& g, int batch) {
+    if (a_t || !b_n || g.lower_only || gemm_uses_ll(g, batch) || gemm_dma_shape(false, g, batch) != 1) return false;
+    return (int64_t)(g.M + 1) * g.ldc * 8 < ((int64_t)1 << 32) && (!g.D || (int64_t)(g.M + 1) * g.ldd * 8 < ((int64_t)1 << 32));
+}
+inline bool gemm_try_dma_tail(hipStream_t st, bool a_t, bool b_n, const GemmArgs& g, int batch, hipEvent_t ev_start, hipEvent_t ev_stop,
+                              hipError_t* err) {
+    if (!gemm_tail_ok(a_t, b_n, g, batch)) return false;
+    GemmArgs gs = g;
+    gs.lower_only = 0;
+    const dim3 grid((unsigned)((int64_t)(g.N / 64) * (g.M / 64) * batch)), block(256);
+    const size_t lds = (size_t)gemm_dma_stages() * (64 + 64 + DMA_BK) * DMA_BK * sizeof(double);
+    if (gemm_dma_stages() == 3) {
+        if (ev_start) hipExtLaunchKernelGGL((gemm_f64_dma<64, 64, true, 3, false, true>), grid, block, lds, st, ev_start, ev_stop, 0, gs);
+        else hipLaunchKernelGGL((gemm_f64_dma<64, 64, true, 3, false, true>), grid, block, lds, st, gs);
+    } else {
+        if (ev_start) hipExtLaunchKernelGGL((gemm_f64_dma<64, 64, true, 2, false, true>), grid, block, lds, st, ev_start, ev_stop, 0, gs);
+        else hipLaunchKernelGGL((gemm_f64_dma<64, 64, true, 2, false, true>), grid, block, lds, st, gs);
+    }
+    *err = hipGetLastError();
+    return true;
 }
 
 inline bool gemm_try_dma(hipStream_t st, bool a_t, bool b_n, const GemmArgs& g, int batch, hipEvent_t ev_start, hipEvent_t ev_stop,
diff --git a/diffeqgmrfs.jl_amd/csrc/gmrf_hip.hip b/diffeqgmrfs.jl_amd/csrc/gmrf_hip.hip
--- a/diffeqgmrfs.jl_amd/csrc/gmrf_hip.hip
+++ b/diffeqgmrfs.jl_amd/csrc/gmrf_hip.hip
@@ -180,6 +180,9 @@
     bool eager = false;
     bool split_step = false;
     bool sweep_no_gemm = false;
+    bool no_fused_posterior = false;
+    bool tail_probe = false;
+    bool tail_refused = false;
     unsigned long long* dbg_stamps = nullptr;
     bool fork_graph = false;
     bool no_staircase = false;
@@ -316,7 +319,7 @@
                         double beta, double* C, int64_t ldc, int64_t pA, int64_t pB, int64_t pC,
                         int batch = 1, int64_t sA = 0, int64_t sB = 0, int64_t sC = 0, const double* D = nullptr,
                         int64_t ldd = 0, int64_t pD = 0, int pclass = 0, double pwork = -1.0,
-                        const int* kb_m = nullptr, const int* kb_n = nullptr, const int* ke_n = nullptr) {
+                        const int* kb_m = nullptr, const int* kb_n = nullptr, const int* ke_n = nullptr, bool tail = false) {
     GemmArgs g;
     g.kb_m = kb_m; g.kb_n = kb_n; g.ke_n = ke_n;
     g.D = D; g.ldd = ldd; g.pD = pD;
@@ -329,6 +332,36 @@
     double flops = 2.0 * M * N * (double)K * batch * (double)h->B;
     if (lower_only) flops *= 0.5 * (1.0 + 64.0 / std::max(M, 64));
     if (tri) flops *= 0.5 * (1.0 + 64.0 / std::max(K, 64));
+    if (tail) {
+        if (!gemm_tail_ok(a_t, b_n, g, batch * (int)h->B)) {
+            h->tail_refused = true;
+            return h->tail_probe ? GMRF_OK : bad_shape("internal: a product of the fused sweep does not qualify for the tail-row GEMM");
+        }
+        if (h->tail_probe) return GMRF_OK;
+        flops *= (M + 1.0) / M;
+        if (pwork >= 0.0) pwork *= (M + 1.0) / M;
+        pclass = b_n ? 15 : 14;
+        hipError_t e = hipSuccess;
+        if (h->profiling > 0) {
+            EvPair p;
+            p.kind = pclass; p.work = pwork >= 0.0 ? pwork : flops;
+            p.a = ev_get(h); p.b = ev_get(h);
+            const int64_t key[8] = {pclass, M + 1, N, K, tri, lower_only, batch * h->B, (kb_m || kb_n || ke_n) ? 1 : 0};
+            for (size_t i = 0; i < h->gemm_shapes.size() && p.shape < 0; ++i)
+                if (!memcmp(h->gemm_shapes[i].key, key, sizeof(key))) p.shape = (int)i;
+            if (p.shape < 0) {
+                GemmShapeStat st; memcpy(st.key, key, sizeof(key));
+                h->gemm_shapes.push_back(st); p.shape = (int)h->gemm_shapes.size() - 1;
+            }
+            (void)gemm_try_dma_tail(h->gemm_stream ? h->gemm_stream : h->stream, a_t, b_n, g, batch * (int)h->B, p.a, p.b, &e);
+            HIPCHK(e);
+            h->events.push_back(p);
+            return GMRF_OK;
+        }
+        (void)gemm_try_dma_tail(h->gemm_stream ? h->gemm_stream : h->stream, a_t, b_n, g, batch * (int)h->B, nullptr, nullptr, &e);
+        HIPCHK(e);
+        return GMRF_OK;
+    }
     if (gemm_uses_big(a_t, g, batch * (int)h->B)) { pclass = b_n ? 7 : 6; pwork = -1.0; }
     else if (pclass == 0) {
         if (gemm_uses_ll(g, batch * (int)h->B)) pclass = 13;
@@ -1544,8 +1577,8 @@
     return body();
 }
 
-static gmrf_status sweep_launches(gmrf_handle* h, bool backward, int kp, double* Pin, double* Yout) {
-    if (sweep_persist_ok(h, kp)) return launch_sweep_persist(h, backward, kp, Pin, Yout);
+static gmrf_status sweep_launches(gmrf_handle* h, bool backward, int kp, double* Pin, double* Yout, bool tail = false) {
+    if (!tail && sweep_persist_ok(h, kp)) return launch_sweep_persist(h, backward, kp, Pin, Yout);
     const int bsp = (int)h->bsp;
     const int64_t ld = bsp, bstride = (int64_t)bsp * bsp, npad = h->n_pad;
     const int64_t N = h->N;
@@ -1553,7 +1586,7 @@
     s.ld = ld;
     const int nprob = (int)h->B;
     s.narrow = (nprob < 8 && bsp >= 512 && bsp <= SWEEP_PERSIST_XMAX) ? 1 : 0;
-    const int64_t pPanel = (int64_t)kp * npad;
+    const int64_t pPanel = (int64_t)(kp + (tail ? 1 : 0)) * npad;
     const int64_t pX = stride_pX(h), pCm = stride_pC(h);
     const int64_t ldc = c_ld(h), cstride = c_blk(h);
     const int cm = (int)h->cmin, rm = (int)h->rmax, wc = bsp - cm;
@@ -1561,6 +1594,7 @@
     const double blk_work_c = ((kp == 1) ? 8.0 * h->c_streamed : 2.0 * h->c_streamed * kp) * nprob;
     const double blk_work_t = ((kp == 1) ? 4.0 * bsp * (double)(bsp + 1) : 1.0 * bsp * (double)(bsp + 1) * kp) * nprob;
     const bool via_gemm = (kp % 64 == 0) && !h->sweep_no_gemm && (int64_t)nprob * (bsp / 64) * (kp / 64) >= 128;
+    if (tail && (!via_gemm || !backward)) return bad_shape("internal: the tail row needs the backward sweep on the GEMM");
     for (int64_t step = 0; step < N; ++step) {
         const int64_t i = backward ? (N - 1 - step) : step;
         double* rhs = Pin + i * bsp;
@@ -1574,7 +1608,7 @@
             if (via_gemm) {
                 GCHK(gemm(h, false, backward, kp, rows, kdim, 0, 0, -1.0, xin, npad, Cs, ldc, 1.0, out, npad, pPanel, pCm,
                           pPanel, 1, 0, 0, 0, nullptr, 0, 0, 0, 2.0 * h->c_streamed * kp * nprob,
-                          nullptr, backward ? nullptr : h->d_kst, backward ? h->d_mend : nullptr));
+                          nullptr, backward ? nullptr : h->d_kst, backward ? h->d_mend : nullptr, tail));
             } else {
                 s.Mat = Cs; s.ld = ldc; s.Xin = xin; s.ldx = npad; s.Bin = out; s.ldb = npad; s.Out = out; s.ldo = npad;
                 s.rows = rows; s.kdim = kdim; s.sub = 1;
@@ -1593,16 +1627,18 @@
             for (int part = 0; part < 3; ++part) {
                 const int which = backward ? 2 - part : part;
                 if (via_gemm) {
+                    constexpr int64_t z0 = 0;
                     if (which == 0)
                         GCHK(gemm(h, false, backward, kp, p, p, backward ? TRI_B_LOWER : TRI_B_UPPER, 0, 1.0, rhs, npad, X, ld, 0.0, yout, npad,
-                                  pPanel, pX, pPanel));
+                                  pPanel, pX, pPanel, 1, z0, z0, z0, nullptr, z0, z0, 0, -1.0, nullptr, nullptr, nullptr, tail));
                     else if (which == 2)
                         GCHK(gemm(h, false, backward, kp, q, q, backward ? TRI_B_LOWER : TRI_B_UPPER, 0, 1.0, rhs + p, npad, Xbb, ld, 0.0,
-                                  yout + p, npad, pPanel, pX, pPanel));
+                                  yout + p, npad, pPanel, pX, pPanel, 1, z0, z0, z0, nullptr, z0, z0, 0, -1.0, nullptr, nullptr, nullptr, tail));
                     else if (!backward)
                         GCHK(gemm(h, false, false, kp, q, p, 0, 0, -1.0, yout, npad, Lba, ld, 1.0, rhs + p, npad, pPanel, pX, pPanel));
                     else
-                        GCHK(gemm(h, false, true, kp, p, q, 0, 0, -1.0, yout + p, npad, Lba, ld, 1.0, rhs, npad, pPanel, pX, pPanel));
+                        GCHK(gemm(h, false, true, kp, p, q, 0, 0, -1.0, yout + p, npad, Lba, ld, 1.0, rhs, npad, pPanel, pX, pPanel,
+                                  1, z0, z0, z0, nullptr, z0, z0, 0, -1.0, nullptr, nullptr, nullptr, tail));
                 } else {
                     s.ld = ld; s.ldx = npad; s.ldo = npad; s.pMat = pX; s.pXin = pPanel; s.pOut = pPanel; s.kst = nullptr; s.mend = nullptr;
                     if (which == 0) { s.Mat = X; s.Xin = rhs; s.Bin = nullptr; s.ldb = 0; s.Out = yout; s.rows = p; s.kdim = p; s.sub = 0; s.pBin = 0; }
@@ -1616,7 +1652,7 @@
             }
         } else if (via_gemm) {
             GCHK(gemm(h, false, backward, kp, bsp, bsp, backward ? TRI_B_LOWER : TRI_B_UPPER, 0, 1.0, rhs, npad, X, ld, 0.0,
-                      yout, npad, pPanel, pX, pPanel, 1, 0, 0, 0, nullptr, 0, 0, 0, -1.0));
+                      yout, npad, pPanel, pX, pPanel, 1, 0, 0, 0, nullptr, 0, 0, 0, -1.0, nullptr, nullptr, nullptr, tail));
         } else {
             s.Mat = X; s.ld = ld; s.Xin = rhs; s.ldx = npad; s.Bin = nullptr; s.ldb = 0; s.Out = yout; s.ldo = npad;
             s.rows = bsp; s.kdim = bsp; s.sub = 0;
@@ -1629,16 +1665,17 @@
     return GMRF_OK;
 }
 
-constexpr int SWEEP_BACKWARD_YP = 3;
+constexpr int SWEEP_BACKWARD_YP = 3, SWEEP_BACKWARD_TAIL = 4;
 static gmrf_status run_sweeps(gmrf_handle* h, int mode, int kp) {
     auto body = [&]() -> gmrf_status {
         if (mode == GMRF_SOLVE_FORWARD) return sweep_launches(h, false, kp, h->d_P, h->d_Y);
+        if (mode == SWEEP_BACKWARD_TAIL) return sweep_launches(h, true, kp, h->d_P, h->d_Y, true);
         if (mode == SWEEP_BACKWARD_YP) return sweep_launches(h, true, kp, h->d_Y, h->d_P);
         if (mode == GMRF_SOLVE_BACKWARD) return sweep_launches(h, true, kp, h->d_P, h->d_Y);
         GCHK(sweep_launches(h, false, kp, h->d_P, h->d_Y));
         return sweep_launches(h, true, kp, h->d_Y, h->d_P);
     };
-    const bool persistent = sweep_persist_ok(h, kp);
+    const bool persistent = mode != SWEEP_BACKWARD_TAIL && sweep_persist_ok(h, kp);
     if (persistent) {
         GCHK(sweep_persist_prepare(h, kp));
         h->sweep_persist_launched = true;
@@ -1829,6 +1866,7 @@
     if (((eager & 32768) != 0) != h->no_persist_panels) { destroy_graphs(h); h->no_persist_panels = (eager & 32768) != 0; }
     if (((eager & 65536) != 0) != h->no_sweep_persist) { destroy_graphs(h); h->no_sweep_persist = (eager & 65536) != 0; }
     if (((eager & 131072) != 0) != h->no_scatter_fold) { destroy_graphs(h); h->no_scatter_fold = (eager & 131072) != 0; }
+    h->no_fused_posterior = (eager & 262144) != 0;
     h->eager = (eager & 1) != 0;
     h->eager_bits = eager;
     if (h->tw)
@@ -2609,7 +2647,7 @@
     } else {
         const int64_t total = (int64_t)kp * h->n_pad;
         hipLaunchKernelGGL(fill_normals_panel, dim3((unsigned)((total + 255) / 256), (unsigned)h->B), dim3(256), 0,
-                           h->stream, h->d_P, h->n_pad, (int)h->bs, (int)h->bsp, kc, kp, seed, first_id, id_stride);
+                           h->stream, h->d_P, h->n_pad, (int)h->bs, (int)h->bsp, kc, kp, seed, first_id, id_stride, nullptr, (int64_t)0);
         HIPCHK(hipGetLastError());
     }
     return run_sweeps(h, GMRF_SOLVE_BACKWARD, kp);
@@ -2699,7 +2737,7 @@
     {
         const int64_t total = (int64_t)kp * h->n_pad;
         hipLaunchKernelGGL(fill_normals_panel, dim3((unsigned)((total + 255) / 256), 1), dim3(256), 0, h->aux, h->d_P2, h->n_pad,
-                           (int)h->bs, (int)h->bsp, (int)k, kp, seed, first_id, k);
+                           (int)h->bs, (int)h->bsp, (int)k, kp, seed, first_id, k, nullptr, (int64_t)0);
         HIPCHK(hipGetLastError());
         GCHK(launch_sweep_persist(h, true, kp, h->d_P2, h->d_Y2, h->aux, h->d_T2));
         HIPCHK(hipEventRecord(ev_join, h->aux));
@@ -2712,6 +2750,44 @@
     GCHK(launch_unpack(h, h->d_Y2, samples, ld, (int)k, mean));
     HIPCHK(hipEventRecord(h->ev1, h->stream));
     HIPCHK(hipStreamSynchronize(h->stream));
+    return GMRF_OK;
+}
+
+static bool posterior_fused_ok(gmrf_handle* h, int64_t k, bool dev_all) {
+    if (tw_on(h) || h->B <= 1 || !dev_all || h->no_fused_posterior || h->sweep_no_gemm || k <= 0 || k > KP_CHUNK) return false;
+    const int kp = pad_k(k);
+    if (kp % 64 != 0 || (int64_t)h->B * (h->bsp / 64) * (kp / 64) < 128) return false;
+    if ((int64_t)(kp + 1) * h->n_pad * 8 >= ((int64_t)1 << 32)) return false;
+    if (ensure_panels(h, kp + 1) != GMRF_OK) return false;
+    h->tail_probe = true; h->tail_refused = false;
+    const gmrf_status st = sweep_launches(h, true, kp, h->d_P, h->d_Y, true);
+    h->tail_probe = false;
+    return st == GMRF_OK && !h->tail_refused;
+}
+
+static gmrf_status posterior_fused(gmrf_handle* h, const double* b, uint64_t seed, int64_t first_id, int64_t k, double* mean,
+                                   double* samples, int64_t ld) {
+    const int kp = pad_k(k);
+    GCHK(ensure_panels(h, kp + 1));
+    HIPCHK(hipEventRecord(h->ev0, h->stream));
+    GCHK(launch_pack(h, b, h->n, 1, 1));
+    GCHK(run_sweeps(h, GMRF_SOLVE_FORWARD, 1));
+    {
+        const int64_t total = (int64_t)(kp + 1) * h->n_pad;
+        hipLaunchKernelGGL(fill_normals_panel, dim3((unsigned)((total + 255) / 256), (unsigned)h->B), dim3(256), 0,
+                           h->stream, h->d_P, h->n_pad, (int)h->bs, (int)h->bsp, (int)k, kp, seed, first_id, k, h->d_Y, h->n_pad);
+        HIPCHK(hipGetLastError());
+    }
+    GCHK(run_sweeps(h, SWEEP_BACKWARD_TAIL, kp));
+    {
+        const int64_t total = h->n * (k + 1);
+        hipLaunchKernelGGL(unpack_panel_mean, dim3((unsigned)((total + 255) / 256), (unsigned)h->B), dim3(256), 0, h->stream, h->d_Y,
+                           h->n_pad, samples, ld, mean, (int)h->bs, (int)h->bsp, h->n, (int)k, kp);
+        HIPCHK(hipGetLastError());
+    }
+    HIPCHK(hipEventRecord(h->ev1, h->stream));
+    HIPCHK(hipStreamSynchronize(h->stream));
+    if (h->profiling) prof_collect(h);
     return GMRF_OK;
 }
 
@@ -2724,17 +2800,19 @@
     HIPCHK(hipSetDevice(h->device));
     const bool dev_all = is_device_ptr(b) && is_device_ptr(mean) && is_device_ptr(samples);
     const int64_t vec_bytes = h->n * h->B * (int64_t)sizeof(double), smp_bytes = cols_bytes(h->n, k * h->B, ld);
-    bool beside = false;
+    bool beside = false, fused = false;
     GCHK(sweep_guarded(h, {{b, vec_bytes, mean, vec_bytes}, {b, vec_bytes, samples, smp_bytes}, {mean, vec_bytes, samples, smp_bytes}},
                        [&]() -> gmrf_status {
         beside = !tw_on(h) && h->B == 1 && k <= KP_CHUNK && k >= 2 && dev_all && !h->profiling && sweep_persist_ok(h, 1) &&
                  sweep_persist_ok(h, pad_k(k));
-        return beside ? posterior_beside(h, b, seed, first_id, k, mean, samples, ld) : GMRF_OK;
+        if (beside) return posterior_beside(h, b, seed, first_id, k, mean, samples, ld);
+        fused = !h->sweep_persist_hold && posterior_fused_ok(h, k, dev_all);
+        return fused ? posterior_fused(h, b, seed, first_id, k, mean, samples, ld) : GMRF_OK;
     }, [&]() -> gmrf_status {
-        HIPCHK(hipStreamSynchronize(h->aux));
+        if (h->aux) HIPCHK(hipStreamSynchronize(h->aux));
         return GMRF_OK;
     }));
-    if (!beside) {
+    if (!beside && !fused) {
         GCHK(gmrf_bt_solve(h, b, mean, 1, h->n, h->n, GMRF_SOLVE_FULL));
         return gmrf_bt_sample(h, seed, first_id, k, mean, nullptr, samples, ld);
     }
@@ -2758,7 +2836,7 @@
         GCHK(ensure_panels(h, kp));
         const int64_t total = (int64_t)kp * h->n_pad;
         hipLaunchKernelGGL(fill_normals_panel, dim3((unsigned)((total + 255) / 256), (unsigned)h->B), dim3(256), 0,
-                           h->stream, h->d_P, h->n_pad, (int)h->bs, (int)h->bsp, kc, kp, seed, first_id + c0, k);
+                           h->stream, h->d_P, h->n_pad, (int)h->bs, (int)h->bsp, kc, kp, seed, first_id + c0, k, nullptr, (int64_t)0);
         HIPCHK(hipGetLastError());
         GCHK(cols_out(h, h->d_P, kc, nullptr, z + c0 * ld, ld, z_dev));
         HIPCHK(hipStreamSynchronize(h->stream));
@@ -4497,15 +4575,17 @@
                            int32_t tri_flags, int32_t lower_only, double alpha, const double* A, int64_t lda,
                            const double* B, int64_t ldb, double beta, double* C, int64_t ldc) {
     if (M % 64 || N % 64 || K % 16 || (lda & 1) || (ldb & 1)) return bad_shape("gemm test sizes");
+    const bool tail = (tri_flags & 65536) != 0;
+    if (tail && (transA || transB)) return bad_shape("gemm test: the tail row needs A [m][k] and B [k][n]");
     HIPCHK(hipSetDevice(device));
-    const int64_t a_rows = transA ? K : M, b_rows = transB ? N : K;
+    const int64_t a_rows = transA ? K : M + (tail ? 1 : 0), b_rows = transB ? N : K, c_rows = M + (tail ? 1 : 0);
     double *dA, *dB, *dC;
     HIPCHK(hipMalloc(&dA, sizeof(double) * a_rows * lda));
     HIPCHK(hipMalloc(&dB, sizeof(double) * b_rows * ldb));
-    HIPCHK(hipMalloc(&dC, sizeof(double) * M * ldc));
+    HIPCHK(hipMalloc(&dC, sizeof(double) * c_rows * ldc));
     HIPCHK(hipMemcpy(dA, A, sizeof(double) * a_rows * lda, hipMemcpyHostToDevice));
     HIPCHK(hipMemcpy(dB, B, sizeof(double) * b_rows * ldb, hipMemcpyHostToDevice));
-    HIPCHK(hipMemcpy(dC, C, sizeof(double) * M * ldc, hipMemcpyHostToDevice));
+    HIPCHK(hipMemcpy(dC, C, sizeof(double) * c_rows * ldc, hipMemcpyHostToDevice));
     GemmArgs g;
     g.A = dA; g.B = dB; g.C = dC; g.lda = lda; g.ldb = ldb; g.ldc = ldc;
     g.strideA = g.strideB = g.strideC = 0;
@@ -4513,14 +4593,27 @@
     g.D = nullptr; g.ldd = 0; g.pD = 0;
     const bool force_big = (tri_flags & 2048) != 0, use_ll = (tri_flags & 4096) != 0;
     const int dma_shape = (tri_flags & 8192) ? 1 : ((tri_flags & 16384) ? 2 : ((tri_flags & 32768) ? 3 : 0));
-    g.M = (int)M; g.N = (int)N; g.K = (int)K; g.tri = tri_flags & ~(2048 | 4096 | 8192 | 16384 | 32768); g.lower_only = lower_only;
+    g.M = (int)M; g.N = (int)N; g.K = (int)K; g.tri = tri_flags & ~(2048 | 4096 | 8192 | 16384 | 32768 | 65536); g.lower_only = lower_only;
     g.alpha = alpha; g.beta = beta;
     unsigned long long* dst = nullptr;
     HIPCHK(hipMalloc(&dst, 16));
     HIPCHK(hipMemset(dst, 0, 16));
-    g.stamps = (force_big || use_ll || dma_shape) ? nullptr : dst;
+    g.stamps = (force_big || use_ll || dma_shape || tail) ? nullptr : dst;
     HIPCHK(gemm_init());
     HIPCHK(gemm_dma_init());
+    if (tail) {
+        const int saved_dma = gemm_dma_policy(), saved_ll = gemm_ll_policy();
+        gemm_dma_policy() = 1; gemm_ll_policy() = 2;
+        hipError_t le = hipSuccess;
+        const bool ok = gemm_try_dma_tail(nullptr, false, true, g, 1, nullptr, nullptr, &le);
+        gemm_dma_policy() = saved_dma; gemm_ll_policy() = saved_ll;
+        if (!ok) { hipFree(dst); hipFree(dA); hipFree(dB); hipFree(dC); return bad_shape("gemm test: not a tail-row product"); }
+        HIPCHK(le);
+        HIPCHK(hipDeviceSynchronize());
+        HIPCHK(hipMemcpy(C, dC, sizeof(double) * c_rows * ldc, hipMemcpyDeviceToHost));
+        hipFree(dst); hipFree(dA); hipFree(dB); hipFree(dC);
+        return GMRF_OK;
+    }
     const int saved = gemm_big_policy(), saved_ll = gemm_ll_policy(), saved_dma = gemm_dma_policy(), saved_force = gemm_dma_force();
     gemm_big_policy() = force_big ? 1 : 2;
     gemm_ll_policy() = use_ll ? 0 : 2;
@@ -4612,9 +4705,9 @@
     HIPCHK(hipMalloc(&dC, sizeof(double) * pm * batch));
     const int64_t tot = pm * batch;
     hipLaunchKernelGGL(fill_normals_panel, dim3((unsigned)((tot + 255) / 256)), dim3(256), 0, nullptr, dA, tot, 1 << 30,
-                       1 << 30, 1, 1, 1ull, 0, 0);
+                       1 << 30, 1, 1, 1ull, 0, 0, nullptr, (int64_t)0);
     hipLaunchKernelGGL(fill_normals_panel, dim3((unsigned)((tot + 255) / 256)), dim3(256), 0, nullptr, dB, tot, 1 << 30,
-                       1 << 30, 1, 1, 2ull, 0, 0);
+                       1 << 30, 1, 1, 2ull, 0, 0, nullptr, (int64_t)0);
     HIPCHK(hipMemset(dC, 0, sizeof(double) * pm * batch));
     GemmArgs g;
     g.A = dA; g.B = dB; g.C = dC; g.lda = g.ldb = g.ldc = ld;
diff --git a/diffeqgmrfs.jl_amd/csrc/misc_kernels.hpp b/diffeqgmrfs.jl_amd/csrc/misc_kernels.hpp
--- a/diffeqgmrfs.jl_amd/csrc/misc_kernels.hpp
+++ b/diffeqgmrfs.jl_amd/csrc/misc_kernels.hpp
@@ -109,15 +109,30 @@
 }
 
 __global__ void fill_normals_panel(double* __restrict__ P, int64_t n_pad, int bs, int bsp,
-                                   int k, int kp, uint64_t seed, int64_t first_id, int64_t id_stride) {
+                                   int k, int kp, uint64_t seed, int64_t first_id, int64_t id_stride,
+                                   const double* __restrict__ yrow, int64_t ystride) {
     const int64_t idx = (int64_t)blockIdx.x * blockDim.x + threadIdx.x;
-    if (idx >= (int64_t)kp * n_pad) return;
+    const int rows = kp + (yrow ? 1 : 0);
+    if (idx >= (int64_t)rows * n_pad) return;
     const int64_t r = idx / n_pad, j = idx % n_pad;
     const int64_t blk = j / bsp, off = j % bsp;
     double v = 0.0;
-    if (r < k && off < bs)
+    if (r == kp) v = yrow[(int64_t)blockIdx.y * ystride + j];
+    else if (r < k && off < bs)
         v = philox_normal(seed, (uint64_t)(blk * bs + off), (uint64_t)(first_id + (int64_t)blockIdx.y * id_stride + r));
-    P[(int64_t)blockIdx.y * kp * n_pad + idx] = v;
+    P[(int64_t)blockIdx.y * rows * n_pad + idx] = v;
+}
+
+__global__ void unpack_panel_mean(const double* __restrict__ P, int64_t n_pad, double* __restrict__ dst, int64_t ld,
+                                  double* __restrict__ mean_out, int bs, int bsp, int64_t n, int k, int kp) {
+    const int64_t idx = (int64_t)blockIdx.x * blockDim.x + threadIdx.x;
+    if (idx >= n * (int64_t)(k + 1)) return;
+    const int64_t r = idx / n, j = idx % n;
+    const int64_t blk = j / bs, off = j % bs;
+    const double* Pp = P + (int64_t)blockIdx.y * (kp + 1) * n_pad + blk * bsp + off;
+    const double mu = Pp[(int64_t)kp * n_pad];
+    if (r == k) mean_out[(int64_t)blockIdx.y * n + j] = mu;
+    else dst[((int64_t)blockIdx.y * k + r) * ld + j] = Pp[r * n_pad] + mu;
 }
 
 struct BxtArgs {
diff --git a/diffeqgmrfs.jl_amd/posterior.py b/diffeqgmrfs.jl_amd/posterior.py
--- a/diffeqgmrfs.jl_amd/posterior.py
+++ b/diffeqgmrfs.jl_amd/posterior.py
@@ -132,6 +132,12 @@
             outs = outs + [x] if keep else [x]
         return self.torch.cat(outs, dim=1) if keep else outs[0]
 
+    def posterior(self, k: int, seed: int, first_id: int, keep: bool = True):
+        if self.batch == 1 or k > 128:
+            mu = self.mean()
+            return mu, self.sample(k, mu, seed, first_id, keep)
+        return self.F.posterior_batch(self.rhs, k, seed=seed, first_id=first_id)
+
     def synchronize(self):
         self.torch.cuda.synchronize(self.dev)
 
@@ -268,10 +274,13 @@
 
     def step(self, step_index: int = 0):
         self._factor_and_share()
-        mu = self.e.mean()
         nb = getattr(self.e, "batch", 1)
         first = (step_index * self.world + self.rank) * self.k * nb
-        X = self.e.sample(self.k, mu, self.seed, first) if self.keep_samples else self.e.sample(self.k, mu, self.seed, first, keep=False)
+        if self.replicate and type(self.e) is HipEngine:
+            mu, X = self.e.posterior(self.k, self.seed, first, keep=self.keep_samples)
+        else:
+            mu = self.e.mean()
+            X = self.e.sample(self.k, mu, self.seed, first) if self.keep_samples else self.e.sample(self.k, mu, self.seed, first, keep=False)
         self._mark(3)
         return mu, X
 
```

Result: faster. 51420 solves/s, median of 6 (+5.1%).
